# OmerKerner/noLZSS

Measured on AMD Instinct MI355X. Metric: bases/sec factorized (1 GB sigma=4 DNA) + HBM GB/s fraction, higher is better.
Workload: dtype u32; 1 GPU; dna1g: one 2^30-base synthetic DNA sequence per GPU (sigma=4, 40% copied blocks, 1% substitutions), full factorization to (start,length,ref) records in HBM; bases_per_gpu=1073741824, parallelism=1 independent sequence shard(s), all-gather of counts

## Files before the change

### nolzss_amd/csrc/batch.hip

```cpp
#include "api_internal.hpp"

#include <array>

namespace nolzss {
namespace api {

constexpr uint8_t kBatchSeparator = 0x01;

struct RecordPlanScope {
    Context &ctx;
    RecordScatterPlan plan;
    RecordPlanScope(Context &c, const std::vector<uint32_t> &seps, uint32_t n) : ctx(c) {
        static const bool off = getenv("NOLZSS_NO_RECORD_SCATTER") != nullptr;
        if (off || seps.empty()) return;
        std::vector<uint32_t> terms(seps);
        terms.push_back(n);
        if (record_scatter_plan(terms, n, ctx.arena, ctx.stream, plan)) ctx.rec_plan = &plan;
    }
    ~RecordPlanScope() { ctx.rec_plan = nullptr; }
    RecordPlanScope(const RecordPlanScope &) = delete;
    RecordPlanScope &operator=(const RecordPlanScope &) = delete;
};
constexpr size_t kMergeChunkBases = size_t(1) << 25;
constexpr size_t kMergeLanes = 2;

__global__ void batch_bounds_kernel(const nolzss_factor *__restrict__ recs, uint32_t z,
                                    const uint32_t *__restrict__ seps, uint32_t nsep, uint32_t *__restrict__ fidx,
                                    uint32_t *__restrict__ err) {
    const uint32_t k = blockIdx.x * blockDim.x + threadIdx.x;
    if (k >= nsep) return;
    const uint64_t target = seps[k];
    uint32_t lo = 0, hi = z;
    while (lo < hi) {
        const uint32_t mid = lo + ((hi - lo) >> 1);
        if (recs[mid].start >= target)
            hi = mid;
        else
            lo = mid + 1;
    }
    fidx[k] = lo;
    if (lo >= z || recs[lo].start != target || recs[lo].length != 1) atomicOr(err, 1u);
}

__global__ void batch_bounds_pos_kernel(const uint32_t *__restrict__ fpos, uint32_t z,
                                        const uint32_t *__restrict__ seps, uint32_t nsep, uint32_t *__restrict__ fidx,
                                        uint32_t *__restrict__ err) {
    const uint32_t k = blockIdx.x * blockDim.x + threadIdx.x;
    if (k >= nsep) return;
    const uint32_t target = seps[k];
    uint32_t lo = 0, hi = z;
    while (lo < hi) {
        const uint32_t mid = lo + ((hi - lo) >> 1);
        if (fpos[mid] >= target)
            hi = mid;
        else
            lo = mid + 1;
    }
    fidx[k] = lo;
    if (lo >= z || fpos[lo] != target || (lo + 1 < z && fpos[lo + 1] != target + 1)) atomicOr(err, 1u);
}

__global__ void batch_rebase_kernel(nolzss_factor *__restrict__ recs, uint32_t z, TermTable terms) {
    const uint32_t j = blockIdx.x * blockDim.x + threadIdx.x;
    if (j >= z) return;
    const uint64_t p = recs[j].start;
    const uint32_t k = term_lower_bound(terms, (uint32_t)p);
    const uint64_t base = k ? (uint64_t)terms.pos[k - 1] + 1 : 0;
    recs[j].start = p - base;
    const uint64_t ref = recs[j].ref, flag = ref & (1ull << 63);
    recs[j].ref = ((ref ^ flag) - base) | flag;
}

void *alloc_factor_block(size_t bytes) {
    constexpr size_t kHuge = size_t(1) << 21;
    if (bytes >= 4 * kHuge) {
        void *p = nullptr;
        if (posix_memalign(&p, kHuge, (bytes + kHuge - 1) & ~(kHuge - 1)) == 0 && p) {
            (void)madvise(p, (bytes + kHuge - 1) & ~(kHuge - 1), MADV_HUGEPAGE);
            return p;
        }
    }
    return std::malloc(bytes);
}

bool run_merged_chunk(Context &ctx, const uint8_t *const *texts, const size_t *lens, const std::vector<size_t> &ids,
                      bool with_rc, size_t *zs, nolzss_factor **fs, std::vector<void *> *blocks, size_t *zs_plain) {
    if (zs_plain && (!with_rc || fs)) throw std::logic_error("run_merged_chunk: plain counts come with reverse-complement counts only");
    const bool trace = getenv("NOLZSS_TRACE") != nullptr;
    const auto t_begin = std::chrono::steady_clock::now();
    auto since = [&] { return std::chrono::duration<double, std::milli>(std::chrono::steady_clock::now() - t_begin).count(); };
    const size_t c = ids.size();
    size_t n = c - 1;
    for (size_t j : ids) n += lens[j];
    const bool direct = n / c >= (size_t(1) << 16);
    uint8_t *host = direct ? nullptr : host_stage(ctx, n);
    std::vector<uint32_t> seps;
    seps.reserve(c - 1);
    {
        size_t at = 0;
        for (size_t k = 0; k < c; ++k) {
            if (!direct) std::memcpy(host + at, texts[ids[k]], lens[ids[k]]);
            at += lens[ids[k]];
            if (k + 1 < c) {
                seps.push_back((uint32_t)at);
                if (!direct) host[at] = kBatchSeparator;
                ++at;
            }
        }
    }
    const double t_concat = since();
    Arena &arena = ctx.arena;
    hipStream_t s = ctx.stream;
    const size_t m2 = 2 * n + 2;
    reserve_arena_for(ctx, with_rc ? m2 : n, (with_rc ? m2 : 0) + n + 32 * c + (size_t(1) << 20) +
                                                (zs_plain ? 4 * n + (size_t(32) << 20) : 0));
    const size_t mark = arena.mark();
    struct Rewind {
        Arena &a;
        size_t m;
        ~Rewind() { a.rewind(m); }
    } rewind{arena, mark};
    uint8_t *d_text = arena.alloc<uint8_t>(n);
    if (direct) {
        ProfScope ps(ctx.profiler(), "batch_upload", s, (double)n);
        size_t at = 0;
        for (size_t k = 0; k < c; ++k) {
            upload_bytes(ctx, d_text + at, texts[ids[k]], lens[ids[k]]);
            at += lens[ids[k]];
            if (k + 1 < c) HIP_CHECK(hipMemsetAsync(d_text + at++, kBatchSeparator, 1, s));
        }
    } else {
        HIP_CHECK(hipMemcpyAsync(d_text, host, n, hipMemcpyHostToDevice, s));
    }
    PackedText text;
    void *d_recs = nullptr;
    uint32_t *d_fpos = nullptr;
    uint32_t z = 0;
    RcPlainOut plain;
    plain.want_fpos = c > 1;
    if (with_rc) {
        uint8_t *d_S = arena.alloc<uint8_t>(m2);
        prepare_batch_rc_on_device(ctx, d_text, (uint32_t)n, kBatchSeparator, d_S);
        std::vector<uint32_t> terms(seps);
        terms.reserve(2 * c);
        terms.push_back((uint32_t)n);
        for (size_t k = seps.size(); k-- > 0;) terms.push_back((uint32_t)(2 * n - seps[k]));
        terms.push_back((uint32_t)(2 * n + 1));
        if (!pack_independent_text(ctx, d_S, m2, terms, text, true)) return false;
        if (zs_plain)
            z = run_rc_pipeline_packed(ctx, text, 0, nullptr, &plain, &d_fpos);
        else
            z = run_rc_pipeline_packed(ctx, text, 0, &d_recs);
    } else {
        if (!pack_independent_text(ctx, d_text, n, seps, text)) return false;
        RecordPlanScope plan_scope(ctx, seps, (uint32_t)n);
        uint32_t *sa = arena.alloc<uint32_t>(n);
        uint32_t *isa = arena.alloc<uint32_t>(n);
        uint32_t *lcp = arena.alloc<uint32_t>(n + 1);
        bool isa_deferred = false;
        build_suffix_array(ctx, text, sa, isa, lcp, &isa_deferred);
        const Pyramid Psa = alloc_pyramid(sa, (uint32_t)n, arena), Plcp = alloc_pyramid(lcp, (uint32_t)n + 1, arena);
        uint32_t *lstar = arena.alloc<uint32_t>(n);
        build_lstar(ctx, (uint32_t)n, sa, isa, lcp, Psa, Plcp, lstar, isa_deferred ? isa : nullptr, &text);
        z = resolve_chain(ctx, (uint32_t)n, 0, lstar, sa, isa, lcp, Psa, Plcp, fs ? &d_recs : nullptr, 0, nullptr,
                          &d_fpos, fs ? &text.terms : nullptr);
    }
    nolzss_factor *recs = static_cast<nolzss_factor *>(d_recs);
    std::vector<uint32_t> fidx(c, z), fidx_plain(zs_plain ? c : 0, plain.z);
    if (c > 1) {
        uint32_t *d_fidx = arena.alloc<uint32_t>(c);
        HIP_CHECK(hipMemsetAsync(d_fidx + (c - 1), 0, sizeof(uint32_t), s));
        if (with_rc && !zs_plain)
            batch_bounds_kernel<<<(unsigned)div_up(c - 1, 256), 256, 0, s>>>(recs, z, text.terms.pos, (uint32_t)(c - 1),
                                                                             d_fidx, d_fidx + (c - 1));
        else
            batch_bounds_pos_kernel<<<(unsigned)div_up(c - 1, 256), 256, 0, s>>>(d_fpos, z, text.terms.pos,
                                                                                 (uint32_t)(c - 1), d_fidx, d_fidx + (c - 1));
        KERNEL_CHECK();
        uint32_t *d_fidx_plain = nullptr;
        if (zs_plain) {
            d_fidx_plain = arena.alloc<uint32_t>(c);
            HIP_CHECK(hipMemsetAsync(d_fidx_plain + (c - 1), 0, sizeof(uint32_t), s));
            batch_bounds_pos_kernel<<<(unsigned)div_up(c - 1, 256), 256, 0, s>>>(plain.fpos, plain.z, text.terms.pos,
                                                                                 (uint32_t)(c - 1), d_fidx_plain,
                                                                                 d_fidx_plain + (c - 1));
            KERNEL_CHECK();
            HIP_CHECK(hipMemcpyAsync(fidx_plain.data(), d_fidx_plain, c * sizeof(uint32_t), hipMemcpyDeviceToHost, s));
        }
        HIP_CHECK(hipMemcpyAsync(fidx.data(), d_fidx, c * sizeof(uint32_t), hipMemcpyDeviceToHost, s));
        HIP_CHECK(hipStreamSynchronize(s));
        if (fidx[c - 1] || (zs_plain && fidx_plain[c - 1])) throw HipError("merged batch: a separator is not a literal factor");
        fidx[c - 1] = z;
        if (zs_plain) fidx_plain[c - 1] = plain.z;
    }
    nolzss_factor *block = nullptr;
    if (fs && z) {
        if (with_rc) {
            batch_rebase_kernel<<<(unsigned)div_up(z, 256), 256, 0, s>>>(recs, z, text.terms);
            KERNEL_CHECK();
        }
        block = static_cast<nolzss_factor *>(alloc_factor_block(sizeof(nolzss_factor) * (size_t)z));
        if (!block) throw std::bad_alloc();
        try {
            download_bytes(ctx, block, recs, sizeof(nolzss_factor) * (size_t)z);
        } catch (...) {
            std::free(block);
            throw;
        }
    }
    const hipError_t e = hipStreamSynchronize(s);
    if (e != hipSuccess) {
        std::free(block);
        HIP_CHECK(e);
    }
    ctx.prof.collect();
    if (trace)
        fprintf(stderr, "[nolzss] merged batch run: %zu records, %zu symbols, %u factors: gather %.1f ms, device%s %.1f ms\n",
                c, n, z, t_concat, block ? " + download" : "", since() - t_concat);
    if (block) blocks->push_back(block);
    for (size_t k = 0; k < c; ++k) {
        const uint32_t a = k ? fidx[k - 1] + 1 : 0, b = fidx[k];
        zs[ids[k]] = b - a;
        if (fs) fs[ids[k]] = (block && b > a) ? block + a : nullptr;
        if (zs_plain) zs_plain[ids[k]] = (k ? fidx_plain[k] - fidx_plain[k - 1] - 1 : fidx_plain[k]);
    }
    return true;
}

struct GatherRec {
    const uint8_t *src;
    uint64_t off, len;
};
__global__ __launch_bounds__(256) void gather_records_kernel(const GatherRec *__restrict__ recs, uint32_t c,
                                                             uint8_t *__restrict__ dst, uint8_t sep) {
    for (uint32_t k = blockIdx.y; k < c; k += gridDim.y) {
        const GatherRec r = recs[k];
        for (uint64_t p0 = (uint64_t)blockIdx.x * 4096; p0 < r.len; p0 += (uint64_t)gridDim.x * 4096) {
            uint8_t b[16];
#pragma unroll
            for (int j = 0; j < 16; ++j) {
                const uint64_t p = p0 + (uint64_t)j * 256 + threadIdx.x;
                b[j] = r.src[p < r.len ? p : r.len - 1];
            }
#pragma unroll
            for (int j = 0; j < 16; ++j) {
                const uint64_t p = p0 + (uint64_t)j * 256 + threadIdx.x;
                if (p < r.len) dst[r.off + p] = b[j];
            }
        }
        if (blockIdx.x == 0 && threadIdx.x == 0 && k + 1 < c) dst[r.off + r.len] = sep;
    }
}

bool run_merged_chunk_device(Context &ctx, const void *const *d_texts, const size_t *lens, const std::vector<size_t> &ids,
                             bool emit, size_t *zs) {
    const size_t c = ids.size();
    size_t n = c - 1;
    for (size_t j : ids) n += lens[j];
    Arena &arena = ctx.arena;
    hipStream_t s = ctx.stream;
    reserve_arena_for(ctx, n, n + 64 * c + (size_t(1) << 20));
    const size_t mark = arena.mark();
    struct Rewind {
        Arena &a;
        size_t m;
        ~Rewind() { a.rewind(m); }
    } rewind{arena, mark};
    std::vector<GatherRec> table(c);
    std::vector<uint32_t> seps;
    seps.reserve(c - 1);
    {
        size_t at = 0;
        for (size_t k = 0; k < c; ++k) {
            table[k] = GatherRec{static_cast<const uint8_t *>(d_texts[ids[k]]), at, lens[ids[k]]};
            at += lens[ids[k]];
            if (k + 1 < c) seps.push_back((uint32_t)at++);
        }
    }
    uint8_t *d_text = arena.alloc<uint8_t>(n);
    GatherRec *d_table = arena.alloc<GatherRec>(c);
    HIP_CHECK(hipMemcpyAsync(d_table, table.data(), sizeof(GatherRec) * c, hipMemcpyHostToDevice, s));
    {
        ProfScope ps(ctx.profiler(), "batch_gather", s, 2.0 * (double)n);
        const size_t longest = lens[*std::max_element(ids.begin(), ids.end(), [&](size_t a, size_t b) { return lens[a] < lens[b]; })];
        const unsigned gy = (unsigned)std::min<size_t>(c, 32768);
        const unsigned gx = (unsigned)std::max<size_t>(1, std::min<size_t>(div_up(longest, 4096), div_up((size_t)65536, gy)));
        gather_records_kernel<<<dim3(gx, gy), 256, 0, s>>>(d_table, (uint32_t)c, d_text, kBatchSeparator);
        KERNEL_CHECK();
    }
    HIP_CHECK(hipStreamSynchronize(s));
    PackedText text;
    if (!pack_independent_text(ctx, d_text, n, seps, text)) return false;
    RecordPlanScope plan_scope(ctx, seps, (uint32_t)n);
    uint32_t *sa = arena.alloc<uint32_t>(n);
    uint32_t *isa = arena.alloc<uint32_t>(n);
    uint32_t *lcp = arena.alloc<uint32_t>(n + 1);
    bool isa_deferred = false;
    build_suffix_array(ctx, text, sa, isa, lcp, &isa_deferred);
    const Pyramid Psa = alloc_pyramid(sa, (uint32_t)n, arena), Plcp = alloc_pyramid(lcp, (uint32_t)n + 1, arena);
    uint32_t *lstar = arena.alloc<uint32_t>(n);
    build_lstar(ctx, (uint32_t)n, sa, isa, lcp, Psa, Plcp, lstar, isa_deferred ? isa : nullptr, &text);
    void *d_recs = nullptr;
    uint32_t *d_fpos = nullptr;
    const uint32_t z = resolve_chain(ctx, (uint32_t)n, 0, lstar, sa, isa, lcp, Psa, Plcp, emit ? &d_recs : nullptr, 0,
                                     nullptr, &d_fpos, emit ? &text.terms : nullptr);
    std::vector<uint32_t> fidx(c, z);
    if (c > 1) {
        uint32_t *d_fidx = arena.alloc<uint32_t>(c);
        HIP_CHECK(hipMemsetAsync(d_fidx + (c - 1), 0, sizeof(uint32_t), s));
        batch_bounds_pos_kernel<<<(unsigned)div_up(c - 1, 256), 256, 0, s>>>(d_fpos, z, text.terms.pos, (uint32_t)(c - 1),
                                                                             d_fidx, d_fidx + (c - 1));
        KERNEL_CHECK();
        HIP_CHECK(hipMemcpyAsync(fidx.data(), d_fidx, c * sizeof(uint32_t), hipMemcpyDeviceToHost, s));
        HIP_CHECK(hipStreamSynchronize(s));
        if (fidx[c - 1]) throw HipError("merged batch: a separator is not a literal factor");
        fidx[c - 1] = z;
    }
    HIP_CHECK(hipStreamSynchronize(s));
    ctx.prof.collect();
    for (size_t k = 0; k < c; ++k) {
        const uint32_t a = k ? fidx[k - 1] + 1 : 0, b = fidx[k];
        zs[ids[k]] = b - a;
    }
    return true;
}

std::atomic<uint64_t> g_merged_records{0}, g_single_records{0};

void check_records_both(const uint8_t *const *texts, const size_t *lens, size_t m) {
    size_t first_long = m;
    for (size_t j = 0; j < m && first_long == m; ++j)
        if (2 * lens[j] + 2 > kMaxText) first_long = j;
    static const auto cls = [] {
        std::array<uint8_t, 256> t;
        t.fill(2);
        for (const char *b = "ACGT"; *b; ++b) {
            t[(unsigned char)*b] = 0;
            t[(unsigned char)(*b + 32)] = 1;
        }
        return t;
    }();
    std::vector<size_t> start(m + 1, 0);
    for (size_t j = 0; j < m; ++j) start[j + 1] = start[j] + lens[j];
    std::atomic<size_t> first_bad{first_long}, first_lower{m};
    auto lower_to = [](std::atomic<size_t> &a, size_t v) {
        size_t cur = a.load();
        while (v < cur && !a.compare_exchange_weak(cur, v)) {
        }
    };
    host_parallel(start[m], [&](size_t lo, size_t hi) {
        size_t j = (size_t)(std::upper_bound(start.begin(), start.end(), lo) - start.begin()) - 1;
        for (size_t at = lo; at < hi && j < first_bad.load(std::memory_order_relaxed);) {
            while (start[j + 1] <= at) ++j;
            const size_t stop = std::min(hi, start[j + 1]);
            const uint8_t *p = texts[j] + (at - start[j]);
            uint8_t acc = 0;
            for (size_t k = 0, e = stop - at; k < e; ++k) acc |= cls[p[k]];
            if (acc & 2) lower_to(first_bad, j);
            if (acc & 1) lower_to(first_lower, j);
            at = stop;
        }
    });
    const size_t j = first_bad.load();
    if (j < m) {
        if (j == first_long) throw std::invalid_argument("text too long: the device pipeline uses 32-bit indices");
        const size_t k = first_invalid_nucleotide(reinterpret_cast<const char *>(texts[j]), lens[j]);
        throw std::runtime_error("Invalid nucleotide '" + std::string(1, (char)texts[j][k]) + "' found in sequence 0");
    }
    if (first_lower.load() < m)
        throw std::invalid_argument("record " + std::to_string(first_lower.load()) +
                                    " holds lower-case bases: both counts take upper-case A/C/G/T only (the plain count "
                                    "of lower-case letters differs)");
}

[[noreturn]] void rethrow_worker_error(int status, const std::string &message) {
    switch (status) {
    case NOLZSS_ERR_INVALID_ARGUMENT: throw std::invalid_argument(message);
    case NOLZSS_ERR_NOMEM: throw std::bad_alloc();
    case NOLZSS_ERR_DEVICE: throw HipError(message);
    default: throw std::runtime_error(message);
    }
}

std::mutex g_batch_mu;
std::map<nolzss_factor **, std::vector<void *>> g_batch_blocks;

size_t merge_below() {
    const char *e = getenv("NOLZSS_BATCH_MERGE_BELOW");
    return e ? (size_t)atoll(e) : (size_t(1) << 21);
}

BatchPlan plan_batch(const size_t *lens, size_t m, bool with_rc) {
    std::vector<size_t> singles;
    std::vector<std::vector<size_t>> chunks;
    const size_t below = with_rc ? merge_below() / 2 : merge_below();
    static const size_t chunk_bases = [] {
        const char *e = getenv("NOLZSS_BATCH_MERGE_BASES");
        const long long v = e ? atoll(e) : 0;
        return v > 0 ? (size_t)v : kMergeChunkBases;
    }();
    const size_t run_bases = with_rc ? chunk_bases / 2 : chunk_bases;
    const size_t long_below = [] {
        const char *e = getenv("NOLZSS_BATCH_MERGE_LONG_BELOW");
        return e ? (size_t)atoll(e) : (size_t(1) << 27);
    }();
    const size_t long_run_bases = [] {
        const char *e = getenv("NOLZSS_BATCH_MERGE_LONG_BASES");
        const long long v = e ? atoll(e) : 0;
        return v > 0 ? (size_t)v : (size_t(1) << 28);
    }();
    const size_t long_cut = with_rc ? long_below / 2 : long_below;
    const size_t long_run = with_rc ? long_run_bases / 4 : long_run_bases;
    std::vector<size_t> longs;
    if (below > 0)
        for (size_t j = 0; j < m; ++j)
            if (lens[j] >= below && lens[j] < long_cut) longs.push_back(j);
    if (longs.size() >= 2) {
        size_t total = 0;
        for (size_t j : longs) total += lens[j] + 1;
        size_t runs = div_up(total - longs.size(), long_run);
        if (runs < 2 && total >= (with_rc ? size_t(1) << 26 : size_t(1) << 27)) runs = 2;
        const size_t share = div_up(total, runs);
        std::vector<size_t> cur;
        size_t cur_bases = 0;
        for (size_t j : longs) {
            cur.push_back(j);
            cur_bases += lens[j] + 1;
            if (cur_bases >= share) {
                chunks.push_back(std::move(cur));
                cur.clear();
                cur_bases = 0;
            }
        }
        if (!cur.empty()) chunks.push_back(std::move(cur));
    } else {
        longs.clear();
    }
    const bool merge_longs = !longs.empty();
    {
        size_t short_bases = 0;
        for (size_t j = 0; j < m; ++j)
            if (lens[j] && lens[j] < below) short_bases += lens[j] + 1;
        const size_t runs = div_up(short_bases ? short_bases : 1, run_bases);
        const size_t share = div_up(short_bases, runs);
        std::vector<size_t> cur;
        size_t cur_bases = 0;
        for (size_t j = 0; j < m; ++j) {
            if (lens[j] == 0) continue;
            if (lens[j] >= below) {
                if (!(merge_longs && lens[j] < long_cut)) singles.push_back(j);
                continue;
            }
            cur.push_back(j);
// ... 353 lines not shown
```

### nolzss_amd/csrc/c_abi.hip

```cpp
#include "api_internal.hpp"

namespace nolzss {

void Context::read_back(const uint32_t *d_src, uint32_t *dst, int count) {
    HIP_CHECK(hipMemcpyAsync(h_pinned, d_src, sizeof(uint32_t) * count, hipMemcpyDeviceToHost, stream));
    HIP_CHECK(hipStreamSynchronize(stream));
    for (int k = 0; k < count; ++k) dst[k] = h_pinned[k];
}

namespace api {

thread_local std::string g_error;

int set_error(int code, const std::string &msg) {
    g_error = msg;
    return code;
}

std::mutex g_ctx_mu;
std::map<int, std::unique_ptr<DeviceContext>> g_ctx;

size_t arena_bytes_for(size_t n) { return kArenaBytesPerSymbol * n + kArenaSlack; }
size_t arena_min_bytes_for(size_t n) { return kArenaMinPerSymbol * n + kArenaSlack; }

// ... 3 lines not shown
        throw HipError("no HIP device available: libnolzss_hip has no CPU fallback");
    if (device < 0 || device >= count) throw std::invalid_argument("device ordinal out of range");
    if (lane < 0 || lane >= kMaxLanes) throw std::invalid_argument("lane out of range");
    std::lock_guard<std::mutex> lk(g_ctx_mu);
    auto &slot = g_ctx[device * kMaxLanes + lane];
    if (!slot) slot = std::make_unique<DeviceContext>();
    return *slot;
}

size_t trim_idle_arenas(int device, const Context *keep) {
    size_t released = 0;
    std::lock_guard<std::mutex> lk(g_ctx_mu);
    for (auto &kv : g_ctx) {
        DeviceContext &dc = *kv.second;
        if (&dc.ctx == keep || kv.first / kMaxLanes != device) continue;
        std::unique_lock<std::mutex> idle(dc.mu, std::try_to_lock);
        if (!idle.owns_lock()) continue;
        released += dc.ctx.arena.capacity();
        dc.ctx.arena.release();
    }
    return released;
}

void reserve_arena_for(Context &ctx, size_t n, size_t extra) {
    const size_t want = arena_bytes_for(n) + extra, least = arena_min_bytes_for(n) + extra;
    if (want <= ctx.arena.capacity()) return;
    auto available = [&]() -> size_t {
        size_t free_b = 0, total_b = 0;
        if (hipMemGetInfo(&free_b, &total_b) != hipSuccess) return ~size_t(0);
        return (size_t)((double)(free_b + ctx.arena.capacity()) * 0.97);
    };
    size_t avail = available();
    if (avail < want) {
        trim_idle_arenas(ctx.device, &ctx);
        avail = available();
    }
    if (avail < least) {
        if (least <= ctx.arena.capacity()) return;
        size_t free_b = 0, total_b = 0;
        (void)hipMemGetInfo(&free_b, &total_b);
        char buf[320];
        snprintf(buf, sizeof buf,
                 "input too large for this device: a text of %zu symbols needs at least %.1f GiB of device memory "
                 "(%zu bytes per symbol), %.1f GiB are free of %.1f GiB (one MI355X takes about %.1f Gi symbols in plain "
                 "mode, half of that with reverse complement)",
                 n, (double)least / 1073741824.0, kArenaMinPerSymbol, (double)free_b / 1073741824.0,
                 (double)total_b / 1073741824.0, (double)total_b * 0.97 / (double)kArenaMinPerSymbol / 1073741824.0);
        throw std::invalid_argument(buf);
    }
    const size_t take = want <= avail ? want : avail;
    if (take <= ctx.arena.capacity()) return;
    try {
        ctx.arena.reserve(take);
        return;
    } catch (const HipError &) {
        (void)hipGetLastError();
    }
    trim_idle_arenas(ctx.device, &ctx);
    ctx.arena.reserve(least > ctx.arena.capacity() ? least : ctx.arena.capacity());
}

uint8_t *host_stage(Context &ctx, size_t bytes) {
    if (bytes > ctx.h_stage_cap) {
        if (ctx.h_stage) (void)hipHostFree(ctx.h_stage);
        ctx.h_stage = nullptr;
        ctx.h_stage_cap = 0;
        const size_t cap = (bytes + (size_t(1) << 22)) & ~((size_t(1) << 22) - 1);
        HIP_CHECK(hipHostMalloc(reinterpret_cast<void **>(&ctx.h_stage), cap));
        ctx.h_stage_cap = cap;
    }
    return ctx.h_stage;
}

constexpr size_t kCopyChunk = size_t(8) << 20;
constexpr size_t kCopyThreshold = size_t(32) << 20;
int copy_threads() {
    static const int t = [] {
        const char *e = getenv("NOLZSS_COPY_THREADS");
        const long v = e ? atol(e) : 4;
        return (int)(v < 1 ? 1 : (v > 16 ? 16 : v));
    }();
    return t;
}

void upload_bytes(Context &ctx, void *d_dst, const void *h_src, size_t n) {
    HIP_CHECK(hipMemcpyAsync(d_dst, h_src, n, hipMemcpyHostToDevice, ctx.stream));
}

void download_bytes(Context &ctx, void *h_dst, const void *d_src, size_t n) {
    const int T = copy_threads();
    if (n < kCopyThreshold || T <= 1) {
        HIP_CHECK(hipMemcpyAsync(h_dst, d_src, n, hipMemcpyDeviceToHost, ctx.stream));
        HIP_CHECK(hipStreamSynchronize(ctx.stream));
        return;
    }
    uint8_t *ring = host_stage(ctx, (size_t)T * kCopyChunk);
    const size_t chunks = div_up(n, kCopyChunk);
    std::atomic<size_t> next{0};
    std::vector<hipError_t> err((size_t)T, hipSuccess);
    auto work = [&](int t) {
        hipError_t e = hipSetDevice(ctx.device);
        hipEvent_t ev = nullptr;
        if (e == hipSuccess) e = hipEventCreateWithFlags(&ev, hipEventDisableTiming);
        uint8_t *buf = ring + (size_t)t * kCopyChunk;
        while (e == hipSuccess) {
            const size_t c = next.fetch_add(1);
            if (c >= chunks) break;
            const size_t off = c * kCopyChunk, len = n - off < kCopyChunk ? n - off : kCopyChunk;
            e = hipMemcpyAsync(buf, static_cast<const uint8_t *>(d_src) + off, len, hipMemcpyDeviceToHost, ctx.stream);
            if (e == hipSuccess) e = hipEventRecord(ev, ctx.stream);
            if (e == hipSuccess) e = hipEventSynchronize(ev);
            if (e == hipSuccess) std::memcpy(static_cast<uint8_t *>(h_dst) + off, buf, len);
        }
        if (ev) (void)hipEventDestroy(ev);
        err[(size_t)t] = e;
    };
    std::vector<std::thread> threads;
    for (int t = 1; t < T; ++t) threads.emplace_back(work, t);
    work(0);
    for (auto &th : threads) th.join();
    for (hipError_t e : err) HIP_CHECK(e);
}

void order_behind_default_stream(Context &ctx) {
    hipEvent_t ev = nullptr;
    HIP_CHECK(hipEventCreateWithFlags(&ev, hipEventDisableTiming));
    hipError_t e = hipEventRecord(ev, nullptr);
    if (e == hipSuccess) e = hipStreamWaitEvent(ctx.stream, ev, 0);
    (void)hipEventDestroy(ev);
    HIP_CHECK(e);
}

void copy_out(Context &ctx, uint32_t *host, const uint32_t *dev, size_t count) {
    if (!host || !count) return;
    HIP_CHECK(hipMemcpyAsync(host, dev, count * sizeof(uint32_t), hipMemcpyDeviceToHost, ctx.stream));
}

size_t run_plain(Context &ctx, const uint8_t *d_text, size_t n, size_t start_pos, nolzss_factor **out_host,
                 DebugOut *dbg, bool records_on_device_only, const ChainLengthsOut *lengths, void **d_records_out) {
    if (out_host) *out_host = nullptr;
    if (d_records_out) *d_records_out = nullptr;
    if (n == 0 || start_pos >= n) return 0;
    Arena &arena = ctx.arena;
    const size_t mark = arena.mark();
    hipStream_t s = ctx.stream;

    PackedText text = pack_text(ctx, d_text, n);
    uint32_t *sa = arena.alloc<uint32_t>(n);
    uint32_t *isa = arena.alloc<uint32_t>(n);
    uint32_t *lcp = arena.alloc<uint32_t>(n + 1);
    bool isa_deferred = false;
    build_suffix_array(ctx, text, sa, isa, lcp, &isa_deferred);
    const Pyramid Psa = alloc_pyramid(sa, (uint32_t)n, arena), Plcp = alloc_pyramid(lcp, (uint32_t)n + 1, arena);
    uint32_t *lstar = arena.alloc<uint32_t>(n);
    build_lstar(ctx, (uint32_t)n, sa, isa, lcp, Psa, Plcp, lstar, isa_deferred ? isa : nullptr, &text);
    if (dbg) {
        copy_out(ctx, dbg->sa, sa, n);
        copy_out(ctx, dbg->isa, isa, n);
        copy_out(ctx, dbg->lcp, lcp, n + 1);
        copy_out(ctx, dbg->lstar, lstar, n);
        if (dbg->records) {
            const size_t rmark = arena.mark();
            const void *recs = position_factors(ctx, (uint32_t)n, lstar, sa, isa, lcp, Psa, Plcp);
            HIP_CHECK(hipMemcpyAsync(dbg->records, recs, n * sizeof(nolzss_factor), hipMemcpyDeviceToHost, s));
            HIP_CHECK(hipStreamSynchronize(s));
            arena.rewind(rmark);
        }
    }
    void *d_recs = nullptr;
    const uint32_t z = resolve_chain(ctx, (uint32_t)n, (uint32_t)start_pos, lstar, sa, isa, lcp, Psa, Plcp,
                                     (out_host || records_on_device_only || d_records_out) ? &d_recs : nullptr, 0, nullptr, nullptr,
                                     nullptr, lengths);
    if (out_host && z) {
        nolzss_factor *h = static_cast<nolzss_factor *>(alloc_factor_block(sizeof(nolzss_factor) * (size_t)z));
        if (!h) throw std::bad_alloc();
        ProfScope ps(ctx.profiler(), "factors_d2h", s);
        try {
            download_bytes(ctx, h, d_recs, sizeof(nolzss_factor) * (size_t)z);
        } catch (...) {
            std::free(h);
            throw;
        }
        *out_host = h;
    }
    {
        const hipError_t e = hipStreamSynchronize(s);
        if (e != hipSuccess) {
            if (out_host && *out_host) {
                std::free(*out_host);
                *out_host = nullptr;
            }
            HIP_CHECK(e);
        }
    }
    ctx.prof.collect();
    if (d_records_out) *d_records_out = d_recs;
    if (!lengths && !d_records_out) arena.rewind(mark);
    return z;
}

size_t run_plain_host(Context &ctx, const uint8_t *text, size_t n, size_t start_pos, nolzss_factor **out,
                      DebugOut *dbg) {
    if (out) *out = nullptr;
    if (n == 0 || start_pos >= n) return 0;
    reserve_arena_for(ctx, n, n);
    const size_t mark = ctx.arena.mark();
    uint8_t *d_text = ctx.arena.alloc<uint8_t>(n);
    {
        ProfScope ps(ctx.profiler(), "text_h2d", ctx.stream);
        upload_bytes(ctx, d_text, text, n);
    }
    size_t z;
    try {
        z = run_plain(ctx, d_text, n, start_pos, out, dbg);
    } catch (...) {
        ctx.arena.rewind(mark);
        throw;
    }
    ctx.arena.rewind(mark);
    return z;
}

void check_text_args(const void *text, size_t n, size_t start_pos) {
    if (n && !text) throw std::invalid_argument("text pointer is null");
    if (n > kMaxText) throw std::invalid_argument("text too long: the device pipeline uses 32-bit indices");
    if (start_pos > n) throw std::invalid_argument("start_pos beyond the end of the text");
}

uint8_t rc_sentinel(size_t index) {
    uint8_t s = 1;
    size_t count = 0;
    for (;;) {
        if (s != 0 && s != 'A' && s != 'C' && s != 'G' && s != 'T') {
            if (count == index) return s;
            ++count;
        }
        ++s;
        if (s == 0) s = 1;
    }
}

inline uint8_t upper_base(uint8_t c) { return (c >= 'a' && c <= 'z') ? (uint8_t)(c - 'a' + 'A') : c; }

inline uint8_t complement_base(uint8_t c) {
    switch (c) {
    case 'A': return 'T';
    case 'C': return 'G';
    case 'G': return 'C';
    default: return 'A';
    }
}

struct DnaTables {
    uint8_t invalid[256], comp[256];
    DnaTables() {
        for (int c = 0; c < 256; ++c) {
            invalid[c] = 1;
            comp[c] = 0;
        }
        const char *b = "ACGT", *r = "TGCA";
        for (int i = 0; i < 4; ++i) {
            invalid[(unsigned char)b[i]] = invalid[(unsigned char)(b[i] + 32)] = 0;
            comp[(unsigned char)b[i]] = comp[(unsigned char)(b[i] + 32)] = (uint8_t)r[i];
        }
    }
};
const DnaTables &dna_tables() {
    static const DnaTables t;
    return t;
}

size_t first_invalid_nucleotide(const char *s, size_t n) {
    const DnaTables &t = dna_tables();
    std::atomic<size_t> first{n};
    host_parallel(n, [&](size_t lo, size_t hi) {
        constexpr size_t kBlock = 4096;
        for (size_t at = lo; at < hi && at < first.load(std::memory_order_relaxed); at += kBlock) {
            const size_t stop = std::min(hi, at + kBlock);
            uint8_t bad = 0;
            for (size_t j = at; j < stop; ++j) bad |= t.invalid[(unsigned char)s[j]];
            if (bad)
                for (size_t j = at; j < stop; ++j)
                    if (t.invalid[(unsigned char)s[j]]) {
                        size_t cur = first.load();
                        while (j < cur && !first.compare_exchange_weak(cur, j)) {
                        }
                        return;
                    }
        }
    });
    return first.load();
}
void copy_upper(uint8_t *dst, const char *src, size_t n) {
    host_parallel(n, [&](size_t lo, size_t hi) {
        for (size_t j = lo; j < hi; ++j) dst[j] = (uint8_t)src[j] & 0xdfu;
    });
}
void copy_reverse_complement(uint8_t *dst, const char *src, size_t n) {
    const DnaTables &t = dna_tables();
    host_parallel(n, [&](size_t lo, size_t hi) {
        for (size_t j = lo; j < hi; ++j) dst[j] = t.comp[(unsigned char)src[n - 1 - j]];
    });
}

void prepare_w_rc(const char *const *seqs, const size_t *lens, size_t k, HostBytes &S,
                  size_t &original_length, std::vector<uint64_t> &sentinels) {
    S.clear();
    sentinels.clear();
    original_length = 0;
    if (k == 0) return;
    size_t non_empty = 0, empty = 0, total = 0;
    for (size_t i = 0; i < k; ++i) (lens[i] ? ++non_empty : ++empty);
    if (empty)
        fprintf(stderr, "Warning: Skipping %zu empty sequence(s) in prepare_multiple_dna_sequences_w_rc\n", empty);
    if (non_empty == 0) throw std::runtime_error("All sequences are empty - cannot prepare for factorization");
    if (non_empty > 125)
        throw std::invalid_argument(
            "Too many sequences: maximum 125 sequences supported (due to sentinel character limitations)");
    for (size_t i = 0; i < k; ++i) {
        const size_t j = first_invalid_nucleotide(seqs[i], lens[i]);
// ... 423 lines not shown
```

### nolzss_amd/csrc/chain.hip

```cpp
#include "pipeline.hpp"
#include "pyramid.hpp"
#include "scan.hpp"

#include <cassert>

namespace nolzss {
namespace {

constexpr int kThreads = 256;
constexpr int kTile = 4096;
constexpr int kPerThread = kTile / kThreads;
constexpr uint32_t kNone = 0xffffffffu;

constexpr uint32_t kLenMask = 0x7fffffffu;

__device__ __forceinline__ uint32_t next_pos(uint32_t p, uint32_t code, uint32_t n) {
    const uint32_t L = code & kLenMask;
    const uint64_t nx = (uint64_t)p + (L ? L : 1u);
    return nx > n ? n : (uint32_t)nx;
}

__global__ __launch_bounds__(kThreads) void chain_exit_kernel(const uint32_t *__restrict__ lstar, uint32_t n,
                                                              uint32_t start_pos,
                                                              uint32_t *__restrict__ exit0,
                                                              uint32_t *__restrict__ target_bits) {
    __shared__ uint32_t jump[kTile];
    const uint32_t base = blockIdx.x * (uint32_t)kTile;
    const uint32_t tile_end = (n - base < (uint32_t)kTile) ? n : base + kTile;
    const int tid = threadIdx.x;
    uint32_t ls[kPerThread];
#pragma unroll
    for (int j = 0; j < kPerThread; ++j) {
        const uint32_t p = base + j * kThreads + tid;
        ls[j] = lstar[p < n ? p : n - 1u];
    }
#pragma unroll
    for (int j = 0; j < kPerThread; ++j) {
        const uint32_t lp = j * kThreads + tid;
        const uint32_t p = base + lp;
        jump[lp] = (p < n) ? next_pos(p, ls[j], n) : n;
    }
    __syncthreads();
    for (int round = 0; round < 13; ++round) {
        int changed = 0;
#pragma unroll
        for (int j = 0; j < kPerThread; ++j) {
            const uint32_t lp = j * kThreads + tid;
            const uint32_t t = jump[lp];
            if (t < tile_end) {
                jump[lp] = jump[t - base];
                changed = 1;
            }
        }
        if (!__syncthreads_or(changed)) break;
    }
#pragma unroll
    for (int j = 0; j < kPerThread; ++j) {
        const uint32_t lp = j * kThreads + tid;
        const uint32_t p = base + lp;
        if (p < n) {
            const uint32_t e = jump[lp];
            exit0[p] = e;
            const bool last = (lp + 1 == (uint32_t)kTile) || (p + 1 >= n);
            if (e < n && (last || jump[lp + 1] != e)) atomicOr(&target_bits[e >> 5], 1u << (e & 31));
        }
    }
    if (blockIdx.x == 0 && tid == 0 && start_pos < n) atomicOr(&target_bits[start_pos >> 5], 1u << (start_pos & 31));
}

__global__ __launch_bounds__(kThreads) void popcount_kernel(const uint32_t *__restrict__ bits, uint32_t nwords,
                                                            uint32_t *__restrict__ counts) {
    const size_t stride = (size_t)gridDim.x * blockDim.x;
    for (size_t w = (size_t)blockIdx.x * blockDim.x + threadIdx.x; w < nwords; w += stride)
        counts[w] = (uint32_t)__popc(bits[w]);
}

__global__ __launch_bounds__(kThreads) void node_fill_kernel(const uint32_t *__restrict__ bits,
                                                             const uint32_t *__restrict__ prefix, uint32_t nwords,
                                                             uint32_t *__restrict__ node_pos) {
    const size_t stride = (size_t)gridDim.x * blockDim.x;
    for (size_t w = (size_t)blockIdx.x * blockDim.x + threadIdx.x; w < nwords; w += stride) {
        uint32_t b = bits[w];
        uint32_t id = prefix[w];
        while (b) {
            const int bit = __ffs((int)b) - 1;
            node_pos[id++] = (uint32_t)(w * 32 + bit);
            b &= b - 1;
        }
    }
}

__device__ __forceinline__ uint32_t node_id(const uint32_t *bits, const uint32_t *prefix, uint32_t p) {
    return prefix[p >> 5] + (uint32_t)__popc(bits[p >> 5] & ((1u << (p & 31)) - 1u));
}

__global__ __launch_bounds__(kThreads) void node_edges_kernel(const uint32_t *__restrict__ node_pos, uint32_t K,
                                                              const uint32_t *__restrict__ exit0, uint32_t n,
                                                              const uint32_t *__restrict__ bits,
                                                              const uint32_t *__restrict__ prefix,
                                                              uint32_t start_pos, uint32_t *__restrict__ nxt,
                                                              uint32_t *__restrict__ reach) {
    const size_t stride = (size_t)gridDim.x * blockDim.x;
    for (size_t k = (size_t)blockIdx.x * blockDim.x + threadIdx.x; k <= K; k += stride) {
        if (k == K) {
            nxt[k] = K;
            reach[k] = 0;
            continue;
        }
        const uint32_t p = node_pos[k];
        const uint32_t e = exit0[p];
        nxt[k] = (e >= n) ? K : node_id(bits, prefix, e);
        reach[k] = (p == start_pos) ? 1u : 0u;
    }
}

__global__ __launch_bounds__(kThreads) void wyllie_kernel(const uint32_t *__restrict__ nxt_in,
                                                          uint32_t *__restrict__ nxt_out, uint32_t K,
                                                          uint32_t *reach) {
    const size_t stride = (size_t)gridDim.x * blockDim.x;
    for (size_t k = (size_t)blockIdx.x * blockDim.x + threadIdx.x; k < K; k += stride) {
        const uint32_t w = nxt_in[k];
        if (w < K) {
            if (reach[k]) reach[w] = 1u;
            nxt_out[k] = nxt_in[w];
        } else {
            nxt_out[k] = K;
        }
    }
}

__global__ __launch_bounds__(kThreads) void tile_entries_kernel(const uint32_t *__restrict__ node_pos,
                                                                const uint32_t *__restrict__ reach, uint32_t K,
                                                                uint32_t *__restrict__ entry) {
    const size_t stride = (size_t)gridDim.x * blockDim.x;
    for (size_t k = (size_t)blockIdx.x * blockDim.x + threadIdx.x; k < K; k += stride)
        if (reach[k]) {
            const uint32_t p = node_pos[k];
            entry[p / kTile] = p;
        }
}

__global__ __launch_bounds__(64) void chain_mark_kernel(const uint32_t *__restrict__ lstar, uint32_t n,
                                                        const uint32_t *__restrict__ entry,
                                                        unsigned long long *__restrict__ chain_bits,
                                                        uint32_t *__restrict__ tile_count) {
    __shared__ uint16_t jmp[kTile];
    __shared__ unsigned long long bits[kTile / 64];
    const uint32_t base = blockIdx.x * (uint32_t)kTile;
    const uint32_t tile_end = (n - base < (uint32_t)kTile) ? n : base + kTile;
    const int lane = threadIdx.x;
    const uint32_t e = entry[blockIdx.x];
    const size_t word0 = (size_t)blockIdx.x * (kTile / 64);
    if (e == kNone) {
        chain_bits[word0 + lane] = 0ull;
        if (lane == 0) tile_count[blockIdx.x] = 0;
        return;
    }
    constexpr int kBatch = 16;
    for (int j0 = 0; j0 < kTile / 64; j0 += kBatch) {
        uint32_t ls[kBatch];
#pragma unroll
        for (int j = 0; j < kBatch; ++j) {
            const uint32_t p = base + (uint32_t)(j0 + j) * 64u + lane;
            ls[j] = lstar[p < n ? p : n - 1u];
        }
#pragma unroll
        for (int j = 0; j < kBatch; ++j) {
            const uint32_t lp = (uint32_t)(j0 + j) * 64u + lane;
            const uint32_t p = base + lp;
            uint32_t nl = kTile;
            if (p < n) {
                const uint32_t nx = next_pos(p, ls[j], n);
                if (nx < tile_end) nl = nx - base;
            }
            jmp[lp] = (uint16_t)nl;
        }
    }
    bits[lane] = 0ull;
    __syncthreads();
    if (lane == 0) {
        uint32_t p = e - base, cnt = 0;
        while (p < (uint32_t)kTile) {
            bits[p >> 6] |= 1ull << (p & 63);
            ++cnt;
            p = jmp[p];
        }
        tile_count[blockIdx.x] = cnt;
    }
    __syncthreads();
    chain_bits[word0 + lane] = bits[lane];
}

__global__ __launch_bounds__(64) void emit_positions_kernel(const unsigned long long *__restrict__ chain_bits,
                                                            const uint32_t *__restrict__ tile_off,
                                                            uint32_t *__restrict__ fpos) {
    const int lane = threadIdx.x;
    const size_t word = (size_t)blockIdx.x * (kTile / 64) + lane;
    unsigned long long b = chain_bits[word];
    const uint32_t c = (uint32_t)__popcll(b);
    uint32_t off = wave_scan_inclusive(c, OpAdd<uint32_t>()) - c + tile_off[blockIdx.x];
    const uint32_t p0 = blockIdx.x * (uint32_t)kTile + lane * 64u;
    while (b) {
        const int bit = __ffsll((long long)b) - 1;
        fpos[off++] = p0 + (uint32_t)bit;
        b &= b - 1;
    }
}

template <bool kRC>
__global__ __launch_bounds__(kThreads) void length_hist_kernel(const unsigned long long *__restrict__ chain_bits,
                                                               uint32_t nwords, const uint32_t *__restrict__ lstar,
                                                               uint32_t *__restrict__ hist,
                                                               uint64_t *__restrict__ tail,
                                                               uint32_t *__restrict__ tail_count, uint32_t tail_cap) {
    constexpr uint32_t T = kLengthHistBins;
    constexpr uint32_t kBins = kRC ? 2 * T : T;
    __shared__ uint32_t h[kBins];
    for (uint32_t b = threadIdx.x; b < kBins; b += kThreads) h[b] = 0;
    __syncthreads();
    const uint32_t stride = gridDim.x * kThreads;
    for (uint32_t w = blockIdx.x * kThreads + threadIdx.x; w < nwords; w += stride) {
        unsigned long long b = chain_bits[w];
        while (b) {
            const int bit = __ffsll((long long)b) - 1;
            b &= b - 1;
            const uint32_t code = lstar[(size_t)w * 64 + (uint32_t)bit];
            const uint32_t strand = kRC ? (code >> 31) : 0u;
            uint32_t L = code & kLenMask;
            L = L ? L : 1u;
            if (L < T) {
                atomicAdd(&h[strand * T + L], 1u);
            } else {
                const uint32_t slot = atomicAdd(tail_count, 1u);
                assert(slot < tail_cap);
                if (slot < tail_cap) tail[slot] = (uint64_t)L | ((uint64_t)strand << 32);
            }
        }
    }
    __syncthreads();
    for (uint32_t b = threadIdx.x; b < kBins; b += kThreads)
        if (h[b]) atomicAdd(&hist[b], h[b]);
}

__global__ __launch_bounds__(kThreads) void gather_lengths_kernel(uint32_t *__restrict__ fpos, uint32_t z,
                                                                  const uint32_t *__restrict__ lstar) {
    const size_t stride = (size_t)gridDim.x * blockDim.x;
    for (size_t k = (size_t)blockIdx.x * blockDim.x + threadIdx.x; k < z; k += stride) {
        const uint32_t L = lstar[fpos[k]] & kLenMask;
        fpos[k] = L ? L : 1u;
    }
}

constexpr uint32_t kEmitScan = 4;

struct FactorRec {
    uint64_t start, length, ref;
};

template <bool kRC, bool kRebase>
__global__ __launch_bounds__(kThreads) void factor_kernel(const uint32_t *__restrict__ fpos, uint32_t z,
                                                          const uint32_t *__restrict__ lstar,
                                                          const uint32_t *__restrict__ isa,
                                                          const uint32_t *__restrict__ sa,
                                                          const uint32_t *__restrict__ lcp, Pyramid Psa,
                                                          Pyramid Plcp, Pyramid Pmax, uint32_t rcN,
                                                          FactorRec *__restrict__ out, TermTable terms, uint32_t n) {
    const size_t stride = (size_t)gridDim.x * blockDim.x;
    for (size_t k = (size_t)blockIdx.x * blockDim.x + threadIdx.x; k < z; k += stride) {
        const uint32_t i = fpos[k];
        const uint32_t nxt = k + 1 < z ? fpos[k + 1] : n;
        uint32_t code = nxt - i;
        if (kRC || code == 1u) code = lstar[i];
        const uint32_t L = code & kLenMask;
        const bool is_rc = kRC && (code >> 31);
        FactorRec f;
        f.start = i;
        if (L == 0) {
            f.length = 1;
            f.ref = i;
        } else {
            const uint32_t r = isa[i] - 1u;
            uint32_t lo = r, hi = r + 1, steps = 0;
            while (lcp[lo] >= L) {
                --lo;
                if (++steps == kEmitScan) {
                    lo = (uint32_t)pyr_nearest_left<false>(Plcp, lo, L);
                    break;
                }
            }
            steps = 0;
            while (lcp[hi] >= L) {
                ++hi;
                if (++steps == kEmitScan) {
                    hi = pyr_nearest_right<false>(Plcp, hi, L);
                    break;
                }
            }
            hi -= 1;
            f.length = L;
            if (!is_rc) {
                uint32_t mn;
                if (hi - lo < 2 * kEmitScan) {
                    mn = kNone;
                    for (uint32_t q = lo; q <= hi; ++q) {
                        const uint32_t v = sa[q];
                        mn = v < mn ? v : mn;
                    }
                } else {
                    mn = pyr_range<false>(Psa, lo, hi);
                }
                f.ref = mn;
            } else {
                uint32_t mx;
                if (hi - lo < 2 * kEmitScan) {
                    mx = 0;
                    for (uint32_t q = lo; q <= hi; ++q) {
                        const uint32_t v = sa[q];
                        mx = v > mx ? v : mx;
                    }
                } else {
                    mx = pyr_range<true>(Pmax, lo, hi);
                }
                const uint64_t end = 2ull * rcN - mx;
                f.ref = (1ull << 63) | (end - L + 1);
            }
        }
        if (kRebase) {
            const uint32_t t = term_lower_bound(terms, i);
            const uint64_t base = t ? (uint64_t)terms.pos[t - 1] + 1 : 0;
            f.start -= base;
            f.ref -= base;
        }
        out[k] = f;
    }
}

inline unsigned grid_for(size_t items, unsigned cap = 256u * 16u) {
    size_t g = div_up(items, (size_t)kThreads);
    if (g < 1) g = 1;
    return (unsigned)(g > cap ? cap : g);
}

}

uint32_t resolve_chain(Context &ctx, uint32_t n, uint32_t start_pos, const uint32_t *lstar, const uint32_t *sa,
                       const uint32_t *isa, const uint32_t *lcp, const Pyramid &Psa, const Pyramid &Plcp,
                       void **d_factors_out, uint32_t rcN, const Pyramid *Pmax, uint32_t **d_fpos_out,
                       const TermTable *rebase, const ChainLengthsOut *lengths) {
    hipStream_t s = ctx.stream;
    Arena &arena = ctx.arena;
    if (d_factors_out) *d_factors_out = nullptr;
    if (d_fpos_out) *d_fpos_out = nullptr;
    if (start_pos >= n) return 0;

    const uint32_t num_tiles = (uint32_t)div_up(n, kTile);
    const uint32_t tbits_words = (uint32_t)div_up((size_t)n + 1, 32);

    uint32_t *fpos = nullptr;
    const size_t mark = arena.mark();
    uint32_t *exit0 = arena.alloc<uint32_t>(n);
    uint32_t *tbits = arena.alloc<uint32_t>(tbits_words);
    uint32_t *tprefix = arena.alloc<uint32_t>(tbits_words);
    uint32_t *d_total = arena.alloc<uint32_t>(2);
    HIP_CHECK(hipMemsetAsync(tbits, 0, sizeof(uint32_t) * tbits_words, s));
    {
        ProfScope ps(ctx.profiler(), "chain_exit", s);
        chain_exit_kernel<<<num_tiles, kThreads, 0, s>>>(lstar, n, start_pos, exit0, tbits);
        KERNEL_CHECK();
    }
    {
        ProfScope ps(ctx.profiler(), "chain_nodes", s);
        popcount_kernel<<<grid_for(tbits_words), kThreads, 0, s>>>(tbits, tbits_words, tprefix);
        KERNEL_CHECK();
        scan_exclusive_add_u32(tprefix, tprefix, tbits_words, d_total, arena, s);
    }
    uint32_t K = 0;
    ctx.read_back(d_total, &K, 1);

    uint32_t *node_pos = arena.alloc<uint32_t>(K + 1);
    uint32_t *nxt[2] = {arena.alloc<uint32_t>(K + 1), arena.alloc<uint32_t>(K + 1)};
    uint32_t *reach = arena.alloc<uint32_t>(K + 1);
    uint32_t *entry = arena.alloc<uint32_t>(num_tiles);
    {
        ProfScope ps(ctx.profiler(), "chain_nodes", s);
        node_fill_kernel<<<grid_for(tbits_words), kThreads, 0, s>>>(tbits, tprefix, tbits_words, node_pos);
        KERNEL_CHECK();
        node_edges_kernel<<<grid_for((size_t)K + 1), kThreads, 0, s>>>(node_pos, K, exit0, n, tbits, tprefix,
                                                                       start_pos, nxt[0], reach);
        KERNEL_CHECK();
    }
    {
        ProfScope ps(ctx.profiler(), "chain_wyllie", s);
        int rounds = 1;
        while ((1ull << rounds) < (uint64_t)K + 1) ++rounds;
        int cur = 0;
        for (int r = 0; r < rounds; ++r) {
            wyllie_kernel<<<grid_for(K), kThreads, 0, s>>>(nxt[cur], nxt[cur ^ 1], K, reach);
            KERNEL_CHECK();
            cur ^= 1;
        }
        HIP_CHECK(hipMemsetAsync(entry, 0xff, sizeof(uint32_t) * num_tiles, s));
        tile_entries_kernel<<<grid_for(K), kThreads, 0, s>>>(node_pos, reach, K, entry);
        KERNEL_CHECK();
    }
    unsigned long long *cbits = arena.alloc<unsigned long long>((size_t)num_tiles * (kTile / 64));
    uint32_t *tile_count = arena.alloc<uint32_t>(num_tiles);
    {
        ProfScope ps(ctx.profiler(), "chain_mark", s);
        chain_mark_kernel<<<num_tiles, 64, 0, s>>>(lstar, n, entry, cbits, tile_count);
        KERNEL_CHECK();
        scan_exclusive_add_u32(tile_count, tile_count, num_tiles, d_total + 1, arena, s);
    }
    uint32_t z = 0;
    ctx.read_back(d_total + 1, &z, 1);
    if (lengths) {
        if (d_factors_out || d_fpos_out) throw HipError("resolve_chain: factor lengths come without records");
        if (lengths->hist && z) {
            ProfScope ps(ctx.profiler(), "length_hist", s);
            const uint32_t nwords = num_tiles * (uint32_t)(kTile / 64);
            const unsigned g = grid_for(nwords, 1024);
            if (rcN)
                length_hist_kernel<true><<<g, kThreads, 0, s>>>(cbits, nwords, lstar, lengths->hist, lengths->tail,
                                                                lengths->tail_count, lengths->tail_cap);
            else
                length_hist_kernel<false><<<g, kThreads, 0, s>>>(cbits, nwords, lstar, lengths->hist, lengths->tail,
                                                                 lengths->tail_count, lengths->tail_cap);
            KERNEL_CHECK();
        }
        if (!lengths->order || z == 0) {
            arena.rewind(mark);
            return z;
        }
        fpos = arena.alloc<uint32_t>(z);
        ProfScope ps(ctx.profiler(), "length_emit", s);
        emit_positions_kernel<<<num_tiles, 64, 0, s>>>(cbits, tile_count, fpos);
        KERNEL_CHECK();
        gather_lengths_kernel<<<grid_for(z), kThreads, 0, s>>>(fpos, z, lstar);
        KERNEL_CHECK();
        *lengths->order = fpos;
        return z;
    }
    if ((!d_factors_out && !d_fpos_out) || z == 0) {
        arena.rewind(mark);
        return z;
    }
    fpos = arena.alloc<uint32_t>(z);
    if (!d_factors_out) {
        ProfScope ps(ctx.profiler(), "factor_emit", s);
        emit_positions_kernel<<<num_tiles, 64, 0, s>>>(cbits, tile_count, fpos);
        KERNEL_CHECK();
        *d_fpos_out = fpos;
        return z;
    }
    FactorRec *recs_tmp = arena.alloc<FactorRec>(z);
    {
        ProfScope ps(ctx.profiler(), "factor_emit", s);
        emit_positions_kernel<<<num_tiles, 64, 0, s>>>(cbits, tile_count, fpos);
        KERNEL_CHECK();
        if (rcN) {
            if (rebase) throw HipError("resolve_chain: record-relative output exists in plain mode only");
            factor_kernel<true, false><<<grid_for(z), kThreads, 0, s>>>(fpos, z, lstar, isa, sa, lcp, Psa, Plcp, *Pmax,
                                                                        rcN, recs_tmp, TermTable{}, n);
        } else if (rebase) {
            factor_kernel<false, true><<<grid_for(z), kThreads, 0, s>>>(fpos, z, lstar, isa, sa, lcp, Psa, Plcp, Psa,
                                                                        0u, recs_tmp, *rebase, n);
        } else {
            factor_kernel<false, false><<<grid_for(z), kThreads, 0, s>>>(fpos, z, lstar, isa, sa, lcp, Psa, Plcp, Psa,
                                                                         0u, recs_tmp, TermTable{}, n);
        }
        KERNEL_CHECK();
    }
    *d_factors_out = recs_tmp;
    if (d_fpos_out) *d_fpos_out = fpos;
    return z;
}

void *position_factors(Context &ctx, uint32_t n, const uint32_t *lstar, const uint32_t *sa, const uint32_t *isa,
                       const uint32_t *lcp, const Pyramid &Psa, const Pyramid &Plcp, uint32_t rcN, const Pyramid *Pmax,
                       const TermTable *rebase) {
    if (n == 0) return nullptr;
    hipStream_t s = ctx.stream;
    uint32_t *fpos = ctx.arena.alloc<uint32_t>(n);
    FactorRec *recs = ctx.arena.alloc<FactorRec>(n);
    std::vector<uint32_t> iota(n);
    for (uint32_t i = 0; i < n; ++i) iota[i] = i;
    HIP_CHECK(hipMemcpyAsync(fpos, iota.data(), (size_t)n * sizeof(uint32_t), hipMemcpyHostToDevice, s));
    HIP_CHECK(hipStreamSynchronize(s));
    if (rcN) {
        if (rebase) throw HipError("position_factors: record-relative output exists in plain mode only");
        factor_kernel<true, false><<<grid_for(n), kThreads, 0, s>>>(fpos, n, lstar, isa, sa, lcp, Psa, Plcp, *Pmax, rcN, recs,
                                                                    TermTable{}, n);
    } else if (rebase) {
        factor_kernel<false, true><<<grid_for(n), kThreads, 0, s>>>(fpos, n, lstar, isa, sa, lcp, Psa, Plcp, Psa, 0u, recs,
                                                                    *rebase, n);
    } else {
        factor_kernel<false, false><<<grid_for(n), kThreads, 0, s>>>(fpos, n, lstar, isa, sa, lcp, Psa, Plcp, Psa, 0u, recs,
                                                                     TermTable{}, n);
    }
    KERNEL_CHECK();
    return recs;
}

}
```

### nolzss_amd/csrc/lpnf.hip

```cpp
#include "pipeline.hpp"

#include <cstdlib>
#include "nearest_lds.hpp"
#include "queues.hpp"
#include "text_order.hpp"
#include "scan.hpp"

namespace nolzss {

__global__ void shard_totals_kernel(const uint32_t *const *counts, int nq, uint32_t *totals) {
    const int q = blockIdx.x;
    if (q >= nq) return;
    uint32_t v = threadIdx.x < kQShards ? counts[q][threadIdx.x * kQPad] : 0u;
    v = wave_reduce(v, OpAdd<uint32_t>());
    __shared__ uint32_t s_part[kQShards / 64];
    if (lane_id() == 0) s_part[threadIdx.x >> 6] = v;
    __syncthreads();
    if (threadIdx.x == 0) {
        uint32_t t = 0;
        for (uint32_t k = 0; k < kQShards / 64; ++k) t += s_part[k];
        totals[q] = t;
    }
}

namespace {

constexpr int kThreads = 256;
constexpr uint32_t kFarBothUnknown = 0xfffffffeu;

__device__ __forceinline__ bool lpf_decide(uint32_t i, uint32_t lp, uint32_t jp, uint32_t ls, uint32_t js,
                                           uint32_t *__restrict__ dst) {
    const uint32_t M = lp > ls ? lp : ls;
    if (M == 0) {
        *dst = 0;
        return false;
    }
    const bool ok = (lp == M && i - jp >= M) || (ls == M && i - js >= M);
    if (ok) {
        *dst = M;
        return false;
    }
    uint32_t lo = 0;
    if (lp > 0) { const uint32_t c = lp < i - jp ? lp : i - jp; lo = c > lo ? c : lo; }
    if (ls > 0) { const uint32_t c = ls < i - js ? ls : i - js; lo = c > lo ? c : lo; }
    *dst = lo;
    return true;
}

template <bool kTimed>
__global__ __launch_bounds__(kLdsThreads) void lpf_tile_kernel(const uint32_t *__restrict__ sa,
                                                               const uint32_t *__restrict__ lcp, uint32_t n,
                                                               uint32_t *__restrict__ lstar_by_rank,
                                                               ShardQueue exact_q, uint32_t *__restrict__ far_items,
                                                               uint32_t *__restrict__ far_cnt,
                                                               uint32_t *__restrict__ far_aux,
                                                               unsigned long long *__restrict__ phases,
                                                               uint32_t *__restrict__ psa1, uint32_t *__restrict__ plcp1,
                                                               uint32_t pending_min, uint32_t *__restrict__ pending_flag) {
    constexpr int NS = 2;
    const bool timed = kTimed && phases != nullptr && (blockIdx.x & 15) == 0;
    unsigned long long clk[6] = {0, 0, 0, 0, 0, 0};
    if (timed) clk[0] = __builtin_readcyclecounter();
    __shared__ __align__(16) uint32_t s_sa[kLdsSpan];
    __shared__ __align__(16) uint32_t s_lcp[kLdsSpan + 4];
    __shared__ uint32_t s_len[NS * kLdsTile];
    __shared__ uint16_t s_pos[NS * kLdsTile];
    constexpr int kListCapB = 64;
    __shared__ uint16_t s_list0[kLdsWaves][NS * kLdsPerWave];
    __shared__ uint16_t s_list1[kLdsWaves][NS * kListCapB];
    __shared__ uint32_t s_blk[3 * kBlkTableLen];
    const uint32_t base = blockIdx.x * (uint32_t)kLdsTile;
    const uint32_t shard = blockIdx.x % kQShards;
    stage_tile(sa, lcp, n, base, s_sa, s_lcp, pending_min, pending_flag);
    __syncthreads();
    const BlockTables T = block_tables<false>(s_blk);
    build_block_tables<false>(s_sa, s_lcp, T);
    __syncthreads();
    if (psa1 != nullptr && threadIdx.x < kLdsTile / kBlk) {
        const uint32_t B = (uint32_t)kLdsReach / kBlk + threadIdx.x;
        const uint64_t first = (uint64_t)base + (uint64_t)threadIdx.x * kBlk;
        if (first + kBlk <= (uint64_t)n) {
            psa1[first >> 4] = T.mn[B];
            plcp1[first >> 4] = T.ldn[B];
        }
    }
    if (timed) clk[1] = __builtin_readcyclecounter();
    const int w = threadIdx.x >> 6;
    const uint32_t far_bit = n <= 0x80000000u ? 0x80000000u : 0u;
    lds_search_wave_blocks<NS, NS, false, kLdsPerWave, kListCapB>(s_sa, s_lcp, T, n, base, s_len, s_pos, s_list0[w], s_list1[w],
                                   [](uint32_t) { return true; }, [](uint32_t) { return 0u; }, far_bit,
                                   timed ? clk + 2 : nullptr);
    if (timed) clk[4] = __builtin_readcyclecounter();
    constexpr int kRows = kLdsPerWave / 64;
    bool far[kRows], exact[kRows];
    uint32_t aux[kRows], known[kRows], fslot[kRows], eslot[kRows];
#pragma unroll
    for (int row = 0; row < kRows; ++row) {
        const int t = w * kLdsPerWave + row * 64 + lane_id();
        const uint64_t rr = (uint64_t)base + t;
        const bool in = rr < n;
        uint32_t up = s_len[t], down = s_len[kLdsTile + t];
        const bool fu = far_is(up, far_bit), fd = far_is(down, far_bit);
        far[row] = far_resolve(up, down, far_bit, 0u) && in;
        exact[row] = false;
        aux[row] = kFarBothUnknown;
        known[row] = 0;
        if (far[row]) {
            if (far_bit && fu != fd) {
                known[row] = fu ? down : up;
                const uint32_t p = match_pos(s_sa, fu ? s_pos[kLdsTile + t] : s_pos[t]);
                aux[row] = (known[row] ? (p & 0x7fffffffu) : 0x7fffffffu) | (fu ? 0x80000000u : 0u);
            }
        } else if (in) {
            exact[row] = lpf_decide(s_sa[t + kLdsReach], up, match_pos(s_sa, s_pos[t]), down, match_pos(s_sa, s_pos[kLdsTile + t]),
                                    lstar_by_rank + rr);
        }
    }
    {
        const uint32_t region = (blockIdx.x * (uint32_t)kLdsWaves + (uint32_t)w);
        uint32_t used = 0;
#pragma unroll
        for (int row = 0; row < kRows; ++row) {
            const uint64_t bal = __ballot(far[row]);
            fslot[row] = region * (uint32_t)kLdsPerWave + used + (uint32_t)__popcll(bal & lanemask_lt());
            used += (uint32_t)__popcll(bal);
        }
        if (lane_id() == 0) far_cnt[region] = used;
    }
    shard_slots<kRows>(exact_q, shard, exact, eslot);
#pragma unroll
    for (int row = 0; row < kRows; ++row) {
        const int t = w * kLdsPerWave + row * 64 + lane_id();
        const uint64_t rr = (uint64_t)base + t;
        if (far[row]) {
            far_items[fslot[row]] = (uint32_t)rr;
            lstar_by_rank[rr] = known[row];
            far_aux[rr] = aux[row];
        }
        if (exact[row]) exact_q.items[eslot[row]] = s_sa[t + kLdsReach];
    }
    if (timed) {
        __builtin_amdgcn_s_waitcnt(0);
        clk[5] = __builtin_readcyclecounter();
        if (lane_id() == 0) {
            for (int k = 0; k < 5; ++k) atomicAdd(phases + k, clk[k + 1] - clk[k]);
            atomicAdd(phases + 5, 1ull);
        }
    }
}

__global__ __launch_bounds__(kThreads) void compact_far_kernel(const uint32_t *__restrict__ far_items,
                                                               const uint32_t *__restrict__ far_cnt,
                                                               const uint32_t *__restrict__ far_off, uint32_t regions,
                                                               uint32_t *__restrict__ far_list) {
    const size_t stride = (size_t)gridDim.x * blockDim.x / 4;
    for (size_t r = ((size_t)blockIdx.x * blockDim.x + threadIdx.x) / 4; r < regions; r += stride) {
        const uint32_t c = far_cnt[r], o = far_off[r];
        for (uint32_t k = threadIdx.x & 3u; k < c; k += 4) far_list[o + k] = far_items[r * (size_t)kLdsPerWave + k];
    }
}

__global__ __launch_bounds__(kThreads) void lpf_far_kernel(const uint32_t *__restrict__ far_list, uint32_t far_count,
                                                           const uint32_t *__restrict__ sa,
                                                           const uint32_t *__restrict__ lcp, uint32_t n,
                                                           Pyramid Psa, Pyramid Plcp,
                                                           const uint32_t *__restrict__ by_rank,
                                                           const uint32_t *__restrict__ far_aux, bool bounded,
                                                           uint32_t *__restrict__ lstar, uint32_t *__restrict__ far_exact) {
    const size_t stride = (size_t)gridDim.x * blockDim.x;
    for (size_t k = (size_t)blockIdx.x * blockDim.x + threadIdx.x; k < far_count; k += stride) {
        const uint32_t r = far_list[k];
        const uint32_t i = sa[r];
        const uint32_t aux = far_aux[r];
        uint32_t lp, jp, ls, js;
        if (!bounded) {
            nearest_up<false>(sa, lcp, Psa, Plcp, r, i, 0u, lp, jp);
            nearest_down<false>(sa, lcp, n, Psa, Plcp, r, i, lp, ls, js);
        } else if (aux == kFarBothUnknown) {
            far_up<false>(sa, Psa, Plcp, r, i, 0u, lp, jp);
            far_down<false>(sa, n, Psa, Plcp, r, i, lp, ls, js);
        } else if (aux >> 31) {
            ls = by_rank[r];
            js = (aux & 0x7fffffffu) == 0x7fffffffu ? kNoPos : (aux & 0x7fffffffu);
            far_up<false>(sa, Psa, Plcp, r, i, ls, lp, jp);
        } else {
            lp = by_rank[r];
            jp = (aux & 0x7fffffffu) == 0x7fffffffu ? kNoPos : (aux & 0x7fffffffu);
            far_down<false>(sa, n, Psa, Plcp, r, i, lp, ls, js);
        }
        far_exact[k] = lpf_decide(i, lp, jp, ls, js, lstar + i) ? i : kNoPos;
    }
}

__global__ __launch_bounds__(kThreads) void lpnf_fallback_list_kernel(const uint32_t *__restrict__ far_exact,
                                                                      uint32_t far_count, uint32_t n,
                                                                      const uint32_t *__restrict__ isa, Pyramid Psa,
                                                                      Pyramid Plcp, uint32_t *__restrict__ lstar) {
    const size_t stride = (size_t)gridDim.x * blockDim.x;
    for (size_t k = (size_t)blockIdx.x * blockDim.x + threadIdx.x; k < far_count; k += stride) {
        const uint32_t i = far_exact[k];
        if (i == kNoPos) continue;
        const uint32_t cap = (n - i) < i ? (n - i) : i;
        lstar[i] = lpnf_search(Psa, Plcp, isa[i] - 1u, i, lstar[i], cap);
    }
}

__global__ __launch_bounds__(kThreads) void lpnf_fallback_kernel(ShardQueue exact_q, uint32_t n,
                                                                 const uint32_t *__restrict__ isa,
                                                                 Pyramid Psa, Pyramid Plcp,
                                                                 uint32_t *__restrict__ lstar) {
    const uint32_t shard = blockIdx.x;
    const uint32_t count = exact_q.counts[shard * kQPad];
    const uint32_t *items = exact_q.items + (size_t)shard * exact_q.cap;
    for (uint32_t k = blockIdx.y * blockDim.x + threadIdx.x; k < count; k += gridDim.y * blockDim.x) {
        const uint32_t i = items[k];
        const uint32_t cap = (n - i) < i ? (n - i) : i;
        lstar[i] = lpnf_search(Psa, Plcp, isa[i] - 1u, i, lstar[i], cap);
    }
}

}

uint32_t build_lstar(Context &ctx, uint32_t n, const uint32_t *sa, const uint32_t *isa, const uint32_t *lcp,
                     const Pyramid &Psa, const Pyramid &Plcp, uint32_t *lstar, uint32_t *isa_fill,
                     const PackedText *fill_pyramids) {
    hipStream_t s = ctx.stream;
    const size_t mark = ctx.arena.mark();
    uint32_t *pending_flag = nullptr;
    if (fill_pyramids) {
        pending_flag = ctx.arena.alloc<uint32_t>(1);
        HIP_CHECK(hipMemsetAsync(pending_flag, 0, sizeof(uint32_t), s));
        inject_pending_for_test(ctx, const_cast<uint32_t *>(lcp), n);
    }
    uint32_t *psa1 = fill_pyramids && Psa.nlev > 1 ? const_cast<uint32_t *>(Psa.lvl[1]) : nullptr;
    uint32_t *plcp1 = fill_pyramids && Plcp.nlev > 1 ? const_cast<uint32_t *>(Plcp.lvl[1]) : nullptr;
    if (!psa1 || !plcp1) psa1 = plcp1 = nullptr;
    const unsigned tiles = (unsigned)div_up(n, kLdsTile);
    ShardQueue exact_q;
    exact_q.cap = (uint32_t)shard_queue_cap(tiles, kLdsTile);
    exact_q.items = ctx.arena.alloc<uint32_t>((size_t)kQShards * exact_q.cap);
    const uint32_t far_regions = tiles * (uint32_t)kLdsWaves;
    uint32_t *far_items = ctx.arena.alloc<uint32_t>((size_t)far_regions * kLdsPerWave);
    uint32_t *far_cnt = ctx.arena.alloc<uint32_t>(far_regions);
    uint32_t *far_off = ctx.arena.alloc<uint32_t>(far_regions);
    uint32_t *qcounts = ctx.arena.alloc<uint32_t>(kQShards * kQPad);
    exact_q.counts = qcounts;
    const uint32_t **count_ptrs = ctx.arena.alloc<const uint32_t *>(1);
    uint32_t *totals = ctx.arena.alloc<uint32_t>(2);
    uint32_t *by_rank = ctx.arena.alloc<uint32_t>(n);
    uint32_t *far_aux = ctx.arena.alloc<uint32_t>(n);
    uint32_t *scratch_idx = ctx.arena.alloc<uint32_t>(n);
    uint32_t *scratch_val = ctx.arena.alloc<uint32_t>(isa_fill ? 2 * (size_t)n : (size_t)n);
    HIP_CHECK(hipMemsetAsync(qcounts, 0, kQShards * kQPad * sizeof(uint32_t), s));
    const uint32_t *h_ptrs[1] = {exact_q.counts};
    HIP_CHECK(hipMemcpyAsync(count_ptrs, h_ptrs, sizeof h_ptrs, hipMemcpyHostToDevice, s));
    HIP_CHECK(hipStreamSynchronize(s));
    auto read_totals = [&](uint32_t h[2]) {
        shard_totals_kernel<<<1, kQShards, 0, s>>>(count_ptrs, 1, totals);
        KERNEL_CHECK();
        ctx.read_back(totals, h, 2);
    };
    {
        ProfScope ps(ctx.profiler(), "lpf", s, 12.0 * (double)n);
        static const bool want_phases = getenv("NOLZSS_LPF_PHASES") != nullptr;
        unsigned long long *phases = nullptr;
        if (want_phases) {
            phases = ctx.arena.alloc<unsigned long long>(8);
            HIP_CHECK(hipMemsetAsync(phases, 0, 64, s));
        }
        if (phases)
            lpf_tile_kernel<true><<<tiles, kLdsThreads, 0, s>>>(sa, lcp, n, by_rank, exact_q, far_items, far_cnt, far_aux, phases, psa1, plcp1,
                                                                pending_threshold(), pending_flag);
        else
            lpf_tile_kernel<false><<<tiles, kLdsThreads, 0, s>>>(sa, lcp, n, by_rank, exact_q, far_items, far_cnt, far_aux, nullptr, psa1,
                                                                 plcp1, pending_threshold(), pending_flag);
        KERNEL_CHECK();
        if (phases) {
            unsigned long long h[8];
            HIP_CHECK(hipMemcpyAsync(h, phases, 64, hipMemcpyDeviceToHost, s));
            HIP_CHECK(hipStreamSynchronize(s));
            const double w = h[5] ? (double)h[5] : 1.0;
            fprintf(stderr, "[nolzss] lpf_tile phases (cycles per wavefront, %llu sampled): stage %.0f  round0 %.0f  %s %.0f  %s %.0f  epilogue %.0f\n",
                    h[5], h[0] / w, h[1] / w, "roundA", h[2] / w, "roundsBC", h[3] / w, h[4] / w);
        }
    }
    scan_exclusive_add_u32(far_cnt, far_off, far_regions, totals + 1, ctx.arena, s);
    if (fill_pyramids) {
        ProfScope ps(ctx.profiler(), "pyramids", s);
        if (psa1) {
            fill_pyramid_tail(Psa, n >> kPyrShift, false, s);
            fill_pyramid_tail(Plcp, n >> kPyrShift, false, s);
            fill_pyramid(Psa, 2, false, s);
            fill_pyramid(Plcp, 2, false, s);
        } else {
            fill_pyramid(Psa, 1, false, s);
            fill_pyramid(Plcp, 1, false, s);
        }
        uint32_t pending = 0;
        ctx.read_back(pending_flag, &pending, 1);
        if (pending) {
            ctx.arena.rewind(mark);
            finish_pending_lcp(ctx, *fill_pyramids, sa, const_cast<uint32_t *>(lcp));
            fill_pyramid(Psa, 1, false, s);
            fill_pyramid(Plcp, 1, false, s);
            return build_lstar(ctx, n, sa, isa, lcp, Psa, Plcp, lstar, isa_fill, nullptr);
        }
    }
    {
        ProfScope ps(ctx.profiler(), "lpf_to_text_order", s);
        uint32_t *idx[2] = {const_cast<uint32_t *>(sa), scratch_idx};
        uint32_t *val[2] = {by_rank, scratch_val};
        bucketed_scatter(idx, val, n, lstar, n, ctx.arena, s, ctx.profiler(), true, true, ctx.rec_plan, isa_fill);
    }
    uint32_t h[2] = {0, 0};
    read_totals(h);
    static const bool trace = getenv("NOLZSS_TRACE") != nullptr;
    if (trace) fprintf(stderr, "[nolzss] lpf: %u ranks to the far queue, %u positions to the exact search so far\n", h[1], h[0]);
    if (h[1] > 0) {
        ProfScope ps(ctx.profiler(), "lpf_far", s);
        uint32_t *far_list = ctx.arena.alloc<uint32_t>(h[1]);
        compact_far_kernel<<<(unsigned)std::min<size_t>(div_up((size_t)far_regions * 4, kThreads), 256u * 16u), kThreads, 0, s>>>(
            far_items, far_cnt, far_off, far_regions, far_list);
        KERNEL_CHECK();
        uint32_t *far_exact = ctx.arena.alloc<uint32_t>(h[1]);
        const unsigned g = (unsigned)std::min<size_t>(256u * 64u, std::max<size_t>(1, div_up(h[1], kThreads)));
        lpf_far_kernel<<<g, kThreads, 0, s>>>(far_list, h[1], sa, lcp, n, Psa, Plcp, by_rank, far_aux, n <= 0x80000000u,
                                              lstar, far_exact);
        KERNEL_CHECK();
        lpnf_fallback_list_kernel<<<g, kThreads, 0, s>>>(far_exact, h[1], n, isa, Psa, Plcp, lstar);
        KERNEL_CHECK();
    }
    if (h[0] > 0) {
        ProfScope ps(ctx.profiler(), "lpnf_fallback", s);
        const unsigned gy = (unsigned)std::min<size_t>(64, std::max<size_t>(1, div_up(h[0], (size_t)kQShards * kThreads)));
        lpnf_fallback_kernel<<<dim3(kQShards, gy), kThreads, 0, s>>>(exact_q, n, isa, Psa, Plcp, lstar);
        KERNEL_CHECK();
    }
    ctx.arena.rewind(mark);
    return h[0];
}

}
```

### nolzss_amd/csrc/pipeline.hpp

```cpp
#pragma once
#include "common.hpp"
#include "pyramid.hpp"
#include "text.hpp"

#include <vector>

namespace nolzss {

struct Context {
    int device = 0;
    hipStream_t stream = nullptr;
    Arena arena;
    Profiler prof;
    uint32_t *h_pinned = nullptr;
    uint8_t *h_stage = nullptr;
    size_t h_stage_cap = 0;
    const struct RecordScatterPlan *rec_plan = nullptr;

    Profiler *profiler() { return prof.enabled() ? &prof : nullptr; }
    void read_back(const uint32_t *d_src, uint32_t *dst, int count);
};

PackedText pack_text(Context &ctx, const uint8_t *d_text, size_t n);
bool pack_independent_text(Context &ctx, const uint8_t *d_text, size_t n, const std::vector<uint32_t> &separators,
                           PackedText &out, bool mirror = false);

int build_suffix_array(Context &ctx, const PackedText &text, uint32_t *sa, uint32_t *isa, uint32_t *lcp,
                       bool *isa_deferred = nullptr);
Pyramid build_lcp_pyramid(Context &ctx, const PackedText &text, const uint32_t *sa, uint32_t *lcp);

struct Pyramid;

uint32_t build_lstar(Context &ctx, uint32_t n, const uint32_t *sa, const uint32_t *isa, const uint32_t *lcp,
                     const Pyramid &Psa, const Pyramid &Plcp, uint32_t *lstar, uint32_t *isa_fill = nullptr,
                     const PackedText *fill_pyramids = nullptr);
uint32_t pending_threshold();
void finish_pending_lcp(Context &ctx, const PackedText &text, const uint32_t *sa, uint32_t *lcp);
void inject_pending_for_test(Context &ctx, uint32_t *lcp, uint32_t n);

constexpr uint32_t kLengthHistBins = 2048;
struct ChainLengthsOut {
    uint32_t *hist = nullptr;
    uint64_t *tail = nullptr;
    uint32_t *tail_count = nullptr;
    uint32_t tail_cap = 0;
    uint32_t **order = nullptr;
};
inline uint32_t length_tail_cap(uint32_t n) { return n / kLengthHistBins + 1u; }
uint32_t resolve_chain(Context &ctx, uint32_t n, uint32_t start_pos, const uint32_t *lstar, const uint32_t *sa,
                       const uint32_t *isa, const uint32_t *lcp, const Pyramid &Psa, const Pyramid &Plcp,
                       void **d_factors_out, uint32_t rcN = 0, const Pyramid *Pmax = nullptr,
                       uint32_t **d_fpos_out = nullptr, const TermTable *rebase = nullptr,
                       const ChainLengthsOut *lengths = nullptr);
void *position_factors(Context &ctx, uint32_t n, const uint32_t *lstar, const uint32_t *sa, const uint32_t *isa,
                       const uint32_t *lcp, const Pyramid &Psa, const Pyramid &Plcp, uint32_t rcN = 0,
                       const Pyramid *Pmax = nullptr, const TermTable *rebase = nullptr);

struct RcPlainOut;
struct RcDebugOut;
uint32_t run_rc_pipeline(Context &ctx, const uint8_t *d_S, size_t m, size_t start_pos, void **d_factors_out,
                         RcPlainOut *plain = nullptr, const ChainLengthsOut *lengths = nullptr,
                         RcDebugOut *dbg = nullptr);
struct RcPlainOut {
    bool want_fpos = false;
    uint32_t z = 0;
    uint32_t *fpos = nullptr;
};
struct RcDebugOut {
    uint32_t *sa = nullptr;
    uint32_t *lcp = nullptr;
    uint32_t *isa = nullptr;
    uint32_t *code = nullptr;
    uint32_t *plain = nullptr;
    void *records = nullptr;
    uint32_t far_ranks = 0;
    uint32_t exact_from_tiles = 0;
    uint32_t exact_total = 0;
    uint32_t compact = 0;
    uint32_t pending_relaunch = 0;
};
uint32_t run_rc_pipeline_packed(Context &ctx, const PackedText &text, size_t start_pos, void **d_factors_out,
                                RcPlainOut *plain = nullptr, uint32_t **d_fpos_out = nullptr,
                                const ChainLengthsOut *lengths = nullptr, RcDebugOut *dbg = nullptr);
void prepare_batch_rc_on_device(Context &ctx, const uint8_t *d_T, uint32_t n, uint8_t separator, uint8_t *d_S);
uint32_t prepare_single_rc_on_device(Context &ctx, const uint8_t *d_T, uint32_t n, uint8_t *d_S);

struct RlzLayout {
    uint32_t total = 0;
    uint32_t block_length = 0;
    uint32_t rc_block_start = 0;
    uint32_t chain_end = 0;
    uint32_t rcN = 0;
    bool with_rc = false;
};
void rlz_candidates(Context &ctx, const uint32_t *sa, const uint32_t *lcp, uint32_t m, uint32_t B, uint32_t E, bool with_rc,
                    uint32_t *by_rank);
uint32_t run_rlz_pipeline(Context &ctx, const uint8_t *d_S, const RlzLayout &lay, void **d_factors_out,
                          uint32_t **d_fpos_out = nullptr, uint32_t *h_codes = nullptr);
void rlz_count_per_target(Context &ctx, const uint32_t *d_fpos, uint32_t z, const uint32_t *d_bounds, uint32_t k,
                          uint32_t *d_counts);

}
```

### nolzss_amd/csrc/radix_sort.hip

```cpp
#include "radix_sort.hpp"

#include "local_sort.hpp"
#include "radix_pass.hpp"

#include <cstdlib>

namespace nolzss {

SortKnobs::SortKnobs() {
    auto set = [](const char *name) { return getenv(name) != nullptr; };
    auto i64 = [](const char *name, long long dflt) { return getenv(name) ? atoll(getenv(name)) : dflt; };
    trace = set("NOLZSS_TRACE");
    scatter_phases = set("NOLZSS_SCATTER_PHASES");
    no_local_sort = set("NOLZSS_NO_LOCAL_SORT");
    local_sort_min_set = set("NOLZSS_LOCAL_SORT_MIN");
    local_sort_min = (size_t)i64("NOLZSS_LOCAL_SORT_MIN", 0);
    no_local_regroup = set("NOLZSS_NO_LOCAL_REGROUP");
    no_key35 = set("NOLZSS_NO_KEY35");
    local_regroup_min = (size_t)i64("NOLZSS_LOCAL_REGROUP_MIN", 3ll << 28);
    test_local_order_fails = set("NOLZSS_TEST_LOCAL_ORDER_FAILS");
    test_local_lookback_fails = set("NOLZSS_TEST_LOCAL_LOOKBACK_FAILS");
    rec_bucket_min = (uint64_t)i64("NOLZSS_REC_BUCKET_MIN", 1ll << 16);
    text_order_hist = set("NOLZSS_TEXT_ORDER_HIST");
    const char *esc = getenv("NOLZSS_TEXT_ORDER_ESC");
    text_order_esc = esc ? (long long)strtoul(esc, nullptr, 0) : -1;
}

const SortKnobs &sort_knobs() {
    static const SortKnobs k;
    return k;
}

namespace {

template <int BITS> struct TextSrc {
    using Raw = SymWords;
    static constexpr bool kFromText = true;
    const uint64_t *__restrict__ words;
    TermTable terms;
    bool segmented;
    bool digit_from_text = true;
    __device__ __forceinline__ Raw load(size_t idx, const TileExtent &) const { return sym_words<BITS>(words, idx); }
    __device__ __forceinline__ uint64_t key_of(const Raw &raw, size_t idx, const TileExtent &) const {
        return initial_key_of<BITS>(sym_word_of<BITS>(raw, idx), terms, segmented, (uint32_t)idx);
    }
    __device__ __forceinline__ uint32_t val(size_t idx) const { return (uint32_t)idx; }
    __device__ __forceinline__ uint32_t hist_digit_of(const Raw &raw, size_t idx, int shift, const TileExtent &ext) const {
        constexpr int kKeyBits = KeyLayout<BITS>::kSyms * BITS + KeyLayout<BITS>::kTagBits;
        if (!segmented && digit_from_text && shift == kKeyBits - kRadixBits)
            return digit_of(sym_word_of<BITS>(raw, idx) >> (64 - kKeyBits), shift);
        return digit_of(key_of(raw, idx, ext), shift);
    }
    __device__ __forceinline__ bool digits_from_window(int shift) const {
        constexpr int kKeyBits = KeyLayout<BITS>::kSyms * BITS + KeyLayout<BITS>::kTagBits;
        return BITS == 2 && !segmented && digit_from_text && shift == kKeyBits - kRadixBits;
    }
    __device__ __forceinline__ uint64_t window(size_t idx) const { return sym_word<BITS>(words, idx); }
    __device__ __forceinline__ uint32_t window_digit(uint64_t w, int j, size_t) const {
        return (uint32_t)((w >> (64 - kRadixBits - 2 * j)) & (uint64_t)(kBins - 1));
    }
};
struct Text16Src {
    using Raw = SymWords;
    static constexpr bool kFromText = true;
    const uint64_t *__restrict__ words;
    uint32_t n;
    __device__ __forceinline__ uint32_t suffix_of(size_t idx) const {
        return idx < 16 ? n - 1u - (uint32_t)idx : (uint32_t)idx - 16u;
    }
    __device__ __forceinline__ Raw load(size_t idx, const TileExtent &) const { return sym_words<2>(words, suffix_of(idx)); }
    __device__ __forceinline__ uint64_t key_of(const Raw &raw, size_t idx, const TileExtent &) const {
        const uint32_t s = suffix_of(idx);
        const uint32_t lim = n - s;
        const uint32_t tag = lim < (uint32_t)kP16Syms ? lim : (uint32_t)kP16Syms;
        return ((sym_word_of<2>(raw, s) >> 32) << kP16TagBits) | tag;
    }
    __device__ __forceinline__ uint32_t val(size_t idx) const { return suffix_of(idx); }
    __device__ __forceinline__ uint32_t hist_digit_of(const Raw &raw, size_t idx, int, const TileExtent &) const {
        return (uint32_t)(sym_word_of<2>(raw, suffix_of(idx)) >> (64 - kRadixBits));
    }
    __device__ __forceinline__ bool digits_from_window(int) const { return true; }
    __device__ __forceinline__ uint64_t window(size_t idx0) const { return sym_word<2>(words, idx0 == 0 ? (uint64_t)n - 16u : idx0 - 16u); }
    __device__ __forceinline__ uint32_t window_digit(uint64_t w, int j, size_t idx0) const {
        const int jj = idx0 == 0 ? 15 - j : j;
        return (uint32_t)((w >> (64 - kRadixBits - 2 * jj)) & (uint64_t)(kBins - 1));
    }
};
struct Text35Src : Text16Src {
    __device__ __forceinline__ uint64_t key_of(const Raw &raw, size_t idx, const TileExtent &) const {
        const uint32_t s = suffix_of(idx);
        const uint32_t lim = n - s;
        const uint32_t tag = lim < (uint32_t)kP35Syms ? lim : (uint32_t)kP35Syms;
        return ((sym_word_of<2>(raw, s) >> (64 - kP35KeyBits)) << kP35TagBits) | tag;
    }
};
struct Text16SegSrc {
    using Raw = SymWords;
    static constexpr bool kFromText = true;
    const uint64_t *__restrict__ words;
    uint32_t n;
    uint32_t treal;
    uint32_t end_shorts;
    uint32_t nshort;
    uint32_t pos[kTermFew];
    __device__ __forceinline__ uint32_t suffix_of(size_t idx) const {
        if (idx < nshort) {
            const uint32_t c0 = treal, c1 = treal + (end_shorts ? 1u : 0u);
            uint32_t L = 0, j = (uint32_t)idx;
            if (idx >= c0) {
                L = 1u + ((uint32_t)idx - c0) / c1;
                j = ((uint32_t)idx - c0) % c1;
            }
            const uint32_t pj = j == 0 ? pos[0] : (j == 1 ? pos[1] : (j == 2 ? pos[2] : pos[3]));
            return pj - L;
        }
        uint32_t p = (uint32_t)idx - nshort;
#pragma unroll
        for (uint32_t k = 0; k + 1 < kTermFew; ++k)
            if (k < treal && p + 15u >= pos[k]) p += 16u;
        return p;
    }
    __device__ __forceinline__ uint32_t limit_of(uint32_t s) const {
        uint32_t next = n;
#pragma unroll
        for (int k = (int)kTermFew - 2; k >= 0; --k)
            if ((uint32_t)k < treal && pos[k] >= s) next = pos[k];
        return next - s;
    }
    __device__ __forceinline__ uint32_t masked(const Raw &raw, uint32_t s, uint32_t &tag) const {
        const uint32_t lim = limit_of(s);
        tag = lim < (uint32_t)kP16Syms ? lim : (uint32_t)kP16Syms;
        uint32_t sym = (uint32_t)(sym_word_of<2>(raw, s) >> 32);
        if (tag < (uint32_t)kP16Syms) sym = tag == 0 ? 0u : (sym & ~((1u << (2 * ((uint32_t)kP16Syms - tag))) - 1u));
        return sym;
    }
    __device__ __forceinline__ Raw load(size_t idx, const TileExtent &) const { return sym_words<2>(words, suffix_of(idx)); }
    __device__ __forceinline__ uint64_t key_of(const Raw &raw, size_t idx, const TileExtent &) const {
        uint32_t tag;
        const uint32_t sym = masked(raw, suffix_of(idx), tag);
        return ((uint64_t)sym << kP16TagBits) | tag;
    }
    __device__ __forceinline__ uint32_t val(size_t idx) const { return suffix_of(idx); }
    __device__ __forceinline__ uint32_t hist_digit_of(const Raw &raw, size_t idx, int, const TileExtent &) const {
        uint32_t tag;
        return masked(raw, suffix_of(idx), tag) >> (32 - kRadixBits);
    }
    __device__ __forceinline__ bool digits_from_window(int) const { return false; }
    __device__ __forceinline__ uint64_t window(size_t) const { return 0; }
};
struct RecordTextSrc {
    using Raw = SymWords;
    static constexpr bool kFromText = true;
    const uint64_t *__restrict__ words;
    const uint32_t *__restrict__ term_pos;
    __device__ __forceinline__ Raw load(size_t idx, const TileExtent &) const { return sym_words<2>(words, idx); }
    __device__ __forceinline__ uint32_t key_of(const Raw &raw, size_t idx, const TileExtent &ext) const {
        const uint64_t w = sym_word_of<2>(raw, idx);
        const uint32_t lim = term_pos[ext.bucket] - (uint32_t)idx;
        const uint32_t tag = lim < (uint32_t)kRecSyms ? lim : (uint32_t)kRecSyms;
        uint32_t sym = (uint32_t)(w >> (64 - kRecSyms * 2));
        if (tag < (uint32_t)kRecSyms) sym &= ~((1u << (2 * (kRecSyms - (int)tag))) - 1u);
        return (sym << kRecTagBits) | tag;
    }
    __device__ __forceinline__ uint32_t val(size_t idx) const { return (uint32_t)idx; }
    __device__ __forceinline__ uint32_t hist_digit_of(const Raw &raw, size_t idx, int shift, const TileExtent &ext) const {
        return digit_of(key_of(raw, idx, ext), shift);
    }
    __device__ __forceinline__ bool digits_from_window(int) const { return false; }
    __device__ __forceinline__ uint64_t window(size_t) const { return 0; }
};

struct RecArraySrc {
    using Raw = uint64_t;
    static constexpr bool kDigitInRecord = true;
    const uint64_t *__restrict__ recs;
    __device__ __forceinline__ Raw load(size_t idx, const TileExtent &) const { return recs[idx]; }
    __device__ __forceinline__ uint64_t rec_of(Raw raw, size_t, const TileExtent &, uint32_t &) const { return raw; }
};
// ... 486 lines not shown
```

### nolzss_amd/csrc/radix_sort.hpp

```cpp
#pragma once
#include "common.hpp"
#include "text.hpp"

#include <vector>

namespace nolzss {

constexpr int kRadixBits = 8;
#ifndef NOLZSS_SORT_TILE
#define NOLZSS_SORT_TILE 4096
#endif
constexpr int kSortTile = NOLZSS_SORT_TILE;
static_assert(kSortTile == 4096 || kSortTile == 8192, "16 keys per thread on 256 or 512 threads");

constexpr int kSegDescWords = 12;
struct SegView {
    const uint32_t *desc = nullptr;
    uint32_t num_tiles = 0;
};

struct TileExtent {
    size_t first;
    uint32_t count;
    uint32_t bucket;
    size_t hist0;
    uint32_t hstride;
    uint32_t bkt_first, bkt_end, prev_ne, next_ne;
    uint32_t aux;
};

__device__ __forceinline__ TileExtent tile_extent(uint32_t tile, size_t n, uint32_t num_tiles, const SegView &seg) {
    TileExtent e;
    if (seg.desc == nullptr) {
        e.first = (size_t)tile * kSortTile;
        e.count = (uint32_t)((n - e.first < (size_t)kSortTile) ? (n - e.first) : (size_t)kSortTile);
        e.bucket = 0;
        e.hist0 = tile;
        e.hstride = num_tiles;
        e.bkt_first = 0;
        e.bkt_end = (uint32_t)n;
        e.prev_ne = e.next_ne = 0;
        e.aux = 0;
        return e;
    }
    const uint4 *d = reinterpret_cast<const uint4 *>(seg.desc + (size_t)tile * kSegDescWords);
    const uint4 a = d[0], b = d[1], c = d[2];
    e.first = a.x;
    e.count = a.y;
    e.bucket = a.z;
    e.hist0 = a.w;
    e.hstride = b.x;
    e.bkt_first = b.y;
    e.bkt_end = b.z;
    e.prev_ne = b.w;
    e.next_ne = c.x;
    e.aux = c.y;
    return e;
}

struct SortKnobs {
    SortKnobs();
    bool trace;
    bool scatter_phases;
    bool no_local_sort;
    bool local_sort_min_set;
    size_t local_sort_min;
    static constexpr size_t kLocalSortMinText = size_t(1) << 28;
    static constexpr size_t kLocalSortMinRecord = size_t(1) << 20;
    size_t local_min(size_t dflt) const { return local_sort_min_set ? local_sort_min : dflt; }
    bool no_local_regroup;
    size_t local_regroup_min;
    bool no_key35;
    bool test_local_order_fails;
    bool test_local_lookback_fails;
    uint64_t rec_bucket_min;
    bool text_order_hist;
    long long text_order_esc;
};
const SortKnobs &sort_knobs();

int radix_sort_pairs(uint64_t *keys[2], uint32_t *vals[2], size_t n, const int *shifts,
                     int npasses, Arena &arena, hipStream_t stream, Profiler *prof = nullptr);
int radix_sort_pairs(uint32_t *keys[2], uint32_t *vals[2], size_t n, const int *shifts,
                     int npasses, Arena &arena, hipStream_t stream, Profiler *prof = nullptr);

void radix_pass_low16(const uint32_t *keys, const uint32_t *vals, uint16_t *keys16_out, uint32_t *vals_out, size_t n, int shift,
                      Arena &arena, hipStream_t stream, Profiler *prof = nullptr);

int radix_sort_initial_keys(const PackedText &text, uint64_t *keys[2], uint32_t *vals[2], const int *shifts,
                            int npasses, Arena &arena, hipStream_t stream, Profiler *prof = nullptr);

void radix_sort_dna_keys(const PackedText &text, uint32_t *keys32[2], uint32_t *vals[2], uint32_t *seg_mem,
                         SegView &seg_out, Arena &arena, hipStream_t stream, Profiler *prof = nullptr);

bool key16_applicable(const PackedText &text);
struct Round0Regroup {
    uint32_t *lcp = nullptr;
    uint32_t *new_slot = nullptr, *new_grp = nullptr;
    uint32_t *d_total = nullptr;
    bool done = false;
};
void radix_sort_dna_keys16(const PackedText &text, uint32_t *keys32[2], uint32_t *vals[2], uint32_t *seg_mem,
                           SegView &seg_out, Arena &arena, hipStream_t stream, Profiler *prof = nullptr,
                           Round0Regroup *regroup = nullptr, bool key35 = false);
bool key35_applicable(const PackedText &text);

void radix_sort_dna_keys16_fused(const PackedText &text, uint64_t *rec[2], uint32_t *sa_out, uint32_t *seg_mem,
                                 SegView &seg_out, Arena &arena, hipStream_t stream, Profiler *prof = nullptr);

void radix_sort_record_keys(const PackedText &text, const std::vector<uint32_t> &h_terms, uint32_t *keys32[2],
                            uint32_t *vals[2], uint32_t *seg_mem, SegView &seg_out, Arena &arena, hipStream_t stream,
                            Profiler *prof = nullptr);

int radix_sort_segments_u32(uint32_t *keys[2], uint32_t *vals[2], size_t n, const std::vector<uint32_t> &h_start, int npasses,
                            Arena &arena, hipStream_t stream, Profiler *prof = nullptr);

}
```

### nolzss_amd/csrc/rc.hip

```cpp
#include <algorithm>

#include "nearest_lds.hpp"
#include "pipeline.hpp"
#include "queues.hpp"
#include "text_order.hpp"
#include "scan.hpp"

namespace nolzss {
namespace {

constexpr int kThreads = 256;
constexpr uint32_t kRcFlag = 0x80000000u;

__device__ __forceinline__ uint32_t rc_select(uint32_t fwd, uint32_t rc) {
    if (fwd >= 1) return (rc > fwd) ? (rc | kRcFlag) : fwd;
    return (rc > 1) ? (rc | kRcFlag) : 0u;
}

template <bool kPlain>
__device__ __forceinline__ bool rc_decide(uint32_t i, uint32_t lp, uint32_t jp, uint32_t ls, uint32_t js,
                                          uint32_t rc, uint32_t *__restrict__ dst, uint32_t *__restrict__ plain) {
    const uint32_t M = lp > ls ? lp : ls;
    const bool fwd_final = (M == 0) || (lp == M && i - jp >= M) || (ls == M && i - js >= M);
    if (fwd_final) {
// ... 320 lines not shown
    const bool fused_level1 = Pmin.nlev > 1 && Plcp.nlev > 1;
    uint32_t *pending_flag = arena.alloc<uint32_t>(1);
    HIP_CHECK(hipMemsetAsync(pending_flag, 0, sizeof(uint32_t), s));
    inject_pending_for_test(ctx, lcp, m);
    uint32_t *code = arena.alloc<uint32_t>(m);
    uint32_t *plain = plain_out ? arena.alloc<uint32_t>(N) : nullptr;
    {
        const size_t mark = arena.mark();
        const unsigned tiles = (unsigned)div_up(m, kLdsTile);
        ShardQueue exact_q, far_q;
        exact_q.cap = far_q.cap = (uint32_t)shard_queue_cap(tiles, kLdsTile);
        exact_q.items = arena.alloc<uint32_t>((size_t)kQShards * exact_q.cap);
        exact_q.items2 = arena.alloc<uint32_t>((size_t)kQShards * exact_q.cap);
        far_q.items = arena.alloc<uint32_t>((size_t)kQShards * far_q.cap);
        uint32_t *qcounts = arena.alloc<uint32_t>(2 * kQShards * kQPad);
        exact_q.counts = qcounts;
        far_q.counts = qcounts + kQShards * kQPad;
        const uint32_t **count_ptrs = arena.alloc<const uint32_t *>(2);
        uint32_t *totals = arena.alloc<uint32_t>(2);
        uint32_t *by_rank = arena.alloc<uint32_t>(m);
        static const bool no_compact = getenv("NOLZSS_RC_NO_COMPACT") != nullptr;
        static const uint32_t compact_min = getenv("NOLZSS_RC_COMPACT_MIN") ? (uint32_t)atoll(getenv("NOLZSS_RC_COMPACT_MIN")) : (1u << 22);
        const bool compact = isa_deferred && !no_compact && N >= compact_min && N <= (1u << 30);
        uint32_t *scratch_idx = nullptr, *scratch_val = nullptr, *tile_off = nullptr, *cidx = nullptr;
        uint64_t *cpacked = nullptr;
        if (compact) {
            uint32_t *tile_cnt = arena.alloc<uint32_t>(tiles);
            tile_off = arena.alloc<uint32_t>(tiles);
            cidx = arena.alloc<uint32_t>(N);
            cpacked = arena.alloc<uint64_t>(N);
            ProfScope ps(ctx.profiler(), "rc_candidates", s);
            rc_count_original_kernel<<<tiles, kLdsThreads, 0, s>>>(sa, m, N, tile_cnt);
            KERNEL_CHECK();
            scan_exclusive_add_u32(tile_cnt, tile_off, tiles, nullptr, arena, s);
        } else {
            scratch_idx = arena.alloc<uint32_t>(m);
            scratch_val = arena.alloc<uint32_t>(isa_deferred ? 2 * (size_t)m : (size_t)m);
        }
        uint32_t *plain_by_rank = plain ? (compact ? by_rank : arena.alloc<uint32_t>(m)) : nullptr;
        auto launch_tile = [&](uint32_t *p1, uint32_t *p2, uint32_t *p3, uint32_t pmin, uint32_t *pflag) {
            if (plain)
                rc_tile_kernel<true><<<tiles, kLdsThreads, 0, s>>>(sa, lcp, m, N, by_rank, exact_q, far_q, p1, p2, p3, pmin,
                                                                   pflag, tile_off, cidx, cpacked, plain_by_rank);
            else
                rc_tile_kernel<false><<<tiles, kLdsThreads, 0, s>>>(sa, lcp, m, N, by_rank, exact_q, far_q, p1, p2, p3, pmin,
                                                                    pflag, tile_off, cidx, cpacked, nullptr);
            KERNEL_CHECK();
        };
        HIP_CHECK(hipMemsetAsync(qcounts, 0, 2 * kQShards * kQPad * sizeof(uint32_t), s));
        const uint32_t *h_ptrs[2] = {exact_q.counts, far_q.counts};
        HIP_CHECK(hipMemcpyAsync(count_ptrs, h_ptrs, sizeof h_ptrs, hipMemcpyHostToDevice, s));
        HIP_CHECK(hipStreamSynchronize(s));
        auto read_totals = [&](uint32_t h[2]) {
            shard_totals_kernel<<<2, kQShards, 0, s>>>(count_ptrs, 2, totals);
            KERNEL_CHECK();
            ctx.read_back(totals, h, 2);
        };
        {
            ProfScope ps(ctx.profiler(), "rc_candidates", s);
            launch_tile(fused_level1 ? const_cast<uint32_t *>(Pmin.lvl[1]) : nullptr,
                        fused_level1 ? const_cast<uint32_t *>(Pmax.lvl[1]) : nullptr,
                        fused_level1 ? const_cast<uint32_t *>(Plcp.lvl[1]) : nullptr, pending_threshold(), pending_flag);
        }
        {
            ProfScope ps(ctx.profiler(), "pyramids", s);
            const int from = fused_level1 ? 2 : 1;
            if (fused_level1) {
                fill_pyramid_tail(Pmin, m >> kPyrShift, false, s);
                fill_pyramid_tail(Pmax, m >> kPyrShift, true, s);
                fill_pyramid_tail(Plcp, m >> kPyrShift, false, s);
            }
            fill_pyramid(Pmin, from, false, s);
            fill_pyramid(Pmax, from, true, s);
            fill_pyramid(Plcp, from, false, s);
            uint32_t pending = 0;
            ctx.read_back(pending_flag, &pending, 1);
            if (pending) {
                if (dbg) dbg->pending_relaunch = 1;
                finish_pending_lcp(ctx, text, sa, lcp);
                fill_pyramid(Pmin, 1, false, s);
                fill_pyramid(Pmax, 1, true, s);
                fill_pyramid(Plcp, 1, false, s);
                HIP_CHECK(hipMemsetAsync(qcounts, 0, 2 * kQShards * kQPad * sizeof(uint32_t), s));
                launch_tile(nullptr, nullptr, nullptr, 0u, nullptr);
            }
        }
        {
            ProfScope ps(ctx.profiler(), "rc_to_text_order", s);
            if (compact) {
                permute_packed(cidx, cpacked, N, code, isa, arena, s, ctx.profiler());
            } else {
                uint32_t *idx[2] = {sa, scratch_idx};
                uint32_t *val[2] = {by_rank, scratch_val};
                bucketed_scatter(idx, val, m, code, m, arena, s, ctx.profiler(), true, true, nullptr, isa_deferred ? isa : nullptr,
                                 false);
            }
        }
        if (plain) {
            ProfScope ps(ctx.profiler(), "rc_plain_gather", s);
            size_t g = div_up(N, kThreads);
            if (g > 8192) g = 8192;
            rc_plain_gather_kernel<<<(unsigned)g, kThreads, 0, s>>>(isa, plain_by_rank, N, plain);
            KERNEL_CHECK();
        }
        uint32_t h[2] = {0, 0};
        read_totals(h);
        if (dbg) {
            dbg->compact = compact ? 1u : 0u;
            dbg->far_ranks = h[1];
            dbg->exact_from_tiles = h[0];
        }
        if (h[1] > 0) {
            ProfScope ps(ctx.profiler(), "rc_far", s);
            const unsigned gy = (unsigned)std::min<size_t>(64, std::max<size_t>(1, div_up(h[1], (size_t)kQShards * kThreads)));
            if (plain)
                rc_far_kernel<true><<<dim3(kQShards, gy), kThreads, 0, s>>>(far_q, sa, lcp, m, N, Pmin, Pmax, Plcp, by_rank, code,
                                                                            exact_q, plain);
            else
                rc_far_kernel<false><<<dim3(kQShards, gy), kThreads, 0, s>>>(far_q, sa, lcp, m, N, Pmin, Pmax, Plcp, by_rank, code,
                                                                             exact_q, nullptr);
            KERNEL_CHECK();
            read_totals(h);
        }
        if (h[0] > 0) {
            ProfScope ps(ctx.profiler(), "rc_fallback", s);
            const unsigned gy = (unsigned)std::min<size_t>(64, std::max<size_t>(1, div_up(h[0], (size_t)kQShards * kThreads)));
            if (plain)
                rc_fallback_kernel<true><<<dim3(kQShards, gy), kThreads, 0, s>>>(exact_q, m, isa, lcp, Pmin, Plcp, code, plain);
            else
                rc_fallback_kernel<false><<<dim3(kQShards, gy), kThreads, 0, s>>>(exact_q, m, isa, lcp, Pmin, Plcp, code, nullptr);
            KERNEL_CHECK();
        }
        if (dbg) {
            dbg->exact_total = h[0];
            auto copy_out = [&](uint32_t *host, const uint32_t *dev, size_t count) {
                if (host && count) HIP_CHECK(hipMemcpyAsync(host, dev, count * sizeof(uint32_t), hipMemcpyDeviceToHost, s));
            };
            copy_out(dbg->sa, sa, m);
            copy_out(dbg->lcp, lcp, (size_t)m + 1);
            copy_out(dbg->isa, isa, N);
            copy_out(dbg->code, code, N);
            if (plain) copy_out(dbg->plain, plain, N);
            HIP_CHECK(hipStreamSynchronize(s));
        }
        arena.rewind(mark);
    }
    if (dbg && dbg->records) {
        const size_t mark = arena.mark();
        const void *recs = position_factors(ctx, N, code, sa, isa, lcp, Pmin, Plcp, N, &Pmax);
        HIP_CHECK(hipMemcpyAsync(dbg->records, recs, (size_t)N * 3 * sizeof(uint64_t), hipMemcpyDeviceToHost, s));
        HIP_CHECK(hipStreamSynchronize(s));
        arena.rewind(mark);
    }
    const uint32_t z = resolve_chain(ctx, N, (uint32_t)start_pos, code, sa, isa, lcp, Pmin, Plcp, d_factors_out, N, &Pmax,
                                     d_fpos_out, nullptr, lengths);
    if (plain_out) {
        ProfScope ps(ctx.profiler(), "plain_chain", s);
        plain_out->fpos = nullptr;
        plain_out->z = resolve_chain(ctx, N, 0, plain, sa, isa, lcp, Pmin, Plcp, nullptr, 0, nullptr,
                                     plain_out->want_fpos ? &plain_out->fpos : nullptr);
    }
    return z;
}

}
```

### nolzss_amd/csrc/rlz.hip

```cpp
#include "pipeline.hpp"
#include "text_order.hpp"

namespace nolzss {
namespace {

constexpr int kThreads = 256;
constexpr int kItems = 4;
constexpr int kRows = 4;
constexpr int kTile = kThreads * kItems * kRows;
constexpr int kCarryThreads = 1024;
constexpr uint32_t kInf = 0xffffffffu;

struct Seg {
    uint32_t hf, val;
};
template <int NS> struct St {
    Seg s[NS];
};

__device__ __forceinline__ Seg seg_then(Seg x, Seg y) { return y.hf ? y : Seg{x.hf, x.val < y.val ? x.val : y.val}; }
template <int NS> __device__ __forceinline__ St<NS> st_identity() {
    St<NS> r;
#pragma unroll
    for (int k = 0; k < NS; ++k) r.s[k] = Seg{0u, kInf};
// ... 165 lines not shown
                                                             const uint32_t *__restrict__ lcp, uint32_t m, uint32_t B,
                                                             uint32_t E, const uint4 *__restrict__ carry, uint32_t nb,
                                                             uint32_t *__restrict__ code) {
    constexpr int NW = kThreads / 64;
    __shared__ Seg lds[NS * NW];
    const size_t base = (size_t)blockIdx.x * kTile;
    TileRegs t;
    load_tile(sa, lcp, m, B, base, t);
    uint32_t up[NS][kRows][kItems];
    St<NS> run = st_unpack<NS>(carry[blockIdx.x]);
#pragma unroll
    for (int row = 0; row < kRows; ++row) {
        St<NS> loc = st_identity<NS>();
#pragma unroll
        for (int e = 0; e < kItems; ++e) loc = st_then<NS>(loc, element<NS, false>(t.pos[row][e], t.l[row][e], B, E));
        St<NS> total;
        St<NS> pre = st_then<NS>(run, block_scan<NS, NW, false>(loc, lds, total));
#pragma unroll
        for (int e = 0; e < kItems; ++e) {
            const uint32_t l = t.l[row][e];
#pragma unroll
            for (int k = 0; k < NS; ++k) {
                const uint32_t before = pre.s[k].hf ? pre.s[k].val : 0u;
                up[k][row][e] = before < l ? before : l;
            }
            pre = st_then<NS>(pre, element<NS, false>(t.pos[row][e], l, B, E));
        }
        run = st_then<NS>(run, total);
    }
    run = st_unpack<NS>(carry[nb + blockIdx.x]);
#pragma unroll
    for (int row = kRows - 1; row >= 0; --row) {
        St<NS> loc = st_identity<NS>();
#pragma unroll
        for (int e = kItems - 1; e >= 0; --e) loc = st_then<NS>(loc, element<NS, true>(t.pos[row][e], t.l[row][e], B, E));
        St<NS> total;
        St<NS> pre = st_then<NS>(run, block_scan<NS, NW, true>(loc, lds, total));
        uint32_t out[kItems];
#pragma unroll
        for (int e = kItems - 1; e >= 0; --e) {
            uint32_t len[NS];
#pragma unroll
            for (int k = 0; k < NS; ++k) {
                const uint32_t down = pre.s[k].hf ? pre.s[k].val : 0u;
                len[k] = down > up[k][row][e] ? down : up[k][row][e];
            }
            out[e] = (NS == 1 || len[0] >= len[NS - 1]) ? len[0] : (len[NS - 1] | 0x80000000u);
            pre = st_then<NS>(pre, element<NS, true>(t.pos[row][e], t.l[row][e], B, E));
        }
        const size_t idx = base + ((size_t)row * kThreads + threadIdx.x) * kItems;
        if (idx + kItems <= m) {
            *reinterpret_cast<uint4 *>(code + idx) = make_uint4(out[0], out[1], out[2], out[3]);
        } else {
#pragma unroll
            for (int e = 0; e < kItems; ++e)
                if (idx + e < m) code[idx + e] = out[e];
        }
        run = st_then<NS>(run, total);
    }
}

template <int NS>
void launch_candidates(const uint32_t *sa, const uint32_t *lcp, uint32_t m, uint32_t B, uint32_t E, uint4 *agg, uint4 *carry,
                       uint32_t nb, uint32_t *by_rank, hipStream_t s) {
    rlz_reduce_kernel<NS><<<nb, kThreads, 0, s>>>(sa, lcp, m, B, E, agg, nb);
    KERNEL_CHECK();
    rlz_carry_kernel<NS><<<2, kCarryThreads, 0, s>>>(agg, carry, nb);
    KERNEL_CHECK();
    rlz_apply_kernel<NS><<<nb, kThreads, 0, s>>>(sa, lcp, m, B, E, carry, nb, by_rank);
    KERNEL_CHECK();
}

__global__ __launch_bounds__(kThreads) void rlz_count_kernel(const uint32_t *__restrict__ fpos, uint32_t z,
                                                             const uint32_t *__restrict__ bounds, uint32_t k,
                                                             uint32_t *__restrict__ counts) {
    const uint32_t j = blockIdx.x * kThreads + threadIdx.x;
    if (j >= k) return;
    uint32_t at[2];
    for (int side = 0; side < 2; ++side) {
        const uint32_t x = bounds[2 * j + side];
        uint32_t lo = 0, hi = z;
        while (lo < hi) {
            const uint32_t mid = lo + (hi - lo) / 2;
            if (fpos[mid] < x) lo = mid + 1;
            else hi = mid;
        }
        at[side] = lo;
    }
    counts[j] = at[1] - at[0];
}

}

void rlz_candidates(Context &ctx, const uint32_t *sa, const uint32_t *lcp, uint32_t m, uint32_t B, uint32_t E, bool with_rc,
                    uint32_t *by_rank) {
    if (m == 0) return;
    Arena &arena = ctx.arena;
    hipStream_t s = ctx.stream;
    const size_t mark = arena.mark();
    const uint32_t nb = (uint32_t)div_up(m, kTile);
    uint4 *agg = arena.alloc<uint4>(2 * (size_t)nb), *carry = arena.alloc<uint4>(2 * (size_t)nb);
    {
        ProfScope ps(ctx.profiler(), "rlz_candidates", s, 20.0 * (double)m + 128.0 * (double)nb);
        if (with_rc) launch_candidates<2>(sa, lcp, m, B, E, agg, carry, nb, by_rank, s);
        else launch_candidates<1>(sa, lcp, m, B, E, agg, carry, nb, by_rank, s);
    }
    arena.rewind(mark);
}

void rlz_count_per_target(Context &ctx, const uint32_t *d_fpos, uint32_t z, const uint32_t *d_bounds, uint32_t k,
                          uint32_t *d_counts) {
    if (k == 0) return;
    rlz_count_kernel<<<(unsigned)div_up(k, kThreads), kThreads, 0, ctx.stream>>>(d_fpos, z, d_bounds, k, d_counts);
    KERNEL_CHECK();
}

uint32_t run_rlz_pipeline(Context &ctx, const uint8_t *d_S, const RlzLayout &lay, void **d_factors_out, uint32_t **d_fpos_out,
                          uint32_t *h_codes) {
    if (d_factors_out) *d_factors_out = nullptr;
    if (d_fpos_out) *d_fpos_out = nullptr;
    Arena &arena = ctx.arena;
    hipStream_t s = ctx.stream;
    const PackedText text = pack_text(ctx, d_S, lay.total);
    const uint32_t m = text.n;
    uint32_t *sa = arena.alloc<uint32_t>(m);
    uint32_t *isa = arena.alloc<uint32_t>(m);
    uint32_t *lcp = arena.alloc<uint32_t>((size_t)m + 1);
    build_suffix_array(ctx, text, sa, isa, lcp);
    const Pyramid Plcp = build_lcp_pyramid(ctx, text, sa, lcp);
    Pyramid Pmin, Pmax;
    {
        ProfScope ps(ctx.profiler(), "pyramids", s);
        Pmin = build_pyramid(sa, m, false, arena, s);
        Pmax = lay.with_rc ? build_pyramid(sa, m, true, arena, s) : Pmin;
    }
    uint32_t *code = arena.alloc<uint32_t>(m);
    {
        const size_t mark = arena.mark();
        uint32_t *by_rank = arena.alloc<uint32_t>(m);
        uint32_t *scratch_idx = arena.alloc<uint32_t>(m), *scratch_val = arena.alloc<uint32_t>(m);
        rlz_candidates(ctx, sa, lcp, m, lay.block_length, lay.with_rc ? lay.rc_block_start : kInf, lay.with_rc, by_rank);
        {
            ProfScope ps(ctx.profiler(), "rlz_text_order", s, 12.0 * (double)m);
            uint32_t *idx[2] = {sa, scratch_idx};
            uint32_t *val[2] = {by_rank, scratch_val};
            bucketed_scatter(idx, val, m, code, m, arena, s, ctx.profiler(), true, false);
        }
        arena.rewind(mark);
    }
    if (h_codes && lay.chain_end) {
        HIP_CHECK(hipMemcpyAsync(h_codes, code, (size_t)lay.chain_end * sizeof(uint32_t), hipMemcpyDeviceToHost, s));
        HIP_CHECK(hipStreamSynchronize(s));
    }
    return resolve_chain(ctx, lay.chain_end, lay.block_length + 1u, code, sa, isa, lcp, Pmin, Plcp, d_factors_out, lay.rcN,
                         lay.with_rc ? &Pmax : nullptr, d_fpos_out);
}

}
```

### nolzss_amd/csrc/text_order.hip

```cpp
#include "text_order.hpp"

#include "lookback.hpp"
#include "radix_pass.hpp"

#include <algorithm>
#include <cstdio>

namespace nolzss {
namespace {

struct RankSrc {
    using Raw = uint32_t;
    static constexpr bool kFromText = false;
    const uint32_t *__restrict__ keys;
    const uint32_t *__restrict__ vals;
    __device__ __forceinline__ Raw load(size_t idx, const TileExtent &) const { return keys[idx]; }
    __device__ __forceinline__ uint32_t key_of(Raw raw, size_t, const TileExtent &) const { return raw; }
    __device__ __forceinline__ uint32_t hist_digit_of(Raw raw, size_t, int shift, const TileExtent &) const { return digit_of(raw, shift); }
    __device__ __forceinline__ uint64_t val(size_t idx) const { return (uint64_t)vals[idx] | ((uint64_t)((uint32_t)idx + 1u) << 32); }
    __device__ __forceinline__ bool digits_from_window(int) const { return false; }
    __device__ __forceinline__ uint64_t window(size_t) const { return 0; }
};
struct PairSrc {
    using Raw = uint32_t;
// ... 313 lines not shown
        for (int row = 0; row < kKeysPerThread; ++row) {
            s_rec[local0 + (uint32_t)row * 64] = x[row];
            dpk[row >> 2] |= ((uint32_t)(x[row] >> p.dshift) & 255u) << (8 * (row & 3));
        }
    }
    uint32_t *wcount = s_whist + w * kBins;
#pragma unroll
    for (int row = 0; row < kKeysPerThread; ++row) {
        const bool valid = (uint32_t)w * kWaveSpan + (uint32_t)row * 64 + lane < count;
        const uint32_t d = digit_at(row);
        uint32_t diff_lo = 0, diff_hi = 0;
#pragma unroll
        for (int b = 0; b < kRadixBits; ++b) {
            const uint32_t m = (uint32_t)__builtin_amdgcn_sbfe((int)d, (unsigned)b, 1u);
            const uint64_t bal = __ballot((int)m < 0);
            diff_lo = __builtin_amdgcn_bitop3_b32(m, diff_lo, (uint32_t)bal, 0xde);
            diff_hi = __builtin_amdgcn_bitop3_b32(m, diff_hi, (uint32_t)(bal >> 32), 0xde);
        }
        const uint64_t peers = ~(((uint64_t)diff_hi << 32) | diff_lo) & __ballot(valid);
        const uint64_t below = peers & lanemask_lt();
        uint32_t seen = 0;
        if (valid && below == 0) seen = atomicAdd(&wcount[d], (uint32_t)__popcll(peers));
        lrank[row] = seen | ((uint32_t)__popcll(below) << 11) | ((uint32_t)(peers ? __builtin_ctzll(peers) : 0) << 17);
    }
#pragma unroll
    for (int row = 0; row < kKeysPerThread; ++row) {
        const uint32_t packed = lrank[row];
        lrank[row] = ((uint32_t)__shfl((int)packed, (int)(packed >> 17), 64) & 0x7ffu) + ((packed >> 11) & 63u);
    }
    __syncthreads();

    const int d = tid;
    const bool owner = tid < kBins;
    const uint32_t chain = (uint32_t)(first >> (p.dshift + kRadixBits));
    const uint32_t t0 = (uint32_t)(((size_t)chain << (p.dshift + kRadixBits)) >> kLbTileBits);
    uint64_t *my_desc = p.desc + (size_t)tile * kBins + d;
    uint32_t bin_start, total = 0;
    {
        if (owner)
            for (int k = 0; k < kLbWaves; ++k) total += s_whist[k * kBins + d];
        if (owner) desc_store(my_desc, ((tile == t0 ? 2ull : 1ull) << 32) | total);
        uint32_t tile_total;
        bin_start = block_scan_exclusive<kLbWaves>(total, OpAdd<uint32_t>(), s_scan, tile_total);
        if (owner) {
            uint32_t run = bin_start;
            for (int k = 0; k < kLbWaves; ++k) {
                const uint32_t c = s_whist[k * kBins + d];
                s_whist[k * kBins + d] = run;
                run += c;
            }
        }
    }
    __syncthreads();
    uint64_t rec[kKeysPerThread];
#pragma unroll
    for (int row = 0; row < kKeysPerThread; ++row) {
        lrank[row] += s_whist[w * kBins + digit_at(row)];
        rec[row] = s_rec[local0 + (uint32_t)row * 64];
    }
    __syncthreads();
#pragma unroll
    for (int row = 0; row < kKeysPerThread; ++row) {
        if (local0 + (uint32_t)row * 64 < count) {
            s_rec[lrank[row]] = rec[row];
            if constexpr (kFirst) s_dig[lrank[row]] = (uint8_t)digit_at(row);
        }
    }
    if (owner) {
        uint32_t excl = 0;
        if (tile != t0) {
            int64_t look = (int64_t)tile - 1;
            uint32_t spins = 0;
            for (;;) {
                uint64_t v[kLbLook];
#pragma unroll
                for (int j = 0; j < kLbLook; ++j) {
                    const int64_t k = look - j;
                    v[j] = k >= (int64_t)t0 ? desc_load(p.desc + (size_t)k * kBins + d) : (2ull << 32);
                }
                bool done = false, stalled = false;
#pragma unroll
                for (int j = 0; j < kLbLook; ++j) {
                    if (done || stalled) continue;
                    const uint32_t st = (uint32_t)(v[j] >> 32);
                    if (st == 0) {
                        stalled = true;
                    } else {
                        excl += (uint32_t)v[j];
                        --look;
                        done = st == 2;
                    }
                }
                if (done) break;
                if (stalled) {
                    if (++spins > kSpinLimit) {
                        atomicExch(p.ctl + 1, 1u);
                        break;
                    }
                    __builtin_amdgcn_s_sleep(1);
                }
            }
            desc_store(my_desc, (2ull << 32) | (uint64_t)(excl + total));
        }
        s_glob[d] = ((((uint32_t)chain << kRadixBits) | (uint32_t)d) << p.dshift) + excl - bin_start;
    }
    __syncthreads();
#pragma unroll
    for (int j = 0; j < kKeysPerThread; ++j) {
        const uint32_t q = (uint32_t)j * kLbThreads + tid;
        if (q < count) {
            const uint64_t x = s_rec[q];
            const uint32_t dq = kFirst ? (uint32_t)s_dig[q] : (uint32_t)(x >> p.dshift) & 255u;
            const uint32_t g = s_glob[dq] + q;
            if (g < p.n) p.out[g] = x;
        }
    }
}

__global__ __launch_bounds__(kWindow2Threads) void window_unpack_kernel(const uint64_t *__restrict__ in,
                                                                        uint32_t *__restrict__ out,
                                                                        uint32_t *__restrict__ out2, uint32_t n_out,
                                                                        int window_bits, int low_bits, int rank_bits) {
    __shared__ uint32_t s_out[2 << kWindowBitsMax];
    const uint32_t W = 1u << window_bits;
    uint32_t *s_a = s_out, *s_b = s_out + W;
    const size_t base = (size_t)blockIdx.x << window_bits;
    const uint32_t len = (uint32_t)((n_out - base < (size_t)W) ? (n_out - base) : (size_t)W);
    const uint32_t rank_mask = (uint32_t)((1ull << rank_bits) - 1ull);
    constexpr int kBatch = 4;
    for (uint32_t t0 = 0; t0 < len; t0 += kBatch * kWindow2Threads) {
        uint64_t vv[kBatch];
#pragma unroll
        for (int j = 0; j < kBatch; ++j) {
            const uint32_t t = t0 + (uint32_t)j * kWindow2Threads + threadIdx.x;
            vv[j] = in[base + (t < len ? t : 0u)];
        }
#pragma unroll
        for (int j = 0; j < kBatch; ++j) {
            const uint32_t t = t0 + (uint32_t)j * kWindow2Threads + threadIdx.x;
            if (t < len) {
                const uint32_t at = (uint32_t)vv[j] & (W - 1u);
                s_a[at] = (uint32_t)(vv[j] >> (low_bits + rank_bits));
                s_b[at] = ((uint32_t)(vv[j] >> low_bits) & rank_mask) + 1u;
            }
        }
    }
    __syncthreads();
    for (uint32_t t = threadIdx.x; t < len; t += kWindow2Threads) {
        out[base + t] = s_a[t];
        out2[base + t] = s_b[t];
    }
}

__global__ __launch_bounds__(kThreads) void escape_fixup_kernel(const uint32_t *__restrict__ exc, const uint32_t *__restrict__ ctl,
                                                                uint32_t cap, const uint32_t *__restrict__ idx,
                                                                const uint32_t *__restrict__ code, uint32_t *__restrict__ out) {
    const uint32_t cnt = ctl[2];
    if (cnt > cap) return;
    const size_t stride = (size_t)gridDim.x * blockDim.x;
    for (size_t k = (size_t)blockIdx.x * blockDim.x + threadIdx.x; k < cnt; k += stride) {
        const uint32_t r = exc[k];
        out[idx[r]] = code[r];
    }
}

__global__ __launch_bounds__(kThreads) void code_census_kernel(const uint32_t *__restrict__ code, size_t count,
                                                               unsigned long long *__restrict__ cnt) {
    uint32_t c[7] = {0, 0, 0, 0, 0, 0, 0};
    const size_t stride = (size_t)gridDim.x * blockDim.x;
    for (size_t k = (size_t)blockIdx.x * blockDim.x + threadIdx.x; k < count; k += stride) {
        const uint32_t v = code[k];
#pragma unroll
        for (int b = 0; b < 7; ++b) c[b] += v >= (1u << (10 + b)) ? 1u : 0u;
    }
#pragma unroll
    for (int b = 0; b < 7; ++b) {
        const uint32_t t = wave_reduce(c[b], OpAdd<uint32_t>());
        if (lane_id() == 0 && t) atomicAdd(cnt + b, (unsigned long long)t);
    }
}

bool packed_text_order(const uint32_t *idx, const uint32_t *code, size_t count, uint32_t *out, uint32_t *out2, int nb, int wb,
                       uint64_t *buf_a, Arena &arena, hipStream_t stream, Profiler *prof) {
    const bool trace = sort_knobs().trace;
    const int low_bits = wb + kRadixBits;
    const int code_bits = 64 - nb - low_bits;
    uint32_t esc = (uint32_t)((1ull << code_bits) - 1ull);
    if (sort_knobs().text_order_esc >= 0) esc = std::min<uint32_t>(esc, (uint32_t)sort_knobs().text_order_esc);
    const uint32_t num_tiles = (uint32_t)div_up(count, kLbTile);
    const uint32_t cap = (uint32_t)std::max<size_t>(count / 64, 1024);
    uint64_t *buf_b = arena.alloc<uint64_t>(count);
    uint64_t *desc = arena.alloc<uint64_t>((size_t)kBins * num_tiles);
    uint32_t *exc = arena.alloc<uint32_t>(cap);
    uint32_t *ctl = arena.alloc<uint32_t>(8);
    HIP_CHECK(hipMemsetAsync(ctl, 0, 8 * sizeof(uint32_t), stream));
    LbPass p;
    p.n = (uint32_t)count;
    p.exc = exc;
    p.exc_cap = cap;
    p.esc = esc;
    p.low_bits = low_bits;
    p.rank_bits = nb;
    p.desc = desc;
    {
        ProfScope ps(prof, "rs_scatter.u32", stream, 16.0 * (double)count);
        HIP_CHECK(hipMemsetAsync(desc, 0, (size_t)kBins * num_tiles * sizeof(uint64_t), stream));
        p.idx = idx;
        p.code = code;
        p.out = buf_a;
        p.ctl = ctl;
        p.dshift = wb + kRadixBits;
        lb_partition_kernel<true><<<num_tiles, kLbThreads, 0, stream>>>(p);
        KERNEL_CHECK();
    }
    {
        ProfScope ps(prof, "rs_scatter.u32", stream, 16.0 * (double)count);
        HIP_CHECK(hipMemsetAsync(desc, 0, (size_t)kBins * num_tiles * sizeof(uint64_t), stream));
        p.idx = p.code = nullptr;
        p.in = buf_a;
        p.out = buf_b;
        p.ctl = ctl + 4;
        p.dshift = wb;
        lb_partition_kernel<false><<<num_tiles, kLbThreads, 0, stream>>>(p);
        KERNEL_CHECK();
    }
    {
        ProfScope ps(prof, "window_scatter", stream, 16.0 * (double)count);
        window_unpack_kernel<<<(unsigned)div_up(count, (size_t)1 << wb), kWindow2Threads, 0, stream>>>(
            buf_b, out, out2, (uint32_t)count, wb, low_bits, nb);
        KERNEL_CHECK();
        escape_fixup_kernel<<<256, kThreads, 0, stream>>>(exc, ctl, cap, idx, code, out);
        KERNEL_CHECK();
    }
    uint32_t h[8];
    HIP_CHECK(hipMemcpyAsync(h, ctl, sizeof(h), hipMemcpyDeviceToHost, stream));
    HIP_CHECK(hipStreamSynchronize(stream));
    const bool ok = h[1] == 0 && h[5] == 0 && h[2] <= cap;
    if (trace) {
        unsigned long long *d_cnt = arena.alloc<unsigned long long>(7), hc[7];
        HIP_CHECK(hipMemsetAsync(d_cnt, 0, sizeof(hc), stream));
        code_census_kernel<<<1024, kThreads, 0, stream>>>(code, count, d_cnt);
        KERNEL_CHECK();
        HIP_CHECK(hipMemcpyAsync(hc, d_cnt, sizeof(hc), hipMemcpyDeviceToHost, stream));
        HIP_CHECK(hipStreamSynchronize(stream));
        fprintf(stderr, "[nolzss] text order: %zu codes, >= 2^10..2^16: %llu %llu %llu %llu %llu %llu %llu\n", count, hc[0], hc[1],
                hc[2], hc[3], hc[4], hc[5], hc[6]);
    }
    if (trace)
        fprintf(stderr, "[nolzss] text order: packed look-back partition, %u escaped codes (cap %u, threshold %u)%s\n", h[2], cap,
                esc, ok ? "" : (h[2] > cap ? ": list overflow, histogram form instead" : ": look-back gave up, histogram form instead"));
    return ok;
}

}

bool record_scatter_plan(const std::vector<uint32_t> &h_terms, uint32_t n, Arena &arena, hipStream_t stream,
                         RecordScatterPlan &plan) {
    plan = RecordScatterPlan{};
    const uint32_t nb = (uint32_t)h_terms.size();
    const uint64_t rec_min = sort_knobs().rec_bucket_min;
    if (nb < 2 || h_terms.back() != n || rec_min == 0 || (uint64_t)nb * rec_min > (uint64_t)n) return false;
    constexpr int wb = kWindowBitsMax;
    std::vector<uint32_t> tab(5 * ((size_t)nb + 1)), sep(2 * ((size_t)nb - 1));
    uint32_t *h_first = tab.data(), *h_tile0 = h_first + nb + 1, *h_prev = h_tile0 + nb + 1, *h_next = h_prev + nb + 1,
             *h_aux = h_next + nb + 1;
    std::vector<uint32_t> win;
    uint32_t start = 0, dense = 0;
    h_tile0[0] = 0;
    for (uint32_t k = 0; k < nb; ++k) {
        const uint32_t end = k + 1 < nb ? h_terms[k] + 1 : n;
        const uint32_t len = (k + 1 < nb ? h_terms[k] : n) - start;
        if (len == 0 || len > (1u << (wb + kRadixBits))) return false;
        h_first[k] = k + 1 < nb ? start + 1 : start;
        h_aux[k] = start;
        {
            const uint32_t f0 = k + 1 < nb ? start + 1 : start;
            const uint32_t c0 = (uint32_t)kTile - f0 % 64u;
            h_tile0[k + 1] = h_tile0[k] + (len <= c0 ? 1u : 1u + (uint32_t)div_up((size_t)(len - c0), kTile));
        }
        h_prev[k] = k ? k - 1 : 0xffffffffu;
        h_next[k] = k + 1 < nb ? k + 1 : 0xffffffffu;
        if (k + 1 < nb) {
            sep[2 * (size_t)k] = start;
            sep[2 * (size_t)k + 1] = h_terms[k];
        }
        for (uint32_t w0 = 0; w0 < len; w0 += 1u << wb) {
            win.push_back(dense + w0);
            win.push_back(start + w0);
            win.push_back(len - w0 < (1u << wb) ? len - w0 : (1u << wb));
        }
        dense += len;
        start = end;
    }
    h_first[nb] = n;
    h_prev[nb] = h_next[nb] = h_aux[nb] = 0;
    const uint32_t num_tiles = h_tile0[nb];
    std::vector<uint32_t> desc((size_t)num_tiles * kSegDescWords);
    {
        uint32_t s0 = 0;
        for (uint32_t k = 0; k < nb; ++k) {
            const uint32_t len = (k + 1 < nb ? h_terms[k] : n) - s0;
            const uint32_t first = h_first[k], t0 = h_tile0[k], nt = h_tile0[k + 1] - t0;
            const uint32_t c0 = (uint32_t)kTile - first % 64u;
            for (uint32_t local = 0; local < nt; ++local) {
                uint32_t *d = desc.data() + (size_t)(t0 + local) * kSegDescWords;
                const uint32_t f = local == 0 ? first : first + c0 + (local - 1) * (uint32_t)kTile, e = first + len;
                d[0] = f;
                const uint32_t room = local == 0 ? c0 : (uint32_t)kTile;
                d[1] = e - f < room ? e - f : room;
                d[2] = k;
                d[3] = t0 * (uint32_t)kBins + local;
                d[4] = nt;
                d[5] = first;
                d[6] = e;
                d[7] = h_prev[k];
                d[8] = h_next[k];
                d[9] = h_aux[k];
                d[10] = d[11] = 0;
            }
            s0 = k + 1 < nb ? h_terms[k] + 1 : n;
        }
    }
    uint32_t *d_desc = arena.alloc<uint32_t>(desc.size() + 4);
    uint32_t *d_win = arena.alloc<uint32_t>(win.size());
    uint32_t *d_sep = arena.alloc<uint32_t>(sep.size() + 2);
    HIP_CHECK(hipMemcpyAsync(d_desc, desc.data(), desc.size() * sizeof(uint32_t), hipMemcpyHostToDevice, stream));
    HIP_CHECK(hipMemcpyAsync(d_win, win.data(), win.size() * sizeof(uint32_t), hipMemcpyHostToDevice, stream));
    HIP_CHECK(hipMemcpyAsync(d_sep, sep.data(), sep.size() * sizeof(uint32_t), hipMemcpyHostToDevice, stream));
    HIP_CHECK(hipStreamSynchronize(stream));
    plan.seg.desc = d_desc;
    plan.seg.num_tiles = num_tiles;
    plan.win = d_win;
    plan.num_windows = (uint32_t)(win.size() / 3);
    plan.sep = d_sep;
    plan.num_seps = nb - 1;
    plan.n = n;
    plan.window_bits = wb;
    return true;
}

namespace {

int index_bits(uint64_t n_out) {
    int nb = 1;
    while (nb < 32 && (1ull << nb) < n_out) ++nb;
    return nb;
}
int window_bits_of(int nb) { return nb > 2 * kRadixBits + 10 ? nb - 2 * kRadixBits : 10; }

void rank_scatter(const uint32_t *idx, size_t count, uint32_t *out2, uint32_t n_out, hipStream_t stream, Profiler *prof) {
    ProfScope ps(prof, "bucket_scatter", stream, 8.0 * (double)count);
    const unsigned g = (unsigned)std::min<size_t>(div_up(count, kThreads), 256u * 16u);
    plain_rank_scatter_kernel<<<g, kThreads, 0, stream>>>(idx, count, out2, n_out);
    KERNEL_CHECK();
}

void pair_pass_and_windows(const uint32_t *idx_in, const uint64_t *packed_in, uint16_t *idx16, uint64_t *packed_out, size_t count,
                           int wb, uint32_t *hist, uint32_t num_tiles, uint32_t *out, uint32_t *out2, uint32_t n_out, Arena &arena,
                           hipStream_t stream, Profiler *prof) {
    radix_pass<uint32_t, uint16_t, PairSrc, uint64_t>(PairSrc{idx_in, packed_in}, idx16, packed_out, count, wb + kRadixBits, hist,
                                                      num_tiles, 4.0 * (double)count, 22.0 * (double)count, arena, stream, prof);
    ProfScope ps(prof, "window_scatter", stream, 18.0 * (double)count);
    const uint32_t W = 1u << wb;
    window_scatter2_kernel<<<(unsigned)div_up(n_out, W), kWindow2Threads, 0, stream>>>(idx16, packed_out, out, out2, n_out, wb);
    KERNEL_CHECK();
}

void two_value_hist_form(uint32_t *idx[2], uint32_t *val[2], size_t count, uint32_t *out, uint32_t *out2, uint32_t n_out, int wb,
                         bool keep_input, Arena &arena, hipStream_t stream, Profiler *prof) {
    const uint32_t num_tiles = (uint32_t)div_up(count, kTile);
    uint32_t *hist = arena.alloc<uint32_t>((size_t)kBins * num_tiles);
    uint32_t *idx_b = keep_input ? arena.alloc<uint32_t>(count) : idx[0];
    uint64_t *packed1 = reinterpret_cast<uint64_t *>(val[1]);
    uint64_t *packed2 = arena.alloc<uint64_t>(count);
    radix_pass<uint32_t, uint32_t, RankSrc, uint64_t>(RankSrc{idx[0], val[0]}, idx[1], packed1, count, wb, hist, num_tiles,
                                                      4.0 * (double)count, 20.0 * (double)count, arena, stream, prof);
    pair_pass_and_windows(idx[1], packed1, reinterpret_cast<uint16_t *>(idx_b), packed2, count, wb, hist, num_tiles, out, out2,
                          n_out, arena, stream, prof);
}

bool record_plan_form(uint32_t *idx[2], uint32_t *val[2], size_t count, uint32_t *out, uint32_t *out2, const RecordScatterPlan &plan,
                      Arena &arena, hipStream_t stream, Profiler *prof) {
    uint16_t *idx16 = reinterpret_cast<uint16_t *>(idx[1]);
    uint32_t *hist = arena.alloc<uint32_t>((size_t)kBins * plan.seg.num_tiles);
    uint32_t *err = arena.alloc<uint32_t>(1);
    HIP_CHECK(hipMemsetAsync(err, 0, sizeof(uint32_t), stream));
    if (out2) {
        uint64_t *packed = reinterpret_cast<uint64_t *>(val[1]);
        radix_pass<uint32_t, uint16_t, LocalRankSrc, uint64_t>(LocalRankSrc{idx[0], val[0]}, idx16, packed, count, plan.window_bits,
                                                               hist, plan.seg.num_tiles, 4.0 * (double)count, 18.0 * (double)count,
                                                               arena, stream, prof, plan.seg);
        ProfScope ps(prof, "window_scatter", stream, 18.0 * (double)count);
        record_window_scatter2_kernel<<<plan.num_windows, kWindow2Threads, 0, stream>>>(idx16, packed, out, out2, plan.win,
                                                                                       plan.window_bits);
        KERNEL_CHECK();
    } else {
        radix_pass<uint32_t, uint16_t>(LocalIdxSrc{idx[0], val[0]}, idx16, val[1], count, plan.window_bits, hist, plan.seg.num_tiles,
                                       4.0 * (double)count, 14.0 * (double)count, arena, stream, prof, plan.seg);
        ProfScope ps(prof, "window_scatter", stream, 10.0 * (double)count);
        record_window_scatter_kernel<uint16_t><<<plan.num_windows, kThreads, 0, stream>>>(idx16, val[1], out, plan.win,
                                                                                         plan.window_bits);
        KERNEL_CHECK();
    }
    if (plan.num_seps) {
        separator_scatter_kernel<<<(unsigned)div_up(plan.num_seps, kThreads), kThreads, 0, stream>>>(plan.sep, plan.num_seps, idx[0],
                                                                                                   val[0], out, err, out2);
        KERNEL_CHECK();
    }
    uint32_t h_err = 0;
    HIP_CHECK(hipMemcpyAsync(&h_err, err, sizeof(uint32_t), hipMemcpyDeviceToHost, stream));
    HIP_CHECK(hipStreamSynchronize(stream));
    return h_err == 0;
}

void window_perm_form(uint32_t *idx[2], uint32_t *val[2], size_t count, uint32_t *out, uint32_t n_out, int wb, bool three,
                      bool keep_input, bool keep_val, Arena &arena, hipStream_t stream, Profiler *prof) {
    const int shifts[3] = {wb, wb + kRadixBits, wb + 2 * kRadixBits};
    radix_sort_pairs(idx, val, count, shifts, 1, arena, stream, prof);
    uint32_t *idx2[2] = {idx[1], keep_input ? arena.alloc<uint32_t>(count) : idx[0]};
    uint32_t *val2[2] = {val[1], (keep_input && keep_val) ? arena.alloc<uint32_t>(count) : val[0]};
    if (three) {
        radix_sort_pairs(idx2, val2, count, shifts + 1, 1, arena, stream, prof);
        std::swap(idx2[0], idx2[1]);
        std::swap(val2[0], val2[1]);
    }
    uint16_t *idx16 = reinterpret_cast<uint16_t *>(idx2[1]);
    radix_pass_low16(idx2[0], val2[0], idx16, val2[1], count, shifts[three ? 2 : 1], arena, stream, prof);
    ProfScope ps(prof, "window_scatter", stream, 10.0 * (double)count);
    const uint32_t W = 1u << wb;
    window_scatter_kernel<uint16_t><<<(unsigned)div_up(n_out, W), kThreads, 0, stream>>>(idx16, val2[1], out, n_out, wb);
    KERNEL_CHECK();
}

void partial_then_plain_form(uint32_t *idx[2], uint32_t *val[2], size_t count, uint32_t *out, uint32_t n_out, int nbits, bool big,
                             bool keep_input, bool keep_val, Arena &arena, hipStream_t stream, Profiler *prof) {
    int cur = 0;
    const int window_bits = 19;
    if (big && nbits > window_bits) {
        int shift = window_bits;
        radix_sort_pairs(idx, val, count, &shift, 1, arena, stream, prof);
        cur = 1;
        if (nbits > window_bits + kRadixBits) {
            uint32_t *idx2[2] = {idx[1], keep_input ? arena.alloc<uint32_t>(count) : idx[0]};
            uint32_t *val2[2] = {val[1], (keep_input && keep_val) ? arena.alloc<uint32_t>(count) : val[0]};
            shift = window_bits + kRadixBits;
            radix_sort_pairs(idx2, val2, count, &shift, 1, arena, stream, prof);
            idx[1] = idx2[1];
            val[1] = val2[1];
        }
    }
    ProfScope ps(prof, "bucket_scatter", stream, 12.0 * (double)count);
    const uint32_t num_tiles = (uint32_t)div_up(count, kTile);
    plain_scatter_kernel<<<xcd_grid(num_tiles), kThreads, 0, stream>>>(idx[cur], val[cur], count, out, n_out, num_tiles);
    KERNEL_CHECK();
}

}

void bucketed_scatter(uint32_t *idx[2], uint32_t *val[2], size_t count, uint32_t *out, uint32_t n_out, Arena &arena,
                      hipStream_t stream, Profiler *prof, bool keep_input, bool keep_val, const RecordScatterPlan *plan,
                      uint32_t *out2, bool short_codes) {
    if (count == 0) return;
    const size_t amark = arena.mark();
    const int nbits = index_bits(n_out);
    const bool two_passes = nbits <= 2 * kRadixBits + kWindowBitsMax;
    const int wb = two_passes ? window_bits_of(nbits) : kWindowBitsMax;
    const bool big = (size_t)n_out * 4 > (size_t(64) << 20) && count > (size_t(1) << 22);
    const bool perm = big && count == n_out;
    const bool has_plan = plan && plan->seg.desc;
    const bool plan_form = has_plan && count == n_out && n_out == plan->n;
    const bool two_value = out2 && perm && two_passes && !has_plan;
    if (two_value && short_codes && !sort_knobs().text_order_hist) {
        const bool done = packed_text_order(idx[0], val[0], count, out, out2, nbits, wb, reinterpret_cast<uint64_t *>(val[1]), arena,
                                            stream, prof);
        arena.rewind(amark);
        if (done) return;
    }
    bool separators_ok = true;
    if (two_value) {
        two_value_hist_form(idx, val, count, out, out2, n_out, wb, keep_input, arena, stream, prof);
    } else {
        if (out2 && !plan_form) rank_scatter(idx[0], count, out2, n_out, stream, prof);
        if (plan_form)
            separators_ok = record_plan_form(idx, val, count, out, out2, *plan, arena, stream, prof);
        else if (perm)
            window_perm_form(idx, val, count, out, n_out, wb, !two_passes, keep_input, keep_val, arena, stream, prof);
        else
            partial_then_plain_form(idx, val, count, out, n_out, nbits, big, keep_input, keep_val, arena, stream, prof);
    }
    arena.rewind(amark);
    if (!separators_ok) throw HipError("record scatter: a separator suffix is not the first of its record");
}

void permute_packed(uint32_t *idx, uint64_t *packed, size_t count, uint32_t *out, uint32_t *out2, Arena &arena,
                    hipStream_t stream, Profiler *prof) {
    if (count == 0) return;
    const int nb = index_bits(count);
    if (count <= (size_t(1) << 22) || nb > 2 * kRadixBits + kWindowBitsMax) {
        ProfScope ps(prof, "bucket_scatter", stream, 20.0 * (double)count);
        const unsigned g = (unsigned)std::min<size_t>(div_up(count, kThreads), 256u * 16u);
        plain_packed_scatter_kernel<<<g, kThreads, 0, stream>>>(idx, packed, count, out, out2);
        KERNEL_CHECK();
        return;
    }
    const size_t amark = arena.mark();
    const int wb = window_bits_of(nb);
    const uint32_t num_tiles = (uint32_t)div_up(count, kTile);
    uint32_t *hist = arena.alloc<uint32_t>((size_t)kBins * num_tiles);
    uint32_t *idx_b = arena.alloc<uint32_t>(count);
    uint64_t *packed_b = arena.alloc<uint64_t>(count);
    radix_pass<uint32_t, uint32_t, PairSrc, uint64_t>(PairSrc{idx, packed}, idx_b, packed_b, count, wb, hist, num_tiles,
                                                      4.0 * (double)count, 24.0 * (double)count, arena, stream, prof);
    pair_pass_and_windows(idx_b, packed_b, reinterpret_cast<uint16_t *>(idx), packed, count, wb, hist, num_tiles, out, out2,
                          (uint32_t)count, arena, stream, prof);
    arena.rewind(amark);
}

}
```

### nolzss_amd/csrc/text_order.hpp

```cpp
#pragma once
#include "radix_sort.hpp"

#include <vector>

namespace nolzss {

struct RecordScatterPlan {
    SegView seg;
    const uint32_t *win = nullptr;
    uint32_t num_windows = 0;
    const uint32_t *sep = nullptr;
    uint32_t num_seps = 0;
    uint32_t n = 0;
    int window_bits = 0;
};
void bucketed_scatter(uint32_t *idx[2], uint32_t *val[2], size_t count, uint32_t *out, uint32_t n_out,
                      Arena &arena, hipStream_t stream, Profiler *prof, bool keep_input, bool keep_val = true,
                      const RecordScatterPlan *plan = nullptr, uint32_t *out2 = nullptr, bool short_codes = true);
void permute_packed(uint32_t *idx, uint64_t *packed, size_t count, uint32_t *out, uint32_t *out2, Arena &arena,
                    hipStream_t stream, Profiler *prof);
bool record_scatter_plan(const std::vector<uint32_t> &h_terms, uint32_t n, Arena &arena, hipStream_t stream,
                         RecordScatterPlan &plan);

}
```

Measured before the change: 13.71 billion bases/s.

## Store lstar codes and chain exits as 16-bit with wide-code escape list

Introduces an LstarCodes abstraction that can hold the lstar array as 16-bit codes, with overflow values kept in a separate wide-code list, when the suffix-array path defers ISA and no lengths output is requested. The chain exit, mark, factor and window unpack kernels gain narrow variants that read packed pairs and write 16-bit tile-relative exits. This halves the bytes moved for lstar and exit arrays in bandwidth-bound passes. The cost is extra template paths, escape handling for large codes, and a fallback when the packed text-order path does not apply.

```diff
diff --git a/nolzss_amd/csrc/batch.hip b/nolzss_amd/csrc/batch.hip
--- a/nolzss_amd/csrc/batch.hip
+++ b/nolzss_amd/csrc/batch.hip
@@ -160,7 +160,7 @@
         bool isa_deferred = false;
         build_suffix_array(ctx, text, sa, isa, lcp, &isa_deferred);
         const Pyramid Psa = alloc_pyramid(sa, (uint32_t)n, arena), Plcp = alloc_pyramid(lcp, (uint32_t)n + 1, arena);
-        uint32_t *lstar = arena.alloc<uint32_t>(n);
+        LstarCodes lstar = LstarCodes::of(arena.alloc<uint32_t>(n));
         build_lstar(ctx, (uint32_t)n, sa, isa, lcp, Psa, Plcp, lstar, isa_deferred ? isa : nullptr, &text);
         z = resolve_chain(ctx, (uint32_t)n, 0, lstar, sa, isa, lcp, Psa, Plcp, fs ? &d_recs : nullptr, 0, nullptr,
                           &d_fpos, fs ? &text.terms : nullptr);
@@ -298,7 +298,7 @@
     bool isa_deferred = false;
     build_suffix_array(ctx, text, sa, isa, lcp, &isa_deferred);
     const Pyramid Psa = alloc_pyramid(sa, (uint32_t)n, arena), Plcp = alloc_pyramid(lcp, (uint32_t)n + 1, arena);
-    uint32_t *lstar = arena.alloc<uint32_t>(n);
+    LstarCodes lstar = LstarCodes::of(arena.alloc<uint32_t>(n));
     build_lstar(ctx, (uint32_t)n, sa, isa, lcp, Psa, Plcp, lstar, isa_deferred ? isa : nullptr, &text);
     void *d_recs = nullptr;
     uint32_t *d_fpos = nullptr;
diff --git a/nolzss_amd/csrc/c_abi.hip b/nolzss_amd/csrc/c_abi.hip
--- a/nolzss_amd/csrc/c_abi.hip
+++ b/nolzss_amd/csrc/c_abi.hip
@@ -179,20 +179,21 @@
     bool isa_deferred = false;
     build_suffix_array(ctx, text, sa, isa, lcp, &isa_deferred);
     const Pyramid Psa = alloc_pyramid(sa, (uint32_t)n, arena), Plcp = alloc_pyramid(lcp, (uint32_t)n + 1, arena);
-    uint32_t *lstar = arena.alloc<uint32_t>(n);
+    LstarCodes lstar = alloc_lstar(ctx, (uint32_t)n, isa_deferred && !lengths);
     build_lstar(ctx, (uint32_t)n, sa, isa, lcp, Psa, Plcp, lstar, isa_deferred ? isa : nullptr, &text);
     if (dbg) {
+        const size_t dmark = arena.mark();
+        const uint32_t *lstar32 = lstar.width == 32 ? lstar.wide : widened_lstar(ctx, lstar, (uint32_t)n, 0);
         copy_out(ctx, dbg->sa, sa, n);
         copy_out(ctx, dbg->isa, isa, n);
         copy_out(ctx, dbg->lcp, lcp, n + 1);
-        copy_out(ctx, dbg->lstar, lstar, n);
+        copy_out(ctx, dbg->lstar, lstar32, n);
         if (dbg->records) {
-            const size_t rmark = arena.mark();
-            const void *recs = position_factors(ctx, (uint32_t)n, lstar, sa, isa, lcp, Psa, Plcp);
+            const void *recs = position_factors(ctx, (uint32_t)n, lstar32, sa, isa, lcp, Psa, Plcp);
             HIP_CHECK(hipMemcpyAsync(dbg->records, recs, n * sizeof(nolzss_factor), hipMemcpyDeviceToHost, s));
-            HIP_CHECK(hipStreamSynchronize(s));
-            arena.rewind(rmark);
-        }
+        }
+        HIP_CHECK(hipStreamSynchronize(s));
+        arena.rewind(dmark);
     }
     void *d_recs = nullptr;
     const uint32_t z = resolve_chain(ctx, (uint32_t)n, (uint32_t)start_pos, lstar, sa, isa, lcp, Psa, Plcp,
diff --git a/nolzss_amd/csrc/chain.hip b/nolzss_amd/csrc/chain.hip
--- a/nolzss_amd/csrc/chain.hip
+++ b/nolzss_amd/csrc/chain.hip
@@ -20,49 +20,91 @@
     return nx > n ? n : (uint32_t)nx;
 }
 
-__global__ __launch_bounds__(kThreads) void chain_exit_kernel(const uint32_t *__restrict__ lstar, uint32_t n,
-                                                              uint32_t start_pos,
-                                                              uint32_t *__restrict__ exit0,
+template <typename CodeT>
+__global__ __launch_bounds__(kThreads) void chain_exit_kernel(const CodeT *__restrict__ lstar, uint32_t n,
+                                                              uint32_t start_pos, CodeT *__restrict__ exit0,
                                                               uint32_t *__restrict__ target_bits) {
-    __shared__ uint32_t jump[kTile];
+    constexpr bool kNarrow = sizeof(CodeT) == 2;
+    __shared__ __align__(8) uint32_t jump[kTile];
     const uint32_t base = blockIdx.x * (uint32_t)kTile;
     const uint32_t tile_end = (n - base < (uint32_t)kTile) ? n : base + kTile;
     const int tid = threadIdx.x;
-    uint32_t ls[kPerThread];
-#pragma unroll
-    for (int j = 0; j < kPerThread; ++j) {
-        const uint32_t p = base + j * kThreads + tid;
-        ls[j] = lstar[p < n ? p : n - 1u];
-    }
-#pragma unroll
-    for (int j = 0; j < kPerThread; ++j) {
-        const uint32_t lp = j * kThreads + tid;
-        const uint32_t p = base + lp;
-        jump[lp] = (p < n) ? next_pos(p, ls[j], n) : n;
+    if constexpr (kNarrow) {
+        const uint32_t *__restrict__ pairs = reinterpret_cast<const uint32_t *>(lstar);
+        const uint32_t last_pair = (n - 1u) >> 1;
+        uint32_t ls[kPerThread / 2];
+#pragma unroll
+        for (int j = 0; j < kPerThread / 2; ++j) {
+            const uint32_t pr = (base >> 1) + j * kThreads + tid;
+            ls[j] = pairs[pr < last_pair ? pr : last_pair];
+        }
+#pragma unroll
+        for (int j = 0; j < kPerThread / 2; ++j) {
+            const uint32_t lp = 2u * (j * kThreads + tid);
+            const uint32_t p = base + lp;
+            uint2 v;
+            v.x = (p < n) ? next_pos(p, ls[j] & 0xffffu, n) : n;
+            v.y = (p + 1u < n) ? next_pos(p + 1u, ls[j] >> 16, n) : n;
+            *reinterpret_cast<uint2 *>(&jump[lp]) = v;
+        }
+    } else {
+        uint32_t ls[kPerThread];
+#pragma unroll
+        for (int j = 0; j < kPerThread; ++j) {
+            const uint32_t p = base + j * kThreads + tid;
+            ls[j] = lstar[p < n ? p : n - 1u];
+        }
+#pragma unroll
+        for (int j = 0; j < kPerThread; ++j) {
+            const uint32_t lp = j * kThreads + tid;
+            const uint32_t p = base + lp;
+            jump[lp] = (p < n) ? next_pos(p, ls[j], n) : n;
+        }
     }
     __syncthreads();
+    uint32_t own[kPerThread];
+#pragma unroll
+    for (int j = 0; j < kPerThread; ++j) own[j] = jump[j * kThreads + tid];
     for (int round = 0; round < 13; ++round) {
         int changed = 0;
 #pragma unroll
         for (int j = 0; j < kPerThread; ++j) {
+            if (own[j] < tile_end) {
+                own[j] = jump[own[j] - base];
+                jump[j * kThreads + tid] = own[j];
+                changed = 1;
+            }
+        }
+        if (!__syncthreads_or(changed)) break;
+    }
+    if constexpr (kNarrow) {
+        uint32_t *__restrict__ exit_pairs = reinterpret_cast<uint32_t *>(exit0);
+#pragma unroll
+        for (int j = 0; j < kPerThread / 2; ++j) {
+            const uint32_t lp = 2u * (j * kThreads + tid);
+            const uint32_t p = base + lp;
+            if (p < n) {
+                const uint2 e = *reinterpret_cast<const uint2 *>(&jump[lp]);
+                const bool second = p + 1u < n;
+                exit_pairs[p >> 1] = ((e.x - tile_end) & 0xffffu) | (second ? (e.y - tile_end) << 16 : 0u);
+                if (e.x < n && (!second || e.y != e.x)) atomicOr(&target_bits[e.x >> 5], 1u << (e.x & 31));
+                if (second) {
+                    const bool last = (lp + 2u == (uint32_t)kTile) || (p + 2u >= n);
+                    if (e.y < n && (last || jump[lp + 2] != e.y)) atomicOr(&target_bits[e.y >> 5], 1u << (e.y & 31));
+                }
+            }
+        }
+    } else {
+#pragma unroll
+        for (int j = 0; j < kPerThread; ++j) {
             const uint32_t lp = j * kThreads + tid;
-            const uint32_t t = jump[lp];
-            if (t < tile_end) {
-                jump[lp] = jump[t - base];
-                changed = 1;
-            }
-        }
-        if (!__syncthreads_or(changed)) break;
-    }
-#pragma unroll
-    for (int j = 0; j < kPerThread; ++j) {
-        const uint32_t lp = j * kThreads + tid;
-        const uint32_t p = base + lp;
-        if (p < n) {
-            const uint32_t e = jump[lp];
-            exit0[p] = e;
-            const bool last = (lp + 1 == (uint32_t)kTile) || (p + 1 >= n);
-            if (e < n && (last || jump[lp + 1] != e)) atomicOr(&target_bits[e >> 5], 1u << (e & 31));
+            const uint32_t p = base + lp;
+            if (p < n) {
+                const uint32_t e = jump[lp];
+                exit0[p] = e;
+                const bool last = (lp + 1 == (uint32_t)kTile) || (p + 1 >= n);
+                if (e < n && (last || jump[lp + 1] != e)) atomicOr(&target_bits[e >> 5], 1u << (e & 31));
+            }
         }
     }
     if (blockIdx.x == 0 && tid == 0 && start_pos < n) atomicOr(&target_bits[start_pos >> 5], 1u << (start_pos & 31));
@@ -94,8 +136,9 @@
     return prefix[p >> 5] + (uint32_t)__popc(bits[p >> 5] & ((1u << (p & 31)) - 1u));
 }
 
+template <typename ExitT>
 __global__ __launch_bounds__(kThreads) void node_edges_kernel(const uint32_t *__restrict__ node_pos, uint32_t K,
-                                                              const uint32_t *__restrict__ exit0, uint32_t n,
+                                                              const ExitT *__restrict__ exit0, uint32_t n,
                                                               const uint32_t *__restrict__ bits,
                                                               const uint32_t *__restrict__ prefix,
                                                               uint32_t start_pos, uint32_t *__restrict__ nxt,
@@ -108,7 +151,11 @@
             continue;
         }
         const uint32_t p = node_pos[k];
-        const uint32_t e = exit0[p];
+        uint32_t e = exit0[p];
+        if constexpr (sizeof(ExitT) == 2) {
+            const uint32_t tbase = p / (uint32_t)kTile * (uint32_t)kTile;
+            e += (n - tbase < (uint32_t)kTile) ? n : tbase + kTile;
+        }
         nxt[k] = (e >= n) ? K : node_id(bits, prefix, e);
         reach[k] = (p == start_pos) ? 1u : 0u;
     }
@@ -140,11 +187,12 @@
         }
 }
 
-__global__ __launch_bounds__(64) void chain_mark_kernel(const uint32_t *__restrict__ lstar, uint32_t n,
+template <typename CodeT>
+__global__ __launch_bounds__(64) void chain_mark_kernel(const CodeT *__restrict__ lstar, uint32_t n,
                                                         const uint32_t *__restrict__ entry,
                                                         unsigned long long *__restrict__ chain_bits,
                                                         uint32_t *__restrict__ tile_count) {
-    __shared__ uint16_t jmp[kTile];
+    __shared__ __align__(4) uint16_t jmp[kTile];
     __shared__ unsigned long long bits[kTile / 64];
     const uint32_t base = blockIdx.x * (uint32_t)kTile;
     const uint32_t tile_end = (n - base < (uint32_t)kTile) ? n : base + kTile;
@@ -157,23 +205,41 @@
         return;
     }
     constexpr int kBatch = 16;
-    for (int j0 = 0; j0 < kTile / 64; j0 += kBatch) {
-        uint32_t ls[kBatch];
-#pragma unroll
-        for (int j = 0; j < kBatch; ++j) {
-            const uint32_t p = base + (uint32_t)(j0 + j) * 64u + lane;
-            ls[j] = lstar[p < n ? p : n - 1u];
-        }
-#pragma unroll
-        for (int j = 0; j < kBatch; ++j) {
-            const uint32_t lp = (uint32_t)(j0 + j) * 64u + lane;
-            const uint32_t p = base + lp;
-            uint32_t nl = kTile;
-            if (p < n) {
-                const uint32_t nx = next_pos(p, ls[j], n);
-                if (nx < tile_end) nl = nx - base;
-            }
-            jmp[lp] = (uint16_t)nl;
+    auto local_next = [&](uint32_t p, uint32_t code) -> uint32_t {
+        if (p >= n) return (uint32_t)kTile;
+        const uint32_t nx = next_pos(p, code, n);
+        return nx < tile_end ? nx - base : (uint32_t)kTile;
+    };
+    if constexpr (sizeof(CodeT) == 2) {
+        const uint32_t *__restrict__ pairs = reinterpret_cast<const uint32_t *>(lstar);
+        const uint32_t last_pair = (n - 1u) >> 1;
+        for (int j0 = 0; j0 < kTile / 128; j0 += kBatch) {
+            uint32_t ls[kBatch];
+#pragma unroll
+            for (int j = 0; j < kBatch; ++j) {
+                const uint32_t pr = (base >> 1) + (uint32_t)(j0 + j) * 64u + lane;
+                ls[j] = pairs[pr < last_pair ? pr : last_pair];
+            }
+#pragma unroll
+            for (int j = 0; j < kBatch; ++j) {
+                const uint32_t lp = 2u * ((uint32_t)(j0 + j) * 64u + lane);
+                const uint32_t p = base + lp;
+                *reinterpret_cast<uint32_t *>(&jmp[lp]) = local_next(p, ls[j] & 0xffffu) | (local_next(p + 1u, ls[j] >> 16) << 16);
+            }
+        }
+    } else {
+        for (int j0 = 0; j0 < kTile / 64; j0 += kBatch) {
+            uint32_t ls[kBatch];
+#pragma unroll
+            for (int j = 0; j < kBatch; ++j) {
+                const uint32_t p = base + (uint32_t)(j0 + j) * 64u + lane;
+                ls[j] = lstar[p < n ? p : n - 1u];
+            }
+#pragma unroll
+            for (int j = 0; j < kBatch; ++j) {
+                const uint32_t lp = (uint32_t)(j0 + j) * 64u + lane;
+                jmp[lp] = (uint16_t)local_next(base + lp, ls[j]);
+            }
         }
     }
     bits[lane] = 0ull;
@@ -257,9 +323,9 @@
     uint64_t start, length, ref;
 };
 
-template <bool kRC, bool kRebase>
+template <bool kRC, bool kRebase, typename CodeT = uint32_t>
 __global__ __launch_bounds__(kThreads) void factor_kernel(const uint32_t *__restrict__ fpos, uint32_t z,
-                                                          const uint32_t *__restrict__ lstar,
+                                                          const CodeT *__restrict__ lstar,
                                                           const uint32_t *__restrict__ isa,
                                                           const uint32_t *__restrict__ sa,
                                                           const uint32_t *__restrict__ lcp, Pyramid Psa,
@@ -343,7 +409,7 @@
 
 }
 
-uint32_t resolve_chain(Context &ctx, uint32_t n, uint32_t start_pos, const uint32_t *lstar, const uint32_t *sa,
+uint32_t resolve_chain(Context &ctx, uint32_t n, uint32_t start_pos, const LstarCodes &codes, const uint32_t *sa,
                        const uint32_t *isa, const uint32_t *lcp, const Pyramid &Psa, const Pyramid &Plcp,
                        void **d_factors_out, uint32_t rcN, const Pyramid *Pmax, uint32_t **d_fpos_out,
                        const TermTable *rebase, const ChainLengthsOut *lengths) {
@@ -352,20 +418,28 @@
     if (d_factors_out) *d_factors_out = nullptr;
     if (d_fpos_out) *d_fpos_out = nullptr;
     if (start_pos >= n) return 0;
+    const bool narrow = codes.width == 16;
+    if (narrow && (rcN || rebase || lengths)) throw HipError("resolve_chain: 16-bit codes are for plain records and counts only");
+    const uint32_t *lstar = codes.wide;
+    const uint16_t *lstar16 = codes.narrow;
 
     const uint32_t num_tiles = (uint32_t)div_up(n, kTile);
     const uint32_t tbits_words = (uint32_t)div_up((size_t)n + 1, 32);
 
     uint32_t *fpos = nullptr;
     const size_t mark = arena.mark();
-    uint32_t *exit0 = arena.alloc<uint32_t>(n);
+    uint32_t *exit0 = narrow ? nullptr : arena.alloc<uint32_t>(n);
+    uint16_t *exit16 = narrow ? arena.alloc<uint16_t>((size_t)n + 2) : nullptr;
     uint32_t *tbits = arena.alloc<uint32_t>(tbits_words);
     uint32_t *tprefix = arena.alloc<uint32_t>(tbits_words);
     uint32_t *d_total = arena.alloc<uint32_t>(2);
     HIP_CHECK(hipMemsetAsync(tbits, 0, sizeof(uint32_t) * tbits_words, s));
     {
-        ProfScope ps(ctx.profiler(), "chain_exit", s);
-        chain_exit_kernel<<<num_tiles, kThreads, 0, s>>>(lstar, n, start_pos, exit0, tbits);
+        ProfScope ps(ctx.profiler(), "chain_exit", s, (narrow ? 4.0 : 8.0) * (double)n);
+        if (narrow)
+            chain_exit_kernel<uint16_t><<<num_tiles, kThreads, 0, s>>>(lstar16, n, start_pos, exit16, tbits);
+        else
+            chain_exit_kernel<uint32_t><<<num_tiles, kThreads, 0, s>>>(lstar, n, start_pos, exit0, tbits);
         KERNEL_CHECK();
     }
     {
@@ -385,8 +459,12 @@
         ProfScope ps(ctx.profiler(), "chain_nodes", s);
         node_fill_kernel<<<grid_for(tbits_words), kThreads, 0, s>>>(tbits, tprefix, tbits_words, node_pos);
         KERNEL_CHECK();
-        node_edges_kernel<<<grid_for((size_t)K + 1), kThreads, 0, s>>>(node_pos, K, exit0, n, tbits, tprefix,
-                                                                       start_pos, nxt[0], reach);
+        if (narrow)
+            node_edges_kernel<uint16_t><<<grid_for((size_t)K + 1), kThreads, 0, s>>>(node_pos, K, exit16, n, tbits, tprefix,
+                                                                                     start_pos, nxt[0], reach);
+        else
+            node_edges_kernel<uint32_t><<<grid_for((size_t)K + 1), kThreads, 0, s>>>(node_pos, K, exit0, n, tbits, tprefix,
+                                                                                     start_pos, nxt[0], reach);
         KERNEL_CHECK();
     }
     {
@@ -406,8 +484,11 @@
     unsigned long long *cbits = arena.alloc<unsigned long long>((size_t)num_tiles * (kTile / 64));
     uint32_t *tile_count = arena.alloc<uint32_t>(num_tiles);
     {
-        ProfScope ps(ctx.profiler(), "chain_mark", s);
-        chain_mark_kernel<<<num_tiles, 64, 0, s>>>(lstar, n, entry, cbits, tile_count);
+        ProfScope ps(ctx.profiler(), "chain_mark", s, (narrow ? 2.0 : 4.0) * (double)n);
+        if (narrow)
+            chain_mark_kernel<uint16_t><<<num_tiles, 64, 0, s>>>(lstar16, n, entry, cbits, tile_count);
+        else
+            chain_mark_kernel<uint32_t><<<num_tiles, 64, 0, s>>>(lstar, n, entry, cbits, tile_count);
         KERNEL_CHECK();
         scan_exclusive_add_u32(tile_count, tile_count, num_tiles, d_total + 1, arena, s);
     }
@@ -464,6 +545,9 @@
         } else if (rebase) {
             factor_kernel<false, true><<<grid_for(z), kThreads, 0, s>>>(fpos, z, lstar, isa, sa, lcp, Psa, Plcp, Psa,
                                                                         0u, recs_tmp, *rebase, n);
+        } else if (narrow) {
+            factor_kernel<false, false, uint16_t><<<grid_for(z), kThreads, 0, s>>>(fpos, z, lstar16, isa, sa, lcp, Psa, Plcp,
+                                                                                   Psa, 0u, recs_tmp, TermTable{}, n);
         } else {
             factor_kernel<false, false><<<grid_for(z), kThreads, 0, s>>>(fpos, z, lstar, isa, sa, lcp, Psa, Plcp, Psa,
                                                                          0u, recs_tmp, TermTable{}, n);
diff --git a/nolzss_amd/csrc/code16.hpp b/nolzss_amd/csrc/code16.hpp
--- /dev/null
+++ b/nolzss_amd/csrc/code16.hpp
@@ -0,0 +1,49 @@
+#pragma once
+#include "common.hpp"
+
+namespace nolzss {
+
+struct WideCodes {
+    uint64_t *items = nullptr;
+    uint32_t *count = nullptr;
+    uint32_t cap = 0;
+    uint32_t max = 0xffffu;
+};
+
+struct LstarCodes {
+    uint32_t *wide = nullptr;
+    uint16_t *narrow = nullptr;
+    WideCodes list;
+    int width = 32;
+
+    static LstarCodes of(uint32_t *codes) {
+        LstarCodes c;
+        c.wide = codes;
+        return c;
+    }
+};
+
+__device__ __forceinline__ void append_wide_code(const WideCodes &wl, uint32_t i, uint32_t code, bool big) {
+    const uint64_t bal = __ballot(big);
+    if (bal == 0) return;
+    const int leader = __builtin_ctzll(bal);
+    uint32_t slot = 0;
+    if (lane_id() == leader) slot = atomicAdd(wl.count, (uint32_t)__popcll(bal));
+    slot = (uint32_t)__shfl((int)slot, leader, 64) + (uint32_t)__popcll(bal & lanemask_lt());
+    if (big && slot < wl.cap) wl.items[slot] = (uint64_t)i | ((uint64_t)code << 32);
+}
+
+__device__ __forceinline__ void store_code(const LstarCodes &c, uint32_t i, uint32_t code) {
+    if (c.narrow == nullptr) {
+        c.wide[i] = code;
+        return;
+    }
+    const bool big = code >= c.list.max;
+    c.narrow[i] = (uint16_t)(big ? c.list.max : code);
+    append_wide_code(c.list, i, code, big);
+}
+__device__ __forceinline__ uint32_t load_code_bound(const LstarCodes &c, uint32_t i) {
+    return c.narrow ? (uint32_t)c.narrow[i] : c.wide[i];
+}
+
+}
diff --git a/nolzss_amd/csrc/lpnf.hip b/nolzss_amd/csrc/lpnf.hip
--- a/nolzss_amd/csrc/lpnf.hip
+++ b/nolzss_amd/csrc/lpnf.hip
@@ -1,5 +1,6 @@
 #include "pipeline.hpp"
 
+#include <algorithm>
 #include <cstdlib>
 #include "nearest_lds.hpp"
 #include "queues.hpp"
@@ -166,7 +167,7 @@
                                                            Pyramid Psa, Pyramid Plcp,
                                                            const uint32_t *__restrict__ by_rank,
                                                            const uint32_t *__restrict__ far_aux, bool bounded,
-                                                           uint32_t *__restrict__ lstar, uint32_t *__restrict__ far_exact) {
+                                                           LstarCodes lstar, uint32_t *__restrict__ far_exact) {
     const size_t stride = (size_t)gridDim.x * blockDim.x;
     for (size_t k = (size_t)blockIdx.x * blockDim.x + threadIdx.x; k < far_count; k += stride) {
         const uint32_t r = far_list[k];
@@ -188,44 +189,108 @@
             jp = (aux & 0x7fffffffu) == 0x7fffffffu ? kNoPos : (aux & 0x7fffffffu);
             far_down<false>(sa, n, Psa, Plcp, r, i, lp, ls, js);
         }
-        far_exact[k] = lpf_decide(i, lp, jp, ls, js, lstar + i) ? i : kNoPos;
+        uint32_t code;
+        far_exact[k] = lpf_decide(i, lp, jp, ls, js, &code) ? i : kNoPos;
+        store_code(lstar, i, code);
     }
 }
 
 __global__ __launch_bounds__(kThreads) void lpnf_fallback_list_kernel(const uint32_t *__restrict__ far_exact,
                                                                       uint32_t far_count, uint32_t n,
                                                                       const uint32_t *__restrict__ isa, Pyramid Psa,
-                                                                      Pyramid Plcp, uint32_t *__restrict__ lstar) {
+                                                                      Pyramid Plcp, LstarCodes lstar) {
     const size_t stride = (size_t)gridDim.x * blockDim.x;
     for (size_t k = (size_t)blockIdx.x * blockDim.x + threadIdx.x; k < far_count; k += stride) {
         const uint32_t i = far_exact[k];
         if (i == kNoPos) continue;
         const uint32_t cap = (n - i) < i ? (n - i) : i;
-        lstar[i] = lpnf_search(Psa, Plcp, isa[i] - 1u, i, lstar[i], cap);
+        store_code(lstar, i, lpnf_search(Psa, Plcp, isa[i] - 1u, i, load_code_bound(lstar, i), cap));
     }
 }
 
 __global__ __launch_bounds__(kThreads) void lpnf_fallback_kernel(ShardQueue exact_q, uint32_t n,
                                                                  const uint32_t *__restrict__ isa,
-                                                                 Pyramid Psa, Pyramid Plcp,
-                                                                 uint32_t *__restrict__ lstar) {
+                                                                 Pyramid Psa, Pyramid Plcp, LstarCodes lstar) {
     const uint32_t shard = blockIdx.x;
     const uint32_t count = exact_q.counts[shard * kQPad];
     const uint32_t *items = exact_q.items + (size_t)shard * exact_q.cap;
     for (uint32_t k = blockIdx.y * blockDim.x + threadIdx.x; k < count; k += gridDim.y * blockDim.x) {
         const uint32_t i = items[k];
         const uint32_t cap = (n - i) < i ? (n - i) : i;
-        lstar[i] = lpnf_search(Psa, Plcp, isa[i] - 1u, i, lstar[i], cap);
-    }
-}
-
+        store_code(lstar, i, lpnf_search(Psa, Plcp, isa[i] - 1u, i, load_code_bound(lstar, i), cap));
+    }
+}
+
+__global__ __launch_bounds__(kThreads) void widen_codes_kernel(const uint32_t *__restrict__ pairs, uint32_t npairs,
+                                                               uint2 *__restrict__ wide) {
+    const size_t stride = (size_t)gridDim.x * blockDim.x;
+    for (size_t k = (size_t)blockIdx.x * blockDim.x + threadIdx.x; k < npairs; k += stride) {
+        const uint32_t v = pairs[k];
+        wide[k] = make_uint2(v & 0xffffu, v >> 16);
+    }
+}
+__global__ __launch_bounds__(kThreads) void apply_wide_codes_kernel(WideCodes wl, uint32_t count, uint32_t n,
+                                                                    uint32_t *__restrict__ wide) {
+    const size_t stride = (size_t)gridDim.x * blockDim.x;
+    for (size_t k = (size_t)blockIdx.x * blockDim.x + threadIdx.x; k < count; k += stride) {
+        const uint64_t e = wl.items[k];
+        const uint32_t i = (uint32_t)e;
+        if (i < n) atomicMax(&wide[i], (uint32_t)(e >> 32));
+    }
+}
+
+}
+
+LstarCodes alloc_lstar(Context &ctx, uint32_t n, bool want_narrow) {
+    const SortKnobs &knobs = sort_knobs();
+    LstarCodes c;
+    if (want_narrow && !knobs.no_code16 && ctx.code16_off_n != n && packed_text_order_applies(n, ctx.rec_plan != nullptr)) {
+        c.narrow = ctx.arena.alloc<uint16_t>((size_t)n + 8);
+        c.list.cap = (uint32_t)std::max<size_t>(n / 64, 1024);
+        c.list.items = ctx.arena.alloc<uint64_t>(c.list.cap);
+        c.list.count = ctx.arena.alloc<uint32_t>(1);
+        c.list.max = knobs.code16_max;
+        c.width = 16;
+    } else {
+        c.wide = ctx.arena.alloc<uint32_t>(n);
+    }
+    return c;
+}
+
+uint32_t *widened_lstar(Context &ctx, const LstarCodes &codes, uint32_t n, uint32_t listed) {
+    if (!codes.narrow) return codes.wide;
+    hipStream_t s = ctx.stream;
+    ProfScope ps(ctx.profiler(), "widen_codes", s, 6.0 * (double)n);
+    const uint32_t npairs = (uint32_t)div_up((size_t)n, 2);
+    uint32_t *wide = ctx.arena.alloc<uint32_t>(2 * (size_t)npairs);
+    widen_codes_kernel<<<(unsigned)std::min<size_t>(div_up(npairs, kThreads), 256u * 16u), kThreads, 0, s>>>(
+        reinterpret_cast<const uint32_t *>(codes.narrow), npairs, reinterpret_cast<uint2 *>(wide));
+    KERNEL_CHECK();
+    if (listed) {
+        apply_wide_codes_kernel<<<(unsigned)std::min<size_t>(div_up(listed, kThreads), 1024u), kThreads, 0, s>>>(codes.list, listed,
+                                                                                                                n, wide);
+        KERNEL_CHECK();
+    }
+    return wide;
 }
 
 uint32_t build_lstar(Context &ctx, uint32_t n, const uint32_t *sa, const uint32_t *isa, const uint32_t *lcp,
-                     const Pyramid &Psa, const Pyramid &Plcp, uint32_t *lstar, uint32_t *isa_fill,
+                     const Pyramid &Psa, const Pyramid &Plcp, LstarCodes &lstar, uint32_t *isa_fill,
                      const PackedText *fill_pyramids) {
     hipStream_t s = ctx.stream;
     const size_t mark = ctx.arena.mark();
+    static const bool trace = getenv("NOLZSS_TRACE") != nullptr;
+    if (lstar.narrow && !isa_fill) throw HipError("build_lstar: the 16-bit codes come out of the two-value permutation only");
+    if (lstar.narrow) HIP_CHECK(hipMemsetAsync(lstar.list.count, 0, sizeof(uint32_t), s));
+    auto redo_with_wide_codes = [&]() {
+        ctx.arena.rewind(mark);
+        ctx.code16_off_n = n;
+        lstar.narrow = nullptr;
+        lstar.list = WideCodes{};
+        lstar.wide = ctx.arena.alloc<uint32_t>(n);
+        lstar.width = 32;
+        return build_lstar(ctx, n, sa, isa, lcp, Psa, Plcp, lstar, isa_fill, nullptr);
+    };
     uint32_t *pending_flag = nullptr;
     if (fill_pyramids) {
         pending_flag = ctx.arena.alloc<uint32_t>(1);
@@ -310,11 +375,15 @@
         ProfScope ps(ctx.profiler(), "lpf_to_text_order", s);
         uint32_t *idx[2] = {const_cast<uint32_t *>(sa), scratch_idx};
         uint32_t *val[2] = {by_rank, scratch_val};
-        bucketed_scatter(idx, val, n, lstar, n, ctx.arena, s, ctx.profiler(), true, true, ctx.rec_plan, isa_fill);
+        const bool done = bucketed_scatter(idx, val, n, lstar.wide, n, ctx.arena, s, ctx.profiler(), true, true, ctx.rec_plan,
+                                           isa_fill, true, lstar.narrow ? &lstar : nullptr);
+        if (!done) {
+            if (trace) fprintf(stderr, "[nolzss] code16: the packed text-order form did not finish, 32-bit codes instead\n");
+            return redo_with_wide_codes();
+        }
     }
     uint32_t h[2] = {0, 0};
     read_totals(h);
-    static const bool trace = getenv("NOLZSS_TRACE") != nullptr;
     if (trace) fprintf(stderr, "[nolzss] lpf: %u ranks to the far queue, %u positions to the exact search so far\n", h[1], h[0]);
     if (h[1] > 0) {
         ProfScope ps(ctx.profiler(), "lpf_far", s);
@@ -336,7 +405,30 @@
         lpnf_fallback_kernel<<<dim3(kQShards, gy), kThreads, 0, s>>>(exact_q, n, isa, Psa, Plcp, lstar);
         KERNEL_CHECK();
     }
+    if (!lstar.narrow) {
+        lstar.width = 32;
+        ctx.arena.rewind(mark);
+        return h[0];
+    }
+    uint32_t listed = 0;
+    ctx.read_back(lstar.list.count, &listed, 1);
+    if (listed > lstar.list.cap) {
+        if (trace)
+            fprintf(stderr, "[nolzss] code16: wide-code list overflow, %u codes >= %u (cap %u): 32-bit codes instead\n", listed,
+                    lstar.list.max, lstar.list.cap);
+        return redo_with_wide_codes();
+    }
     ctx.arena.rewind(mark);
+    if (listed == 0) {
+        lstar.width = 16;
+        if (trace) fprintf(stderr, "[nolzss] code16: narrow cursor, 0 wide codes (max %u)\n", lstar.list.max);
+    } else {
+        lstar.wide = widened_lstar(ctx, lstar, n, listed);
+        lstar.width = 32;
+        if (trace)
+            fprintf(stderr, "[nolzss] code16: widened, %u wide codes >= %u applied (cap %u)\n", listed, lstar.list.max,
+                    lstar.list.cap);
+    }
     return h[0];
 }
 
diff --git a/nolzss_amd/csrc/pipeline.hpp b/nolzss_amd/csrc/pipeline.hpp
--- a/nolzss_amd/csrc/pipeline.hpp
+++ b/nolzss_amd/csrc/pipeline.hpp
@@ -1,4 +1,5 @@
 #pragma once
+#include "code16.hpp"
 #include "common.hpp"
 #include "pyramid.hpp"
 #include "text.hpp"
@@ -16,6 +17,7 @@
     uint8_t *h_stage = nullptr;
     size_t h_stage_cap = 0;
     const struct RecordScatterPlan *rec_plan = nullptr;
+    uint32_t code16_off_n = 0;
 
     Profiler *profiler() { return prof.enabled() ? &prof : nullptr; }
     void read_back(const uint32_t *d_src, uint32_t *dst, int count);
@@ -31,8 +33,10 @@
 
 struct Pyramid;
 
+LstarCodes alloc_lstar(Context &ctx, uint32_t n, bool want_narrow);
+uint32_t *widened_lstar(Context &ctx, const LstarCodes &codes, uint32_t n, uint32_t listed);
 uint32_t build_lstar(Context &ctx, uint32_t n, const uint32_t *sa, const uint32_t *isa, const uint32_t *lcp,
-                     const Pyramid &Psa, const Pyramid &Plcp, uint32_t *lstar, uint32_t *isa_fill = nullptr,
+                     const Pyramid &Psa, const Pyramid &Plcp, LstarCodes &lstar, uint32_t *isa_fill = nullptr,
                      const PackedText *fill_pyramids = nullptr);
 uint32_t pending_threshold();
 void finish_pending_lcp(Context &ctx, const PackedText &text, const uint32_t *sa, uint32_t *lcp);
@@ -47,7 +51,7 @@
     uint32_t **order = nullptr;
 };
 inline uint32_t length_tail_cap(uint32_t n) { return n / kLengthHistBins + 1u; }
-uint32_t resolve_chain(Context &ctx, uint32_t n, uint32_t start_pos, const uint32_t *lstar, const uint32_t *sa,
+uint32_t resolve_chain(Context &ctx, uint32_t n, uint32_t start_pos, const LstarCodes &lstar, const uint32_t *sa,
                        const uint32_t *isa, const uint32_t *lcp, const Pyramid &Psa, const Pyramid &Plcp,
                        void **d_factors_out, uint32_t rcN = 0, const Pyramid *Pmax = nullptr,
                        uint32_t **d_fpos_out = nullptr, const TermTable *rebase = nullptr,
diff --git a/nolzss_amd/csrc/radix_sort.hip b/nolzss_amd/csrc/radix_sort.hip
--- a/nolzss_amd/csrc/radix_sort.hip
+++ b/nolzss_amd/csrc/radix_sort.hip
@@ -24,6 +24,9 @@
     text_order_hist = set("NOLZSS_TEXT_ORDER_HIST");
     const char *esc = getenv("NOLZSS_TEXT_ORDER_ESC");
     text_order_esc = esc ? (long long)strtoul(esc, nullptr, 0) : -1;
+    no_code16 = set("NOLZSS_NO_CODE16");
+    const long long c16 = i64("NOLZSS_CODE16_MAX", 0xffff);
+    code16_max = (uint32_t)(c16 < 1 ? 1 : (c16 > 0xffff ? 0xffff : c16));
 }
 
 const SortKnobs &sort_knobs() {
diff --git a/nolzss_amd/csrc/radix_sort.hpp b/nolzss_amd/csrc/radix_sort.hpp
--- a/nolzss_amd/csrc/radix_sort.hpp
+++ b/nolzss_amd/csrc/radix_sort.hpp
@@ -76,6 +76,8 @@
     uint64_t rec_bucket_min;
     bool text_order_hist;
     long long text_order_esc;
+    bool no_code16;
+    uint32_t code16_max;
 };
 const SortKnobs &sort_knobs();
 
diff --git a/nolzss_amd/csrc/rc.hip b/nolzss_amd/csrc/rc.hip
--- a/nolzss_amd/csrc/rc.hip
+++ b/nolzss_amd/csrc/rc.hip
@@ -496,12 +496,12 @@
         HIP_CHECK(hipStreamSynchronize(s));
         arena.rewind(mark);
     }
-    const uint32_t z = resolve_chain(ctx, N, (uint32_t)start_pos, code, sa, isa, lcp, Pmin, Plcp, d_factors_out, N, &Pmax,
+    const uint32_t z = resolve_chain(ctx, N, (uint32_t)start_pos, LstarCodes::of(code), sa, isa, lcp, Pmin, Plcp, d_factors_out, N, &Pmax,
                                      d_fpos_out, nullptr, lengths);
     if (plain_out) {
         ProfScope ps(ctx.profiler(), "plain_chain", s);
         plain_out->fpos = nullptr;
-        plain_out->z = resolve_chain(ctx, N, 0, plain, sa, isa, lcp, Pmin, Plcp, nullptr, 0, nullptr,
+        plain_out->z = resolve_chain(ctx, N, 0, LstarCodes::of(plain), sa, isa, lcp, Pmin, Plcp, nullptr, 0, nullptr,
                                      plain_out->want_fpos ? &plain_out->fpos : nullptr);
     }
     return z;
diff --git a/nolzss_amd/csrc/rlz.hip b/nolzss_amd/csrc/rlz.hip
--- a/nolzss_amd/csrc/rlz.hip
+++ b/nolzss_amd/csrc/rlz.hip
@@ -341,7 +341,7 @@
         HIP_CHECK(hipMemcpyAsync(h_codes, code, (size_t)lay.chain_end * sizeof(uint32_t), hipMemcpyDeviceToHost, s));
         HIP_CHECK(hipStreamSynchronize(s));
     }
-    return resolve_chain(ctx, lay.chain_end, lay.block_length + 1u, code, sa, isa, lcp, Pmin, Plcp, d_factors_out, lay.rcN,
+    return resolve_chain(ctx, lay.chain_end, lay.block_length + 1u, LstarCodes::of(code), sa, isa, lcp, Pmin, Plcp, d_factors_out, lay.rcN,
                          lay.with_rc ? &Pmax : nullptr, d_fpos_out);
 }
 
diff --git a/nolzss_amd/csrc/text_order.hip b/nolzss_amd/csrc/text_order.hip
--- a/nolzss_amd/csrc/text_order.hip
+++ b/nolzss_amd/csrc/text_order.hip
@@ -489,15 +489,58 @@
     }
 }
 
+__global__ __launch_bounds__(kWindow2Threads) void window_unpack16_kernel(const uint64_t *__restrict__ in,
+                                                                          uint16_t *__restrict__ out,
+                                                                          uint32_t *__restrict__ out2, uint32_t n_out,
+                                                                          int window_bits, int low_bits, int rank_bits,
+                                                                          WideCodes wl) {
+    __shared__ __align__(16) uint32_t s_b[1 << kWindowBitsMax];
+    __shared__ __align__(16) uint16_t s_a[1 << kWindowBitsMax];
+    const uint32_t W = 1u << window_bits;
+    const size_t base = (size_t)blockIdx.x << window_bits;
+    const uint32_t len = (uint32_t)((n_out - base < (size_t)W) ? (n_out - base) : (size_t)W);
+    const uint32_t rank_mask = (uint32_t)((1ull << rank_bits) - 1ull);
+    constexpr int kBatch = 4;
+    for (uint32_t t0 = 0; t0 < len; t0 += kBatch * kWindow2Threads) {
+        uint64_t vv[kBatch];
+#pragma unroll
+        for (int j = 0; j < kBatch; ++j) {
+            const uint32_t t = t0 + (uint32_t)j * kWindow2Threads + threadIdx.x;
+            vv[j] = in[base + (t < len ? t : 0u)];
+        }
+#pragma unroll
+        for (int j = 0; j < kBatch; ++j) {
+            const uint32_t t = t0 + (uint32_t)j * kWindow2Threads + threadIdx.x;
+            const uint32_t at = (uint32_t)vv[j] & (W - 1u);
+            const uint32_t code = (uint32_t)(vv[j] >> (low_bits + rank_bits));
+            const bool big = t < len && code >= wl.max;
+            if (t < len) {
+                s_a[at] = (uint16_t)(big ? wl.max : code);
+                s_b[at] = ((uint32_t)(vv[j] >> low_bits) & rank_mask) + 1u;
+            }
+            append_wide_code(wl, (uint32_t)base + at, code, big);
+        }
+    }
+    __syncthreads();
+    for (uint32_t t = threadIdx.x; t < len; t += kWindow2Threads) out2[base + t] = s_b[t];
+    for (uint32_t t = threadIdx.x * 8u; t < len; t += kWindow2Threads * 8u) {
+        if (t + 8u <= len) {
+            *reinterpret_cast<uint4 *>(out + base + t) = *reinterpret_cast<const uint4 *>(s_a + t);
+        } else {
+            for (uint32_t k = t; k < len; ++k) out[base + k] = s_a[k];
+        }
+    }
+}
+
 __global__ __launch_bounds__(kThreads) void escape_fixup_kernel(const uint32_t *__restrict__ exc, const uint32_t *__restrict__ ctl,
                                                                 uint32_t cap, const uint32_t *__restrict__ idx,
-                                                                const uint32_t *__restrict__ code, uint32_t *__restrict__ out) {
+                                                                const uint32_t *__restrict__ code, LstarCodes out) {
     const uint32_t cnt = ctl[2];
     if (cnt > cap) return;
     const size_t stride = (size_t)gridDim.x * blockDim.x;
     for (size_t k = (size_t)blockIdx.x * blockDim.x + threadIdx.x; k < cnt; k += stride) {
         const uint32_t r = exc[k];
-        out[idx[r]] = code[r];
+        store_code(out, idx[r], code[r]);
     }
 }
 
@@ -517,7 +560,7 @@
     }
 }
 
-bool packed_text_order(const uint32_t *idx, const uint32_t *code, size_t count, uint32_t *out, uint32_t *out2, int nb, int wb,
+bool packed_text_order(const uint32_t *idx, const uint32_t *code, size_t count, const LstarCodes &out, uint32_t *out2, int nb, int wb,
                        uint64_t *buf_a, Arena &arena, hipStream_t stream, Profiler *prof) {
     const bool trace = sort_knobs().trace;
     const int low_bits = wb + kRadixBits;
@@ -562,9 +605,13 @@
         KERNEL_CHECK();
     }
     {
-        ProfScope ps(prof, "window_scatter", stream, 16.0 * (double)count);
-        window_unpack_kernel<<<(unsigned)div_up(count, (size_t)1 << wb), kWindow2Threads, 0, stream>>>(
-            buf_b, out, out2, (uint32_t)count, wb, low_bits, nb);
+        ProfScope ps(prof, "window_scatter", stream, (out.narrow ? 14.0 : 16.0) * (double)count);
+        const unsigned windows = (unsigned)div_up(count, (size_t)1 << wb);
+        if (out.narrow)
+            window_unpack16_kernel<<<windows, kWindow2Threads, 0, stream>>>(buf_b, out.narrow, out2, (uint32_t)count, wb, low_bits,
+                                                                           nb, out.list);
+        else
+            window_unpack_kernel<<<windows, kWindow2Threads, 0, stream>>>(buf_b, out.wide, out2, (uint32_t)count, wb, low_bits, nb);
         KERNEL_CHECK();
         escape_fixup_kernel<<<256, kThreads, 0, stream>>>(exc, ctl, cap, idx, code, out);
         KERNEL_CHECK();
@@ -794,10 +841,10 @@
 
 }
 
-void bucketed_scatter(uint32_t *idx[2], uint32_t *val[2], size_t count, uint32_t *out, uint32_t n_out, Arena &arena,
+bool bucketed_scatter(uint32_t *idx[2], uint32_t *val[2], size_t count, uint32_t *out, uint32_t n_out, Arena &arena,
                       hipStream_t stream, Profiler *prof, bool keep_input, bool keep_val, const RecordScatterPlan *plan,
-                      uint32_t *out2, bool short_codes) {
-    if (count == 0) return;
+                      uint32_t *out2, bool short_codes, const LstarCodes *narrow) {
+    if (count == 0) return narrow == nullptr;
     const size_t amark = arena.mark();
     const int nbits = index_bits(n_out);
     const bool two_passes = nbits <= 2 * kRadixBits + kWindowBitsMax;
@@ -808,11 +855,12 @@
     const bool plan_form = has_plan && count == n_out && n_out == plan->n;
     const bool two_value = out2 && perm && two_passes && !has_plan;
     if (two_value && short_codes && !sort_knobs().text_order_hist) {
-        const bool done = packed_text_order(idx[0], val[0], count, out, out2, nbits, wb, reinterpret_cast<uint64_t *>(val[1]), arena,
-                                            stream, prof);
+        const bool done = packed_text_order(idx[0], val[0], count, narrow ? *narrow : LstarCodes::of(out), out2, nbits, wb,
+                                            reinterpret_cast<uint64_t *>(val[1]), arena, stream, prof);
         arena.rewind(amark);
-        if (done) return;
-    }
+        if (done) return true;
+    }
+    if (narrow) return false;
     bool separators_ok = true;
     if (two_value) {
         two_value_hist_form(idx, val, count, out, out2, n_out, wb, keep_input, arena, stream, prof);
@@ -827,6 +875,12 @@
     }
     arena.rewind(amark);
     if (!separators_ok) throw HipError("record scatter: a separator suffix is not the first of its record");
+    return true;
+}
+
+bool packed_text_order_applies(size_t count, bool has_plan) {
+    const int nbits = index_bits(count);
+    return count > (size_t(1) << 24) && nbits <= 2 * kRadixBits + kWindowBitsMax && !has_plan && !sort_knobs().text_order_hist;
 }
 
 void permute_packed(uint32_t *idx, uint64_t *packed, size_t count, uint32_t *out, uint32_t *out2, Arena &arena,
diff --git a/nolzss_amd/csrc/text_order.hpp b/nolzss_amd/csrc/text_order.hpp
--- a/nolzss_amd/csrc/text_order.hpp
+++ b/nolzss_amd/csrc/text_order.hpp
@@ -1,4 +1,5 @@
 #pragma once
+#include "code16.hpp"
 #include "radix_sort.hpp"
 
 #include <vector>
@@ -14,9 +15,11 @@
     uint32_t n = 0;
     int window_bits = 0;
 };
-void bucketed_scatter(uint32_t *idx[2], uint32_t *val[2], size_t count, uint32_t *out, uint32_t n_out,
+bool bucketed_scatter(uint32_t *idx[2], uint32_t *val[2], size_t count, uint32_t *out, uint32_t n_out,
                       Arena &arena, hipStream_t stream, Profiler *prof, bool keep_input, bool keep_val = true,
-                      const RecordScatterPlan *plan = nullptr, uint32_t *out2 = nullptr, bool short_codes = true);
+                      const RecordScatterPlan *plan = nullptr, uint32_t *out2 = nullptr, bool short_codes = true,
+                      const LstarCodes *narrow = nullptr);
+bool packed_text_order_applies(size_t count, bool has_plan);
 void permute_packed(uint32_t *idx, uint64_t *packed, size_t count, uint32_t *out, uint32_t *out2, Arena &arena,
                     hipStream_t stream, Profiler *prof);
 bool record_scatter_plan(const std::vector<uint32_t> &h_terms, uint32_t n, Arena &arena, hipStream_t stream,
```

Result: faster. 13.94 billion bases/s, median of 6 (+1.7%).
